# vxlerian/cpu-raymarcher

Measured on AMD Instinct MI355X. Metric: frames/sec, 3840x2160 Dense-Grid sphere-trace (+ avg SDF-calls/pixel), higher is better.
Workload: dtype f64

## Files before the change

cpu_raymarcher_amd/_native.py:

```python
import ctypes as C
import os
import subprocess

_PKG = os.path.dirname(os.path.abspath(__file__))
LIB_PATH = os.environ.get("RM_HIP_LIB") or os.path.join(_PKG, "librm_hip.so")
CSRC = os.path.join(_PKG, "csrc")

RM_OK = 0
RM_E_INVALID = -1
RM_E_UNSUPPORTED = -2
RM_E_NO_DEVICE = -3
RM_E_HIP = -4
RM_E_NO_SCENE = -5
RM_E_NOMEM = -6
RM_SCENE_UPLOADED = -(2 ** 31)

_STATUS_NAMES = {0: "RM_OK", -1: "RM_E_INVALID", -2: "RM_E_UNSUPPORTED", -3: "RM_E_NO_DEVICE",
                 -4: "RM_E_HIP", -5: "RM_E_NO_SCENE", -6: "RM_E_NOMEM"}


class RmError(RuntimeError):
    def __init__(self, code, msg):
        super().__init__("%s (%d): %s" % (_STATUS_NAMES.get(code, "?"), code, msg))
        self.code = code
# ... 48 lines not shown
class rm_field_shade(C.Structure):
    _fields_ = [("map", C.c_int32), ("reserved", C.c_int32), ("range", C.c_double), ("band", C.c_double), ("line", C.c_double),
                ("lo", C.c_uint32), ("hi", C.c_uint32)]


FIELD_MAPS = {"distance": 0, "count": 1}


class rm_point_query(C.Structure):
    _fields_ = [("time", C.c_double), ("iso", C.c_double), ("snap_tol", C.c_double), ("snap_steps", C.c_int32), ("flags", C.c_int32),
                ("reserved", C.c_int32 * 2)]


RM_POINT_NORMAL = 1


class rm_mesh_info(C.Structure):
    _fields_ = [("n_vertices", C.c_int64), ("n_quads", C.c_int64), ("n_holes", C.c_int64), ("reserved", C.c_int64)]


RM_MESH_F64, RM_MESH_F32 = 0, 1


class rm_view(C.Structure):
    _fields_ = [("camera_pitch", C.c_double), ("camera_yaw", C.c_double), ("time", C.c_double)]


class rm_frame_set(C.Structure):
    _fields_ = [("depth", C.c_void_p), ("normal", C.c_void_p), ("sdf", C.c_void_p), ("iters", C.c_void_p)]


class rm_compare_stats(C.Structure):
    _fields_ = [(name, C.c_uint64) for name in (
        "pixels", "sum_sdf_a", "sum_sdf_b", "sum_iters_a", "sum_iters_b", "sum_abs_depth", "surface_a", "surface_b",
        "surface_only_a", "surface_only_b", "depth_differs", "normal_differs", "counters_differ", "b_cheaper", "a_cheaper")] + \
        [("max_abs_depth", C.c_uint32), ("max_abs_normal", C.c_uint32)]


COMPARE_MAPS = {"none": -1, "sdf": 0, "iters": 1, "depth": 2, "normal": 3, "surface": 4}

RM_HIST_BINS = 256


class rm_counter_hist(C.Structure):
    _fields_ = [("pixels", C.c_uint64), ("sum", C.c_uint64), ("min", C.c_uint32), ("max", C.c_uint32), ("range_lo", C.c_uint32),
                ("range_hi", C.c_uint32), ("shift", C.c_uint32), ("reserved", C.c_uint32), ("bins", C.c_uint32 * RM_HIST_BINS)]


class rm_frame_hist(C.Structure):
    _fields_ = [("sdf", rm_counter_hist), ("iters", rm_counter_hist)]


HIST_MASKS = {"all": 0, "surface": 1, "background": 2}


class rm_scene_info(C.Structure):
    _fields_ = [("n_prims", C.c_int32), ("accel", C.c_int32), ("preset_index", C.c_int32),
                ("bvh_nodes", C.c_int32), ("bvh_leaves", C.c_int32), ("bvh_depth", C.c_int32),
                ("oct_nodes", C.c_int32), ("oct_leaves", C.c_int32), ("oct_empty_leaves", C.c_int32),
                ("oct_max_leaf_prims", C.c_int32), ("root_min", C.c_float * 3), ("root_max", C.c_float * 3),
                ("nodes_in_lds", C.c_int32), ("program", C.c_int32)]


class rm_node(C.Structure):
    _fields_ = [("type", C.c_int32), ("child_a", C.c_int32), ("child_b", C.c_int32), ("reserved", C.c_int32),
                ("world_to_local", C.c_float * 16), ("params", C.c_double * 6)]


class rm_prim(C.Structure):
    _fields_ = [("type", C.c_int32), ("reserved", C.c_int32), ("world_to_local", C.c_float * 16),
                ("params", C.c_double * 3), ("reserved2", C.c_double)]


class rm_sphere_edit(C.Structure):
    _fields_ = [("op", C.c_int32), ("index", C.c_int32), ("center", C.c_float * 3), ("reserved", C.c_int32),
                ("radius", C.c_double)]


RM_EDIT_SET, RM_EDIT_INSERT, RM_EDIT_REMOVE = 0, 1, 2
EDIT_OPS = {"set": 0, "insert": 1, "remove": 2}
SCENE_TABLES = {"spheres": "<f4", "radii": "<f8", "bvh": "u1", "bvh_prims": "<i4", "oct": "u1", "oct_prims": "<i4",
                "pq_cells": "<u4", "pq_list": "<u2", "nn_cells": "<u4", "nn_list": "<u2", "prims": "u1", "prog": "u1",
                "obj_ranges": "<i4", "oct_recs": "u1", "oct_lut": "<i4", "oct_sub_hdr": "<u4", "oct_sub_list": "u1",
                "slot_object": "<i4", "ext_cells": "<u4", "ext_list": "<u2", "step_tab": "<u4"}
STEP_BOX_BINS, STEP_BOX_CAP = 32, 62


class rm_diagnostics(C.Structure):
    _fields_ = [("total_sdf_calls", C.c_uint64), ("total_iterations", C.c_uint64),
                ("max_sdf_calls", C.c_uint32), ("min_sdf_calls", C.c_uint32), ("total_pixels", C.c_uint64)]


_VP = C.c_void_p
SIGNATURES = {
    "rm_create": (C.c_int, [C.c_int, C.POINTER(_VP)]),
    "rm_destroy": (None, [_VP]),
    "rm_last_error": (C.c_char_p, [_VP]),
    "rm_last_kernel": (C.c_char_p, [_VP]),
    "rm_version": (C.c_char_p, []),
    "rm_algorithm_from_string": (C.c_int, [C.c_char_p]),
    "rm_accel_from_string": (C.c_int, [C.c_char_p]),
    "rm_shader_from_string": (C.c_int, [C.c_char_p]),
    "rm_preset_count": (C.c_int, []),
    "rm_scene_from_preset": (C.c_int, [_VP, C.c_int32, C.c_int32]),
    "rm_scene_from_spheres": (C.c_int, [_VP, _VP, _VP, C.c_int32, C.c_int32]),
    "rm_scene_edit_spheres": (C.c_int, [_VP, C.POINTER(rm_sphere_edit), C.c_int32]),
    "rm_debug_scene_table": (C.c_int, [_VP, C.c_char_p, C.c_int32, _VP, C.c_int64, C.POINTER(C.c_int64)]),
    "rm_selftest_hypot64": (C.c_int, [_VP, _VP, C.c_int64, C.c_int32, _VP]),
    "rm_scene_from_prims": (C.c_int, [_VP, C.POINTER(rm_prim), C.c_int32, C.c_int32]),
    "rm_make_transform": (C.c_int, [C.c_double, C.c_double, C.c_double, _VP, _VP]),
    "rm_scene_from_nodes": (C.c_int, [_VP, C.POINTER(rm_node), C.c_int32, _VP, C.c_int32, C.c_int32]),
    "rm_scale_transform": (C.c_int, [_VP, C.c_double, C.c_double, C.c_double]),
    "rm_scene_set_time": (C.c_int, [_VP, C.c_double]),
    "rm_selftest_jsmath": (C.c_int, [_VP, C.c_int32, _VP, _VP, C.c_int64, _VP]),
    "rm_scene_get_info": (C.c_int, [_VP, C.POINTER(rm_scene_info)]),
    "rm_camera_from_angles": (C.c_int, [C.c_double, C.c_double, _VP, _VP]),
    "rm_scene_distance": (C.c_int, [_VP, _VP, C.c_int64, _VP, _VP]),
    "rm_debug_wave_distance": (C.c_int, [_VP, _VP, C.c_int64, _VP, _VP]),
    "rm_scene_field": (C.c_int, [_VP, C.POINTER(rm_lattice), _VP, _VP, _VP]),
    "rm_scene_field_device": (C.c_int, [_VP, C.POINTER(rm_lattice), _VP, _VP, _VP, _VP]),
    "rm_scene_points": (C.c_int, [_VP, C.POINTER(rm_point_query), C.c_int64, _VP, _VP, _VP, _VP, _VP, _VP, _VP]),
    "rm_scene_points_device": (C.c_int, [_VP, C.POINTER(rm_point_query), C.c_int64, _VP, _VP, _VP, _VP, _VP, _VP, _VP, _VP]),
    "rm_lattice_points": (C.c_int, [C.POINTER(rm_lattice), C.c_int64, C.c_int64, _VP]),
    "rm_shade_field_device": (C.c_int, [_VP, C.POINTER(rm_field_shade), C.c_int64, _VP, _VP, _VP]),
    "rm_shade_field": (C.c_int, [_VP, C.POINTER(rm_field_shade), C.c_int64, _VP, _VP]),
    "rm_mesh_field_device": (C.c_int, [_VP, C.POINTER(rm_lattice), _VP, C.c_int32, C.c_double, _VP, C.c_int64, _VP, C.c_int64, _VP, _VP]),
    "rm_scene_mesh": (C.c_int, [_VP, C.POINTER(rm_lattice), C.c_double, _VP, C.c_int64, _VP, C.c_int64, C.POINTER(rm_mesh_info)]),
    "rm_ray_march": (C.c_int, [_VP, C.POINTER(rm_ray_query), C.c_int64, _VP, _VP, _VP, _VP, _VP, _VP]),
    "rm_ray_march_device": (C.c_int, [_VP, C.POINTER(rm_ray_query), C.c_int64, _VP, _VP, _VP, _VP, _VP, _VP, _VP]),
    "rm_camera_rays": (C.c_int, [C.c_int32, C.c_int32, C.c_double, C.c_double, C.c_int32, C.c_int32, _VP, _VP]),
    "rm_ray_pick": (C.c_int, [_VP, C.POINTER(rm_ray_query), C.c_int64, _VP, _VP, _VP, _VP, _VP, _VP, _VP]),
    "rm_ray_pick_device": (C.c_int, [_VP, C.POINTER(rm_ray_query), C.c_int64, _VP, _VP, _VP, _VP, _VP, _VP, _VP, _VP]),
    "rm_ray_light": (C.c_int, [_VP, C.POINTER(rm_ray_query), C.POINTER(rm_light), C.c_int64, _VP, _VP, _VP, _VP, _VP, _VP, _VP, _VP, _VP,
                               _VP]),
    "rm_ray_light_device": (C.c_int, [_VP, C.POINTER(rm_ray_query), C.POINTER(rm_light), C.c_int64, _VP, _VP, _VP, _VP, _VP, _VP, _VP, _VP,
                                      _VP, _VP, _VP]),
    "rm_ray_walk": (C.c_int, [_VP, C.POINTER(rm_ray_query), C.c_int64, _VP, _VP, C.c_int32, _VP, _VP]),
    "rm_ray_walk_device": (C.c_int, [_VP, C.POINTER(rm_ray_query), C.c_int64, _VP, _VP, C.c_int32, _VP, _VP, _VP]),
    "rm_phong_light": (C.c_int, [_VP]),
    "rm_shade_lit_device": (C.c_int, [_VP, C.c_int32, C.c_int32, C.c_int32, _VP, _VP, _VP, _VP, _VP, _VP]),
    "rm_shade_lit": (C.c_int, [_VP, C.c_int32, C.c_int32, C.c_int32, _VP, _VP, _VP, _VP, _VP]),
    "rm_scene_object": (C.c_int, [_VP, C.c_int32, C.POINTER(rm_node), C.c_int32, C.POINTER(C.c_int32)]),
    "rm_render_tile": (C.c_int, [_VP, C.POINTER(rm_job), _VP, _VP, _VP, _VP]),
    "rm_render_tile_device": (C.c_int, [_VP, C.POINTER(rm_job), C.c_int32, _VP, _VP, _VP, _VP, _VP, _VP]),
    "rm_render_frames_device": (C.c_int, [_VP, C.POINTER(rm_job), C.c_int32, _VP, C.c_int32, _VP, _VP, _VP, _VP, _VP, _VP, _VP]),
    "rm_compare_frames_device": (C.c_int, [_VP, C.c_int32, C.c_int32, C.c_int32, C.POINTER(rm_frame_set), C.POINTER(rm_frame_set),
                                           C.c_int32, C.c_int32, _VP, _VP, _VP]),
    "rm_compare_frames": (C.c_int, [_VP, C.c_int32, C.c_int32, C.c_int32, C.POINTER(rm_frame_set), C.POINTER(rm_frame_set),
                                    C.c_int32, C.c_int32, _VP, _VP]),
    "rm_counter_hist_device": (C.c_int, [_VP, C.c_int32, C.c_int32, C.c_int32, _VP, _VP, _VP, C.c_int32, C.c_int32, C.c_int32, C.c_int32,
                                         _VP, _VP]),
    "rm_counter_hist": (C.c_int, [_VP, C.c_int32, C.c_int32, C.c_int32, _VP, _VP, _VP, C.c_int32, C.c_int32, C.c_int32, C.c_int32, _VP]),
    "rm_shade_ranged_device": (C.c_int, [_VP, C.c_int32, C.c_int32, C.c_int32, C.c_int32, _VP, _VP, C.c_uint32, C.c_uint32, _VP, _VP]),
    "rm_shade_ranged": (C.c_int, [_VP, C.c_int32, C.c_int32, C.c_int32, C.c_int32, _VP, _VP, C.c_uint32, C.c_uint32, _VP]),
    "rm_sweep_views": (C.c_int, [C.c_double, C.c_double, C.c_double, C.c_double, C.c_double, C.c_double, C.c_int32, _VP]),
    "rm_render_stripes_device": (C.c_int, [_VP, C.POINTER(rm_job), C.c_int32, C.c_int32, C.c_int32, C.c_int32,
                                           _VP, _VP, _VP, _VP, _VP, _VP]),
    "rm_stripe_rows": (C.c_int, [C.c_int32, C.c_int32, C.c_int32, C.c_int32, C.c_int32]),
    "rm_deal_stripes": (C.c_int, [C.c_int32, C.c_int32, C.c_int32, _VP, _VP]),
    "rm_render_stripe_list_device": (C.c_int, [_VP, C.POINTER(rm_job), C.c_int32, C.c_int32, _VP, C.c_int32,
                                               _VP, _VP, _VP, _VP, _VP, _VP]),
    "rm_assemble_frame_device": (C.c_int, [_VP, _VP, C.c_int64, C.c_int64, C.c_int32, C.c_int32, C.c_int32, _VP,
                                           C.c_int32, C.c_int32, _VP, C.c_int64, _VP, _VP]),
    "rm_shade": (C.c_int, [_VP, C.c_int32, C.c_int32, C.c_int32, _VP, _VP, _VP, _VP, _VP]),
    "rm_shade_device": (C.c_int, [_VP, C.c_int32, C.c_int32, C.c_int32, _VP, _VP, _VP, _VP, _VP, _VP]),
    "rm_reduce_counters": (C.c_int, [_VP, _VP, _VP, C.c_int64, C.POINTER(rm_diagnostics)]),
    "rm_reduce_counters_device": (C.c_int, [_VP, _VP, _VP, C.c_int64, C.POINTER(rm_diagnostics), _VP]),
    "rm_reduce_counters_enqueue": (C.c_int, [_VP, _VP, _VP, C.c_int64, _VP, _VP]),
    "rm_render_attach_diagnostics": (C.c_int, [_VP, _VP]),
    "rm_partition_rows": (C.c_int, [C.c_int32, C.c_int32, C.c_int32, C.POINTER(C.c_int32), C.POINTER(C.c_int32)]),
    "rm_selftest_hypot": (C.c_int, [_VP, _VP, C.c_int64, _VP]),
    "rm_selftest_fastdiv": (C.c_int, [_VP, C.c_uint64, C.c_int64, C.POINTER(C.c_uint64)]),
    "rm_selftest_recip": (C.c_int, [_VP, C.c_int, _VP]),
    "rm_debug_read_stamps": (C.c_int, [_VP, _VP]),
    "rm_debug_read_wave_times": (C.c_int, [_VP, _VP]),
    "rm_debug_read_batch_log": (C.c_int, [_VP, _VP]),
    "rm_debug_read_counts": (C.c_int, [_VP, _VP]),
    "rm_debug_read_lpt_costs": (C.c_int, [_VP, _VP, C.c_int64]),
    "rm_debug_launch_fill": (C.c_int, [_VP, C.c_int32, C.POINTER(C.c_int32)]),
    "rm_debug_last_launch": (C.c_int, [_VP, C.POINTER(C.c_uint32)]),
    "rm_debug_overlap_fill": (C.c_int, [_VP, C.c_int32, C.c_int64, C.POINTER(C.c_int32)]),
    "rm_debug_step_box": (C.c_int, [_VP, C.POINTER(C.c_int32)]),
    "rm_debug_rect_cull": (C.c_int, [_VP, _VP, _VP, C.c_int32, C.c_int32, C.POINTER(C.c_int32)]),
    "rm_debug_leaf_rects": (C.c_int, [_VP, _VP, _VP, C.c_int32, C.c_int32, _VP, _VP, C.c_int64, C.POINTER(C.c_int64)]),
    "rm_rtc_source": (C.c_int, [_VP, C.c_char_p, C.c_int64, C.POINTER(C.c_int64)]),
    "rm_rtc_compile_check": (C.c_int, [_VP, C.c_int32, C.c_int32, C.c_char_p, C.c_int64, C.POINTER(C.c_double)]),
    "rm_rtc_status": (C.c_int, [_VP, C.POINTER(C.c_int32), C.POINTER(C.c_int32), C.c_char_p, C.c_int64]),
    "rm_set_option": (C.c_int, [_VP, C.c_char_p, C.c_int64]),
    "rm_get_option": (C.c_int, [_VP, C.c_char_p, C.POINTER(C.c_int64)]),
}

_lib = None


def build(force=False, verbose=False):
    srcs = [os.path.join(CSRC, f) for f in os.listdir(CSRC) if f.endswith((".hip", ".cpp", ".h"))]
    srcs.append(os.path.join(os.path.dirname(_PKG), "include", "rm_raymarch.h"))
    if not force and os.path.exists(LIB_PATH) and all(
            os.path.getmtime(LIB_PATH) >= os.path.getmtime(s) for s in srcs):
        return LIB_PATH
    cmd = ["make", "-j%d" % min(8, os.cpu_count() or 1), "-C", CSRC, "all"] + (["-B"] if force else [])
    subprocess.check_call(cmd, stdout=None if verbose else subprocess.DEVNULL)
    return LIB_PATH


def lib():
    global _lib
    if _lib is None:
        if not os.path.exists(LIB_PATH):
            raise ImportError(
                "cpu_raymarcher_amd: %s is missing. Build it with `python -c 'import __graft_entry__ as g; "
                "g.build()'` or `make -C cpu_raymarcher_amd/csrc`. There is no CPU fallback." % LIB_PATH)
        try:
            import torch
        except ImportError:
            pass
        L = C.CDLL(LIB_PATH)
        for name, (res, args) in SIGNATURES.items():
            if os.environ.get("RM_HIP_LIB") and not hasattr(L, name):
                continue
            fn = getattr(L, name)
            fn.restype = res
            fn.argtypes = args
        _lib = L
    return _lib


def check(ctx, rc):
    if rc == RM_OK:
        return
    msg = lib().rm_last_error(ctx).decode() if ctx else ""
    raise (RmUnsupported if rc == RM_E_UNSUPPORTED else RmError)(rc, msg)
```

cpu_raymarcher_amd/context.py:

```python
import collections
import ctypes as C

import numpy as np

from . import _native as N

Points = collections.namedtuple("Points", "position dist normal object steps count")


def _is_torch(x):
    return type(x).__module__.startswith("torch")


def _ptr(x):
    if x is None:
        return None
    if _is_torch(x):
        return C.c_void_p(x.data_ptr())
    return x.ctypes.data_as(C.c_void_p)


_BPP = {"depth": 1, "normal": 3, "sdf": 2, "iters": 2, "rgba": 4}


# ... 53 lines not shown
    if not (_is_torch(hist) or isinstance(hist, np.ndarray)):
        raise ValueError("hist must be a numpy array or a torch tensor")
    d = bool(_is_torch(hist) and hist.is_cuda)
    contiguous = hist.is_contiguous() if _is_torch(hist) else hist.flags["C_CONTIGUOUS"]
    nbytes = hist.numel() * hist.element_size() if _is_torch(hist) else hist.nbytes
    if not contiguous or nbytes < 2128 * max(0, n_frames):
        raise ValueError("hist must be a contiguous buffer of 2128 bytes per frame")
    if on_dev is not None and on_dev != d:
        raise ValueError("buffers must be all on the host or all on the device")
    return d


def percentile(record, permille):
    p = int(permille)
    if not 0 <= p <= 1000:
        raise ValueError("permille must be in [0, 1000]")
    M = int(record["pixels"])
    if M == 0:
        return 0, 0
    r = p * (M - 1) // 1000
    b = int(np.searchsorted(np.cumsum(np.asarray(record["bins"], dtype=np.uint64)), r, side="right"))
    shift, mn, mx = int(record["shift"]), int(record["min"]), int(record["max"])
    return max(mn, b << shift), (mx if b == 255 else min(mx, ((b + 1) << shift) - 1))


def _current_stream_ptr():
    import torch
    return C.c_void_p(torch.cuda.current_stream().cuda_stream)


class Context:

    def __init__(self, device=0):
        self._h = C.c_void_p()
        self.device = -1 if device is None else int(device)
        rc = N.lib().rm_create(self.device, C.byref(self._h))
        if rc != N.RM_OK:
            raise N.RmError(rc, "rm_create(device=%d) failed: no usable HIP device" % self.device)

    def close(self):
        if self._h:
            N.lib().rm_destroy(self._h)
            self._h = C.c_void_p()

    def __del__(self):
        try:
            self.close()
        except Exception:
            pass

    def __enter__(self):
        return self

    def __exit__(self, *a):
        self.close()

    def set_option(self, key, value):
        N.check(self._h, N.lib().rm_set_option(self._h, key.encode(), int(value)))

    def get_option(self, key):
        v = C.c_int64(0)
        N.check(self._h, N.lib().rm_get_option(self._h, key.encode(), C.byref(v)))
        return v.value

    def launch_fill(self, asked):
        v = C.c_int32(0)
        N.check(self._h, N.lib().rm_debug_launch_fill(self._h, int(asked), C.byref(v)))
        return v.value

    def last_launch(self):
        out = (C.c_uint32 * 4)()
        N.check(self._h, N.lib().rm_debug_last_launch(self._h, out))
        return dict(workgroups=out[0], threads=out[1], lds_bytes=out[2], cus=out[3])

    def overlap_fill(self, asked, items):
        v = C.c_int32(0)
        N.check(self._h, N.lib().rm_debug_overlap_fill(self._h, int(asked), int(items), C.byref(v)))
        return v.value

    def step_box(self):
        out = (C.c_int32 * 6)()
        N.check(self._h, N.lib().rm_debug_step_box(self._h, out))
        return dict(last=bool(out[0]), planned=bool(out[1]), reason=out[2], list_cap=out[3], list_cap_without=out[4], table_bytes=out[5])

    def rect_cull(self, rot, origin, width, height):
        r = np.ascontiguousarray(rot, dtype=np.float32).reshape(9)
        o = np.ascontiguousarray(origin, dtype=np.float32).reshape(3)
        out = (C.c_int32 * 5)()
        N.check(self._h, N.lib().rm_debug_rect_cull(self._h, _ptr(r), _ptr(o), int(width), int(height), out))
        return dict(last=bool(out[0]), planned=bool(out[1]), reason=out[2], leaves=out[3], max_leaves=out[4])

    def leaf_rects(self, rot, origin, width, height):
        r = np.ascontiguousarray(rot, dtype=np.float32).reshape(9)
        o = np.ascontiguousarray(origin, dtype=np.float32).reshape(3)
        n = C.c_int64(0)
        N.check(self._h, N.lib().rm_debug_leaf_rects(self._h, _ptr(r), _ptr(o), int(width), int(height), None, None, 0, C.byref(n)))
        rects = np.zeros((max(1, n.value), 4), np.uint16)
        nodes = np.zeros(max(1, n.value), np.int32)
        N.check(self._h, N.lib().rm_debug_leaf_rects(self._h, _ptr(r), _ptr(o), int(width), int(height), _ptr(rects), _ptr(nodes),
                                                     n.value, C.byref(n)))
        return rects[:n.value], nodes[:n.value]

    def scene_from_preset(self, index, accel):
        N.check(self._h, N.lib().rm_scene_from_preset(self._h, int(index), int(accel)))

    def scene_from_spheres(self, centers, radii, accel):
        c = np.ascontiguousarray(centers, dtype=np.float32).reshape(-1, 3)
        r = np.ascontiguousarray(radii, dtype=np.float64).reshape(-1)
        if len(c) != len(r):
            raise ValueError("centers and radii differ in length")
        N.check(self._h, N.lib().rm_scene_from_spheres(self._h, _ptr(c), _ptr(r), len(r), int(accel)))

    def scene_from_prims(self, prims, accel):
        prims = list(prims)
        arr = (N.rm_prim * max(1, len(prims)))()
        for i, (t, m, par) in enumerate(prims):
            arr[i].type = int(t)
            for k in range(16):
                arr[i].world_to_local[k] = float(m[k])
            for k in range(3):
                arr[i].params[k] = float(par[k]) if k < len(par) else 0.0
        N.check(self._h, N.lib().rm_scene_from_prims(self._h, arr, len(prims), int(accel)))

    def scene_from_nodes(self, nodes, roots, accel):
        nodes = list(nodes)
        arr = (N.rm_node * max(1, len(nodes)))()
        for i, (t, a, b, m, par) in enumerate(nodes):
            arr[i].type, arr[i].child_a, arr[i].child_b = int(t), int(a), int(b)
            for k in range(16):
                arr[i].world_to_local[k] = 0.0 if m is None else float(m[k])
            for k in range(6):
                arr[i].params[k] = float(par[k]) if k < len(par) else 0.0
        r = np.ascontiguousarray(roots, dtype=np.int32)
        N.check(self._h, N.lib().rm_scene_from_nodes(self._h, arr, len(nodes), _ptr(r), len(r), int(accel)))

    def edit_spheres(self, edits):
        if isinstance(edits, C.Array) and edits._type_ is N.rm_sphere_edit:
            arr, n = edits, len(edits)
        else:
            edits = list(edits)
            n = len(edits)
            arr = (N.rm_sphere_edit * max(1, n))()
            for k, e in enumerate(edits):
                arr[k].op = N.EDIT_OPS[e[0]] if isinstance(e[0], str) else int(e[0])
                arr[k].index = int(e[1])
                if len(e) > 2:
                    arr[k].center[:] = [float(v) for v in np.asarray(e[2], np.float32).reshape(3)]
                    arr[k].radius = float(e[3])
        N.check(self._h, N.lib().rm_scene_edit_spheres(self._h, arr, n))

    def scene_table(self, name, from_device=True):
        size = C.c_int64(0)
        key = name.encode()
        N.check(self._h, N.lib().rm_debug_scene_table(self._h, key, int(bool(from_device)), None, 0, C.byref(size)))
        out = np.zeros(size.value, np.uint8)
        N.check(self._h, N.lib().rm_debug_scene_table(self._h, key, int(bool(from_device)), _ptr(out), out.size, C.byref(size)))
        return out.view(N.SCENE_TABLES.get(name, "u1"))

    def selftest_hypot64(self, xyz, on_device=True):
        a = np.ascontiguousarray(xyz, dtype=np.float64).reshape(-1, 3)
        out = np.zeros(len(a), np.float64)
        N.check(self._h, N.lib().rm_selftest_hypot64(self._h, _ptr(a), len(a), int(bool(on_device)), _ptr(out)))
        return out

    def scene_set_time(self, time):
        N.check(self._h, N.lib().rm_scene_set_time(self._h, float(time)))
# ... 789 lines not shown
```

cpu_raymarcher_amd/csrc/rm_api.cpp:

```cpp
#include <hip/hip_runtime_api.h>

#include <algorithm>
#include <array>
#include <cerrno>
#include <climits>
#include <cmath>
#include <cstdio>
#include <cstdlib>
#include <cstring>
#include <functional>
#include <limits>
#include <map>
#include <unordered_map>
#include <new>
#include <string>
#include <vector>

#include "../../include/rm_raymarch.h"
#include "rm_diag.h"
#include "rm_kernels.h"
#include "rm_rtc.h"
#include "rm_scene_host.h"

namespace {

#define RM_SCENE_ARRAYS(X)                                                                                                        \
    X(spheres, 1) X(radii, 1) X(bvh, 1) X(bvh_prims, 1) X(oct, 1) X(oct_prims, 1) X(pq_cells, 1) X(pq_list, 1) X(nn_cells, 1)      \
    X(nn_list, 1) X(prims, 1) X(prog, 1) X(obj_ranges, 1) X(oct_recs, 1) X(oct_lut, 1) X(oct_sub_hdr, 1) X(oct_sub_list, 1)       \
    X(slot_object, 0) X(ext_cells, 1) X(ext_list, 1) X(step_tab, 1)

struct DeviceScene {
#define RM_X(name, always) decltype(rmh::HostScene::name)::value_type *name = nullptr;
    RM_SCENE_ARRAYS(RM_X)
#undef RM_X
    uint16_t *bvh_leaves = nullptr;
    int32_t bvh_leaf_count = 0;
};

struct SceneDesc {
    enum Kind { kSpheres, kPrims, kNodes } kind = kSpheres;
    std::vector<float> centers;
    std::vector<double> radii;
    std::vector<rmh::PrimDesc> prims;
    std::vector<rmh::NodeDesc> nodes;
    std::vector<int> roots;
};

struct LaunchSlots {
    static constexpr unsigned kLaunches = 1024, kHeads = 64, kHeadWords = 64;
    unsigned int *heads = nullptr;
    RmDiagBlock *blocks = nullptr;
    RmLeafRect *rects = nullptr;
    unsigned int head_slot = 0, block_slot = 0;

    hipError_t init() {
        const size_t head_bytes = sizeof(unsigned int) * kLaunches * kHeads * kHeadWords, block_bytes = sizeof(RmDiagBlock) * kLaunches;
        hipError_t e = hipMalloc(reinterpret_cast<void **>(&heads), head_bytes);
        if (e == hipSuccess) e = hipMemset(heads, 0, head_bytes);
        if (e == hipSuccess) e = hipMalloc(reinterpret_cast<void **>(&blocks), block_bytes);
        if (e == hipSuccess) e = hipMemset(blocks, 0, block_bytes);
        return e == hipSuccess ? hipMalloc(reinterpret_cast<void **>(&rects), sizeof(RmLeafRect) * kLaunches * RM_RECT_CULL_MAX_LEAVES) : e;
    }
    void release() {
        (void)hipFree(heads);
        (void)hipFree(blocks);
        (void)hipFree(rects);
    }
    RmLeafRect *rects_of_last_heads() { return rects && head_slot ? rects + static_cast<size_t>(RM_RECT_CULL_MAX_LEAVES) * ((head_slot - 1) % kLaunches) : nullptr; }
    unsigned int *take_heads() { return heads ? heads + static_cast<size_t>(kHeads) * kHeadWords * (head_slot++ % kLaunches) : nullptr; }
    RmDiagBlock *take_block() { return blocks ? blocks + block_slot++ % kLaunches : nullptr; }
};

struct RingClaims {
    struct Claim {
        size_t first, n;
        hipEvent_t done;
    };
    size_t next = 0;
    std::vector<Claim> claims;

    void retire_all() {
        for (Claim &c : claims) (void)hipEventDestroy(c.done);
        claims.clear();
        next = 0;
    }
    hipError_t take(size_t n, size_t cap, size_t *first) {
        if (next + n > cap) next = 0;
        const size_t lo = next, hi = next + n;
        for (size_t k = 0; k < claims.size();) {
            const Claim c = claims[k];
            if (c.first < hi && lo < c.first + c.n) {
                const hipError_t e = hipEventSynchronize(c.done);
                if (e != hipSuccess) return e;
                (void)hipEventDestroy(c.done);
                claims.erase(claims.begin() + static_cast<std::ptrdiff_t>(k));
            } else ++k;
        }
        *first = lo;
        next = hi;
        return hipSuccess;
    }
    void launched(size_t first, size_t n, hipStream_t stream) {
        hipEvent_t ev = nullptr;
        if (hipEventCreateWithFlags(&ev, hipEventDisableTiming) == hipSuccess && hipEventRecord(ev, stream) == hipSuccess) {
            claims.push_back(Claim{first, n, ev});
            return;
        }
        if (ev) (void)hipEventDestroy(ev);
        (void)hipStreamSynchronize(stream);
    }
};

// ... 172 lines not shown
        for (auto &u : t.users) {
            (void)hipEventSynchronize(u.second);
            (void)hipEventDestroy(u.second);
        }
        t.users.clear();
        t.valid = false;
        const size_t n = static_cast<size_t>(oct_nodes);
        if (t.nodes < n) {
            (void)hipFree(t.dev);
            t.dev = nullptr;
            t.nodes = 0;
            if (hipMalloc(reinterpret_cast<void **>(&t.dev), n * sizeof(RmOctFrameNode)) == hipSuccess) t.nodes = n;
            else (void)hipGetLastError();
        }
        if (!t.dev || rm_launch_oct_frame_table(oct, oct_nodes, origin, t.dev, stream) != hipSuccess) return nullptr;
        for (int a = 0; a < 3; ++a) t.origin[a] = origin[a];
        t.gen = gen;
        t.valid = true;
        t.builder = stream;
        if (!t.built && hipEventCreateWithFlags(&t.built, hipEventDisableTiming) != hipSuccess) t.built = nullptr;
        if (!t.built || hipEventRecord(t.built, stream) != hipSuccess) (void)hipStreamSynchronize(stream);
        cur = k;
        return &t;
    }
    static void read_by(Table &t, hipStream_t stream) {
        hipEvent_t ev = nullptr;
        for (auto &u : t.users)
            if (u.first == stream) ev = u.second;
        if (!ev) {
            if (hipEventCreateWithFlags(&ev, hipEventDisableTiming) == hipSuccess) t.users.emplace_back(stream, ev);
            else ev = nullptr;
        }
        if (ev) (void)hipEventRecord(ev, stream);
        else (void)hipStreamSynchronize(stream);
    }
    void release() {
        for (Table &t : slots) {
            (void)hipFree(t.dev);
            for (auto &u : t.users) (void)hipEventDestroy(u.second);
            if (t.built) (void)hipEventDestroy(t.built);
        }
    }
};

}

struct rm_ctx {
    int device = -1;
    bool has_device = false;
    std::string err = "";
    hipStream_t stream = nullptr;

    bool have_scene = false;
    bool scene_is_uploaded = false;
    int scene_preset = 0;
    rmh::HostScene host;
    DeviceScene dev;

    bool have_uploaded = false;
    SceneDesc uploaded;
    double time = 0.0;

    void *scratch = nullptr;
    size_t scratch_bytes = 0;
    hipEvent_t scratch_busy = nullptr;
    RmDiagDevice *d_diag = nullptr;
    float light[3] = {0, 0, 0};

    int64_t opt_tile_w = 8;
    bool tile_w_set = false;
    int64_t opt_filter = 1;
    int64_t opt_lds = 1;
    int64_t opt_kernel = 0;
    int64_t opt_list_cap = 32;
    int64_t opt_coop = 1;
    int64_t opt_grid = 1;
    int64_t opt_nn = 2;
    int64_t opt_ext = 1;
    int64_t opt_blocks_per_cu = 6;
    int64_t opt_lds_fill = 0;
    int64_t opt_min_fill = 1;
    int64_t opt_overlap_fill = 1;
    int hw_queues = 4;
    uint32_t last_v2_shape[5] = {0, 0, 0, 0, 0};
    int64_t opt_item_wide = 0;
    int64_t opt_multi_step = 1;
    int64_t opt_step_box = 1;
    int64_t opt_lds_kb = 0;
    int64_t opt_refill = 64;
    int64_t opt_recs = 1;
    int64_t opt_static = 0;
    int64_t opt_lut = 1;
    int64_t opt_cull = 1;
    int64_t opt_rect_cull = 1;
    std::vector<uint16_t> cull_leaves;
    int64_t opt_rel = 1;
    int64_t opt_uniform = 1;
    int64_t opt_sub = 1;
    int64_t opt_hw_xcd = 1;
    int64_t opt_v1_lists = 1;
    int64_t opt_v1_block = 64;
    int64_t opt_oct_lean = 1;
    int64_t opt_lpt = 1;
    LaunchSlots slots;
    LptRing lpt;
    OctTableRing oct_tables;
    FrameRing frames;
    CompareRing compare;
    HistRing hists;
    unsigned long long scene_gen = 0;
    int64_t opt_n0_batch = 64;
    int64_t opt_length = 0;
    const char *last_kernel = "";
    std::string last_kernel_kept;
    int64_t opt_device_build = 1;
    int64_t opt_specialise = 1;
    int64_t opt_rtc_spheres = 16;
    int64_t opt_prune = 1;
    std::string rtc_src;
    std::map<int, rmrtc::Kernel> rtc_kernels;
    std::vector<rmrtc::Kernel> rtc_owned;
    std::map<int, std::string> rtc_failed;
    std::string rtc_log;
    struct V2Special {
        int launches = 0;
        int state = 0;
        bool lite = false;
        rmrtc::Kernel k;
    };
    std::unordered_map<uint64_t, V2Special> v2_special;
    int64_t opt_v2_after = 3;
    struct DevTable {
        std::vector<int32_t> host;
        int32_t *dev = nullptr;
    };
    std::vector<DevTable> tables;
    int64_t opt_item_px = 128;
    void *diag_next = nullptr;
    unsigned long long *d_stamps = nullptr;
    int num_cus = 256;
};

namespace {

int fail(rm_ctx *ctx, int code, const std::string &msg) {
    if (ctx) ctx->err = msg;
    return code;
}

int hip_fail(rm_ctx *ctx, hipError_t e, const char *what) {
    return fail(ctx, RM_E_HIP, std::string(what) + ": " + hipGetErrorString(e));
}

int read_hw_queues() {
    const char *s = std::getenv("GPU_MAX_HW_QUEUES");
    if (!s || !*s) return 4;
    char *end = nullptr;
    errno = 0;
    const long long v = std::strtoll(s, &end, 10);
    if (errno || end == s || *end != '\0' || v <= 0) return 4;
    return static_cast<int>(std::min<long long>(v, INT_MAX));
}

int launch_fill(int asked, int queues, bool min_fill) {
    if (!min_fill) return asked;
    const int q = queues > 0 ? queues : 4;
    return std::max(asked, (RM_V2_WAVES + q - 1) / q);
}

int overlap_fill(int asked, int queues, bool min_fill, bool overlap) {
// ... 567 lines not shown
    p.step_size = std::isnan(job->step_size) ? 0.1 : job->step_size;
    p.local_rows = job->y_end > job->y_start ? job->y_end - job->y_start : 0;
    p.stripe_rows = 0;
    p.n_parts = 1;
    p.part = 0;
    rmh::camera_from_angles(job->camera_pitch, job->camera_yaw, p.rot, p.origin);
    std::memcpy(p.light, ctx->light, sizeof p.light);
    for (int k = 0; k < 9; ++k) p.rot_d[k] = p.rot[k];
    for (int k = 0; k < 3; ++k) {
        p.origin_d[k] = p.origin[k];
        p.light_d[k] = p.light[k];
    }
    fill_scene_view(ctx, p);
    if (!std::isfinite(job->time)) return fail(ctx, RM_E_INVALID, "non-finite time");
    ctx->time = job->time;
    p.time = job->time;
    p.tile_w = static_cast<int32_t>(ctx->opt_tile_w);
    p.nodes_in_lds = static_cast<int32_t>(ctx->opt_lds);
    p.filter = static_cast<int32_t>(ctx->opt_filter);
    p.variant = static_cast<int32_t>(ctx->opt_kernel);
    if (p.variant == 0)
        p.variant = (ctx->host.accel == RM_ACCEL_OCTREE || ctx->host.spheres.size() < 8 ||
                     (ctx->opt_specialise && !ctx->rtc_src.empty() && rmrtc::available(nullptr) &&
                      static_cast<int64_t>(ctx->host.spheres.size()) < ctx->opt_rtc_spheres))
                        ? 1
                        : 2;
    if (p.algorithm != RM_ALG_SPHERE_TRACER) p.variant = 1;
    if (ctx->host.general) p.variant = 1;
    if (p.variant == 1 && !ctx->tile_w_set) p.tile_w = 8;
    p.list_cap = static_cast<int32_t>(ctx->opt_list_cap);
    p.coop = static_cast<int32_t>(ctx->opt_coop);
    p.bvh_prim_count = static_cast<int32_t>(ctx->host.bvh_prims.size());
    p.oct_prim_count = static_cast<int32_t>(ctx->host.oct_prims.size());
    p.blocks_per_cu = static_cast<int32_t>(ctx->opt_blocks_per_cu);
    p.launch_per_cu = launch_fill(p.blocks_per_cu, ctx->hw_queues, ctx->opt_min_fill != 0);
    p.overlap_per_cu = overlap_fill(p.blocks_per_cu, ctx->hw_queues, ctx->opt_min_fill != 0, ctx->opt_overlap_fill != 0);
    p.num_cus = ctx->num_cus;
    p.refill_threshold = static_cast<int32_t>(ctx->opt_refill);
    p.hw_xcd = static_cast<int32_t>(ctx->opt_hw_xcd);
    p.item_px = static_cast<int32_t>(ctx->opt_item_px);
    p.stamps = ctx->d_stamps;
    for (int k = 0; k < 3; ++k) {
        p.pq_dim[k] = ctx->host.pq_dim[k];
        p.pq_origin[k] = ctx->host.pq_origin[k];
        p.pq_inv[k] = ctx->host.pq_inv[k];
        p.pq_cell[k] = ctx->host.pq_inv[k] > 0.f ? static_cast<float>((1.0 / static_cast<double>(ctx->host.pq_inv[k])) * 0.9999) : 0.f;
    }
    p.pq_cell_count = static_cast<int32_t>(ctx->host.pq_cells.size());
    p.pq_list_count = static_cast<int32_t>(ctx->host.pq_list.size());
    p.use_grid = (ctx->opt_grid && !ctx->host.pq_cells.empty()) ? 1 : 0;
    p.pq_cells = ctx->dev.pq_cells;
    p.pq_list = ctx->dev.pq_list;
    p.bvh_leaves = ctx->dev.bvh_leaves;
    p.bvh_leaf_count = (ctx->opt_cull && ctx->host.accel == RM_ACCEL_BVH) ? ctx->dev.bvh_leaf_count : 0;
    p.rect_cull = rect_cull_refusal(ctx, p.rot, p.origin, p.width, p.height) == 0 ? 1 : 0;
    p.nn_cells = ctx->dev.nn_cells;
    p.nn_list = ctx->dev.nn_list;
    p.nn_cell_count = static_cast<int32_t>(ctx->host.nn_cells.size());
    p.nn_list_count = static_cast<int32_t>(ctx->host.nn_list.size());
    const bool nn_on = ctx->opt_nn == 1 || (ctx->opt_nn == 2 && ctx->host.spheres.size() <= 512);
    p.use_nn = (p.use_grid && nn_on && !ctx->host.nn_cells.empty()) ? 1 : 0;
    p.leaf_order = ctx->host.leaf_order ? 1 : 0;
    p.rel_boxes = static_cast<int32_t>(ctx->opt_rel);
    p.n0_batch = static_cast<int32_t>(ctx->opt_n0_batch);
    p.v1_lists = static_cast<int32_t>(ctx->opt_v1_lists);
    p.v1_block = static_cast<int32_t>(ctx->opt_v1_block);
    p.oct_lean = static_cast<int32_t>(ctx->opt_oct_lean);
    p.v1_list_offset = -1;
    p.prim_filter = (ctx->opt_filter && ctx->host.general && !ctx->host.program && ctx->host.prim_filter_ok &&
                     ctx->host.spheres.size() == ctx->host.prims.size()) ? 1 : 0;
    p.lds_budget_kb = static_cast<int32_t>(ctx->opt_lds_kb);
    p.lds_fill = static_cast<int32_t>(ctx->opt_lds_fill);
    p.item_wide = static_cast<int32_t>(ctx->opt_item_wide);
    p.multi_step = static_cast<int32_t>(ctx->opt_multi_step);
    p.step_tab = ctx->dev.step_tab;
    p.sb_bins = ctx->host.sb_bins;
    p.sb_stride = ctx->host.sb_stride;
    for (int k = 0; k < 3; ++k) {
        p.sb_origin[k] = ctx->host.sb_origin[k];
        p.sb_inv[k] = ctx->host.sb_inv[k];
    }
    p.step_box = (ctx->opt_step_box && ctx->opt_multi_step && ctx->host.accel == RM_ACCEL_BVH && !ctx->host.step_tab.empty() &&
                  (ctx->dev.step_tab || !ctx->has_device)) ? 1 : 0;
    p.uniform_radius = 0;
    if (ctx->opt_uniform && !ctx->host.general && ctx->host.spheres.size() >= 2 &&
        ctx->host.spheres.size() <= 256) {
        const auto &sp = ctx->host.spheres;
        const auto &rd = ctx->host.radii;
        bool same = rd.size() == sp.size();
        for (size_t k = 1; same && k < sp.size(); ++k)
            same = std::memcmp(&sp[k].rf, &sp[0].rf, sizeof(float)) == 0 && std::memcmp(&rd[k], &rd[0], sizeof(double)) == 0;
        p.uniform_radius = same ? 1 : 0;
    }
    for (int k = 0; k < 3; ++k) {
        p.nn_dim[k] = ctx->host.nn_dim[k];
        p.nn_inv[k] = ctx->host.nn_inv[k];
    }
    p.oct_recs = ctx->opt_recs ? ctx->dev.oct_recs : nullptr;
    p.oct_sub_hdr = (ctx->opt_sub && ctx->opt_recs) ? ctx->dev.oct_sub_hdr : nullptr;
    p.oct_sub_list = ctx->dev.oct_sub_list;
    return RM_OK;
}

template <typename Launch>
int read_mismatches(rm_ctx *ctx, Launch launch, uint64_t *mismatches) {
    RM_HIP(ctx, hipSetDevice(ctx->device));
    Staging st{ctx};
    const size_t o = st.region(sizeof(unsigned long long));
    const int rc = st.reserve();
    if (rc) return rc;
    RM_HIP(ctx, st.zero(o, sizeof(unsigned long long)));
    RM_HIP(ctx, launch(st.at<unsigned long long>(o)));
    unsigned long long h = 0;
    RM_HIP(ctx, st.out(&h, o, sizeof h));
    RM_HIP(ctx, st.sync());
    *mismatches = h;
    return RM_OK;
}

int norm_shader(int s) { return (s >= RM_SHADE_NORMAL && s <= RM_SHADE_ITERATION_HEATMAP) ? s : RM_SHADE_NORMAL; }

int fill_query_params(rm_ctx *ctx, const rm_ray_query *q, RmRenderParams &p) {
    const double scene_time = ctx->time;
    rm_job job;
    std::memset(&job, 0, sizeof job);
    job.width = 1;
    job.height = 1;
    job.y_end = 1;
    job.time = q->time;
    const bool known = q->algorithm >= RM_ALG_SPHERE_TRACER && q->algorithm <= RM_ALG_ADAPTIVE_STEP_V3;
    job.algorithm = known ? q->algorithm : RM_ALG_SPHERE_TRACER;
    job.scene_preset_index = ctx->scene_is_uploaded ? RM_SCENE_UPLOADED : ctx->scene_preset;
    job.acceleration_structure = ctx->host.accel;
    job.overshoot_factor = q->overshoot_factor;
    job.step_size = q->step_size;
    const int rc = fill_params(ctx, &job, p);
    ctx->time = scene_time;
    p.rtc_function = nullptr;
    return rc;
}

int check_query(rm_ctx *ctx, const rm_ray_query *q, int64_t n, const void *origins, const void *dirs) {
    if (!q) return fail(ctx, RM_E_INVALID, "null query");
    if (n < 0 || n > std::numeric_limits<int32_t>::max()) return fail(ctx, RM_E_INVALID, "ray count out of range");
    if (n > 0 && (!origins || !dirs)) return fail(ctx, RM_E_INVALID, "null ray buffer");
    if (!ctx->has_device) return fail(ctx, RM_E_NO_DEVICE, "host-only context: there is no CPU ray path");
    if (!ctx->have_scene) return fail(ctx, RM_E_NO_SCENE, "no scene set");
    return RM_OK;
}

struct RayColumn {
    void *ptr;
    size_t bytes;
    size_t member;
    bool in;
};
constexpr int kRayMaxColumns = 8;
template <typename Args>
struct RayCall {
    Args args;
    hipError_t (*launch[2])(const RmRenderParams &, const RmRays &, const Args &, hipStream_t, const char **);
    int64_t chunk;
    int n_cols;
    RayColumn cols[kRayMaxColumns];
};
constexpr int64_t kRayChunk = int64_t(1) << 22;
// ... 1756 lines not shown
    if (ok) return RM_OK;
    if (text.compare(0, 8, "refused:") == 0) return fail(ctx, RM_E_UNSUPPORTED, "hiprtc: the specialised kernel spills and would not be loaded (see the log)");
    return fail(ctx, RM_E_INVALID, "hiprtc: the specialised kernel did not compile (see the log)");
}

int rm_rtc_status(rm_ctx *ctx, int32_t *compiled, int32_t *failed, char *log, int64_t cap) {
    if (!ctx) return RM_E_INVALID;
    int v2_ready = 0, v2_failed = 0;
    for (const auto &kv : ctx->v2_special) {
        v2_ready += kv.second.state == 1;
        v2_failed += kv.second.state < 0;
    }
    if (compiled) *compiled = static_cast<int32_t>(ctx->rtc_kernels.size()) + v2_ready;
    if (failed) *failed = static_cast<int32_t>(ctx->rtc_failed.size()) + v2_failed;
    std::string why;
    if (!rmrtc::available(&why)) return copy_text(why, log, cap, nullptr);
    return copy_text(ctx->rtc_log, log, cap, nullptr);
}

int rm_debug_read_lpt_costs(rm_ctx *ctx, uint8_t *out, int64_t n) {
    if (!out) return RM_E_INVALID;
    RM_NEED_DEVICE(ctx, "host-only context");
    const uint8_t *costs = ctx->lpt.last_costs();
    if (!costs || n < 0 || static_cast<size_t>(n) > LptRing::kPerSlot) return fail(ctx, RM_E_INVALID, "no costs recorded");
    RM_HIP(ctx, hipSetDevice(ctx->device));
    RM_HIP(ctx, hipDeviceSynchronize());
    RM_HIP(ctx, hipMemcpy(out, costs, static_cast<size_t>(n), hipMemcpyDeviceToHost));
    return RM_OK;
}

int rm_debug_launch_fill(rm_ctx *ctx, int32_t asked, int32_t *effective) {
    if (!ctx || !effective) return RM_E_INVALID;
    if (asked < 1 || asked > 8) return fail(ctx, RM_E_INVALID, "blocks_per_cu must be in [1, 8]");
    *effective = launch_fill(asked, ctx->hw_queues, ctx->opt_min_fill != 0);
    return RM_OK;
}

int rm_debug_overlap_fill(rm_ctx *ctx, int32_t asked, int64_t items, int32_t *effective) {
    if (!ctx || !effective) return RM_E_INVALID;
    if (asked < 1 || asked > 8) return fail(ctx, RM_E_INVALID, "blocks_per_cu must be in [1, 8]");
    if (items < 0) return fail(ctx, RM_E_INVALID, "items must not be negative");
    const bool min_fill = ctx->opt_min_fill != 0;
    *effective = rm_v2_overlap_per_cu(launch_fill(asked, ctx->hw_queues, min_fill),
                                      overlap_fill(asked, ctx->hw_queues, min_fill, ctx->opt_overlap_fill != 0), items, ctx->num_cus);
    return RM_OK;
}

int rm_debug_last_launch(rm_ctx *ctx, uint32_t out[4]) {
    if (!ctx || !out) return RM_E_INVALID;
    for (int k = 0; k < 3; ++k) out[k] = ctx->last_v2_shape[k];
    out[3] = static_cast<uint32_t>(ctx->num_cus);
    return RM_OK;
}

int rm_debug_step_box(rm_ctx *ctx, int32_t out[6]) {
    if (!ctx || !out) return RM_E_INVALID;
    for (int k = 0; k < 6; ++k) out[k] = 0;
    out[0] = static_cast<int32_t>(ctx->last_v2_shape[3]);
    if (!ctx->have_scene) return fail(ctx, RM_E_NO_SCENE, "no scene set");
    rm_job job;
    std::memset(&job, 0, sizeof job);
    job.width = job.height = job.y_end = 64;
    job.algorithm = RM_ALG_SPHERE_TRACER;
    job.scene_preset_index = ctx->scene_is_uploaded ? RM_SCENE_UPLOADED : ctx->scene_preset;
    job.acceleration_structure = ctx->host.accel;
    job.overshoot_factor = job.step_size = std::nan("");
    const double scene_time = ctx->time;
    RmRenderParams p;
    const int rc = fill_params(ctx, &job, p);
    ctx->time = scene_time;
    if (rc) return rc;
    out[5] = static_cast<int32_t>(ctx->host.step_tab.size() * sizeof(uint32_t));
    RmRenderParams plain = p;
    plain.step_box = 0;
    out[4] = rm_v2_plan(plain).list_cap;
    const RmV2Plan plan = rm_v2_plan(p);
    out[3] = plan.list_cap;
    const bool v2 = p.variant == 2 && p.algorithm == 0 && p.accel == 2;
    out[1] = v2 && plan.step_box ? 1 : 0;
    out[2] = out[1] ? 0 : (ctx->host.step_tab.empty() && v2 && ctx->opt_step_box && ctx->opt_multi_step ? 2 : (v2 && plan.refused ? 3 : 1));
    return RM_OK;
}

int rm_debug_rect_cull(rm_ctx *ctx, const float *rot9, const float *origin3, int32_t width, int32_t height, int32_t out[5]) {
    if (!ctx || !out || !rot9 || !origin3) return RM_E_INVALID;
    for (int k = 0; k < 5; ++k) out[k] = 0;
    out[0] = static_cast<int32_t>(ctx->last_v2_shape[4]);
    out[4] = RM_RECT_CULL_MAX_LEAVES;
    if (!ctx->have_scene) return fail(ctx, RM_E_NO_SCENE, "no scene set");
    rm_job job;
    std::memset(&job, 0, sizeof job);
    job.width = job.height = job.y_end = 64;
    job.algorithm = RM_ALG_SPHERE_TRACER;
    job.scene_preset_index = ctx->scene_is_uploaded ? RM_SCENE_UPLOADED : ctx->scene_preset;
    job.acceleration_structure = ctx->host.accel;
    job.overshoot_factor = job.step_size = std::nan("");
    const double scene_time = ctx->time;
    RmRenderParams p;
    const int rc = fill_params(ctx, &job, p);
    ctx->time = scene_time;
    if (rc) return rc;
    out[3] = static_cast<int32_t>(ctx->cull_leaves.size());
    const bool v2 = p.variant == 2 && p.algorithm == 0 && p.accel == 2;
    out[2] = v2 ? rect_cull_refusal(ctx, rot9, origin3, width, height) : 1;
    out[1] = out[2] == 0 ? 1 : 0;
    return RM_OK;
}

int rm_debug_leaf_rects(rm_ctx *ctx, const float *rot9, const float *origin3, int32_t width, int32_t height, uint16_t *rects,
                        int32_t *nodes, int64_t cap, int64_t *n) {
    if (!ctx || !n || !rot9 || !origin3 || cap < 0) return RM_E_INVALID;
    *n = 0;
    int32_t why[5];
    const int rc = rm_debug_rect_cull(ctx, rot9, origin3, width, height, why);
    if (rc) return rc;
    if (!why[1]) return RM_OK;
    *n = static_cast<int64_t>(ctx->cull_leaves.size());
    for (int64_t j = 0; j < *n && j < cap; ++j) {
        const RmBvhNode &nd = ctx->host.bvh[ctx->cull_leaves[static_cast<size_t>(j)]];
        const RmLeafRect r = rm_leaf_rect(nd.lo, nd.hi, origin3, rot9, width, height);
        if (rects) {
            rects[4 * j] = r.x_lo;
            rects[4 * j + 1] = r.x_hi;
            rects[4 * j + 2] = r.y_lo;
            rects[4 * j + 3] = r.y_hi;
        }
        if (nodes) nodes[j] = ctx->cull_leaves[static_cast<size_t>(j)];
    }
    return RM_OK;
}

enum OptionKind {
    kSwitch,
    kRange,
    kZeroOrRange,
    kSet,
};
struct OptionRow {
    const char *key;
    int64_t rm_ctx::*member;
    OptionKind kind;
    int64_t v[4];
    const char *error;
};
static const OptionRow kOptions[] = {
    {"tile_w", &rm_ctx::opt_tile_w, kSet, {8, 16, 32, 64}, "tile_w must be 8, 16, 32 or 64"},
    {"filter", &rm_ctx::opt_filter, kSwitch, {}, nullptr},
    {"nodes_in_lds", &rm_ctx::opt_lds, kSwitch, {}, nullptr},
    {"kernel", &rm_ctx::opt_kernel, kRange, {0, 2}, "kernel must be 0 (auto), 1 or 2"},
    {"list_cap", &rm_ctx::opt_list_cap, kRange, {1, 64}, "list_cap must be in [1, 64]"},
    {"coop", &rm_ctx::opt_coop, kSwitch, {}, nullptr},
    {"recs", &rm_ctx::opt_recs, kSwitch, {}, nullptr},
    {"lut", &rm_ctx::opt_lut, kSwitch, {}, nullptr},
    {"uniform", &rm_ctx::opt_uniform, kSwitch, {}, nullptr},
    {"lds_kb", &rm_ctx::opt_lds_kb, kZeroOrRange, {16, 64}, "lds_kb must be 0 (auto) or in [16, 64]"},
    {"multi_step", &rm_ctx::opt_multi_step, kSwitch, {}, nullptr},
    {"step_box", &rm_ctx::opt_step_box, kSwitch, {}, nullptr},
    {"item_wide", &rm_ctx::opt_item_wide, kSwitch, {}, nullptr},
    {"prune", &rm_ctx::opt_prune, kSwitch, {}, nullptr},
    {"rtc_spheres", &rm_ctx::opt_rtc_spheres, kRange, {0, 33}, "rtc_spheres must be 0..33"},
    {"specialise_v2_after", &rm_ctx::opt_v2_after, kRange, {0, 1000000}, "specialise_v2_after must be 0 (never) .. 1000000 launches"},
    {"specialise", &rm_ctx::opt_specialise, kRange, {0, 2}, "specialise must be 0, 1 or 2"},
    {"lds_fill", &rm_ctx::opt_lds_fill, kSwitch, {}, nullptr},
    {"min_fill", &rm_ctx::opt_min_fill, kSwitch, {}, nullptr},
    {"overlap_fill", &rm_ctx::opt_overlap_fill, kSwitch, {}, nullptr},
    {"cull", &rm_ctx::opt_cull, kSwitch, {}, nullptr},
    {"rect_cull", &rm_ctx::opt_rect_cull, kSwitch, {}, nullptr},
    {"rel", &rm_ctx::opt_rel, kSwitch, {}, nullptr},
    {"static", &rm_ctx::opt_static, kRange, {0, 95}, "static must be in [0, 95] percent"},
    {"sub", &rm_ctx::opt_sub, kSwitch, {}, nullptr},
    {"refill", &rm_ctx::opt_refill, kRange, {1, 64}, "refill must be in [1, 64]"},
    {"item_px", &rm_ctx::opt_item_px, kSet, {64, 128, 256, 256}, "item_px must be 64, 128 or 256"},
    {"hw_xcd", &rm_ctx::opt_hw_xcd, kSwitch, {}, nullptr},
    {"grid", &rm_ctx::opt_grid, kSwitch, {}, nullptr},
    {"nn", &rm_ctx::opt_nn, kRange, {0, 2}, "nn must be 0 (off), 1 (on) or 2 (auto)"},
    {"ext", &rm_ctx::opt_ext, kSwitch, {}, nullptr},
    {"blocks_per_cu", &rm_ctx::opt_blocks_per_cu, kRange, {1, 8}, "blocks_per_cu must be in [1, 8]"},
    {"v1_lists", &rm_ctx::opt_v1_lists, kSwitch, {}, nullptr},
    {"v1_block", &rm_ctx::opt_v1_block, kSet, {64, 128, 256, 256}, "v1_block must be 64, 128 or 256"},
    {"oct_lean", &rm_ctx::opt_oct_lean, kSwitch, {}, nullptr},
    {"lpt", &rm_ctx::opt_lpt, kSwitch, {}, nullptr},
    {"n0_batch", &rm_ctx::opt_n0_batch, kRange, {1, 64}, "n0_batch must be in [1, 64]"},
    {"device_build", &rm_ctx::opt_device_build, kSwitch, {}, nullptr},
    {"length", &rm_ctx::opt_length, kRange, {0, 1}, "length must be 0 (Math.hypot) or 1 (Math.sqrt)"},
};

static const OptionRow *find_option(const char *key) {
    for (const OptionRow &o : kOptions)
        if (!std::strcmp(key, o.key)) return &o;
    return nullptr;
}

int rm_set_option(rm_ctx *ctx, const char *key, int64_t value) {
    if (!ctx || !key) return RM_E_INVALID;
    const OptionRow *o = find_option(key);
    if (!o) return fail(ctx, RM_E_INVALID, std::string("unknown option ") + key);
    bool ok = true;
    switch (o->kind) {
        case kSwitch: value = value ? 1 : 0; break;
        case kRange: ok = value >= o->v[0] && value <= o->v[1]; break;
        case kZeroOrRange: ok = value == 0 || (value >= o->v[0] && value <= o->v[1]); break;
        case kSet: ok = std::find(std::begin(o->v), std::end(o->v), value) != std::end(o->v); break;
    }
    if (!ok) return fail(ctx, RM_E_INVALID, o->error);
    const bool changed = ctx->*(o->member) != value;
    ctx->*(o->member) = value;
    if (o->member == &rm_ctx::opt_tile_w) ctx->tile_w_set = true;
    if (o->member == &rm_ctx::opt_length && changed && ctx->have_scene) {
        ctx->have_scene = false;
        return ensure_scene(ctx, ctx->scene_is_uploaded ? RM_SCENE_UPLOADED : ctx->scene_preset, ctx->host.accel);
    }
    return RM_OK;
}

int rm_get_option(const rm_ctx *ctx, const char *key, int64_t *value) {
    if (!ctx || !key || !value) return RM_E_INVALID;
    const OptionRow *o = find_option(key);
    if (!o) return RM_E_INVALID;
    *value = ctx->*(o->member);
    return RM_OK;
}

}
```

cpu_raymarcher_amd/csrc/rm_kernels.h:

```cpp
#pragma once
#ifndef __HIPCC_RTC__
#include <hip/hip_runtime_api.h>
#include <stdint.h>
#endif

#include "rm_types.h"

struct RmDiagDevice {
    unsigned long long total_sdf;
    unsigned long long total_iters;
    unsigned int max_sdf;
    unsigned int min_sdf;
    unsigned long long pad;
};

#ifdef RM_LENGTH_SQRT
#define RM_LEN_VARIANT(name) name##_sqrt
#define RM_LEN_TAG " [length=sqrt]"
#define RM_LEN_IS_SQRT true
#else
#define RM_LEN_VARIANT(name) name
#define RM_LEN_TAG ""
#define RM_LEN_IS_SQRT false
#endif
// ... 165 lines not shown
    unsigned int lo, hi;
    int map, pad;
};
#define RM_MESH_BLOCK 256
#define RM_MESH_SCAN_STEP 1024
struct RmMeshInfo {
    long long n_vertices, n_quads, n_holes, reserved;
};
struct RmMeshArgs {
    double origin[3], du[3], dv[3], dw[3];
    const void *values;
    double iso;
    float *vertices;
    uint32_t *quads;
    RmMeshInfo *info;
    uint32_t *map;
    uint32_t *totals;
    long long n, cap_vertices, cap_quads;
    unsigned int nu, nv, nw, n_blocks;
    int f32, pad;
};
struct RmCandGrid {
    double org[3], w[3];
    int32_t dim[3];
    int32_t first, n, pad;
};
#define RM_CAND_NO_LIST 0xFFFFFFFFu
struct RmCandArgs {
    const RmCandGrid *grids;
    const double *spheres;
    const int32_t *ids;
    uint32_t *counts;
    double *u;
    const uint32_t *offsets;
    long long n_cells;
    unsigned long long list_len;
    double u0;
    double root_lo[3], root_hi[3];
    int32_t n_grids, cells_per_grid, n_spheres, n_ids, use_root, pad;
};
struct RmEmptyDistArgs {
    const float *boxes, *prim_lo, *prim_hi;
    double *out;
    int32_t n_nodes, n_prims;
};

#ifndef __HIPCC_RTC__
hipError_t rm_launch_cand_count(const RmCandArgs &a, hipStream_t stream);
hipError_t rm_launch_cand_fill(const RmCandArgs &a, void *list, int elem_bytes, hipStream_t stream);
hipError_t rm_launch_empty_dist(const RmEmptyDistArgs &a, hipStream_t stream);
hipError_t rm_launch_hypot64(const double *xyz, int64_t n, double *out, hipStream_t stream);

hipError_t rm_launch_render(const RmRenderParams &p, hipStream_t stream, const char **kernel_name, uint32_t *v2_shape = nullptr);
hipError_t rm_launch_render_sqrt(const RmRenderParams &p, hipStream_t stream, const char **kernel_name, uint32_t *v2_shape = nullptr);

const void *rm_rtc_v2_hook(const RmRenderParams &p, int accel, bool lds, bool ur, bool rel, bool length_sqrt);

hipError_t rm_launch_render_v2(const RmRenderParams &p, hipStream_t stream, const char **kernel_name, uint32_t *shape = nullptr);
hipError_t rm_launch_render_v2_sqrt(const RmRenderParams &p, hipStream_t stream, const char **kernel_name, uint32_t *shape = nullptr);

#define RM_V2_OVERLAP_ITEMS_PER_WAVE 3
inline int rm_v2_overlap_per_cu(int floor_per_cu, int candidate, long long items, int cus) {
    if (candidate <= floor_per_cu || cus <= 0) return floor_per_cu;
    const long long needed = (items + 3) / 4, resident = static_cast<long long>(cus) * candidate;
    const long long waves = 4 * (needed < resident ? needed : resident);
    return items >= RM_V2_OVERLAP_ITEMS_PER_WAVE * waves ? candidate : floor_per_cu;
}

inline bool rm_rect_cull_camera_ok(const float rot[9], const float origin[3]) {
    for (int k = 0; k < 3; ++k)
        if (!(origin[k] - origin[k] == 0.f)) return false;
    for (int i = 0; i < 3; ++i)
        for (int j = i; j < 3; ++j) {
            double d = 0.0;
            for (int k = 0; k < 3; ++k) d += static_cast<double>(rot[3 * i + k]) * static_cast<double>(rot[3 * j + k]);
            const double err = d - (i == j ? 1.0 : 0.0);
            if (!(err >= -1e-6 && err <= 1e-6)) return false;
        }
    return true;
}

struct RmV2Plan {
    bool lds, rel;
    int list_cap, step_box, tier, refused;
    size_t scene_bytes, list_bytes;
};
RmV2Plan rm_v2_plan(const RmRenderParams &p);

hipError_t rm_launch_wave_distance(const RmRenderParams &p, const float *points, int64_t n, double *dist, uint32_t *count, hipStream_t stream);
hipError_t rm_launch_wave_distance_sqrt(const RmRenderParams &p, const float *points, int64_t n, double *dist, uint32_t *count, hipStream_t stream);

hipError_t rm_launch_oct_frame_table(const RmOctNode *nodes, int n, const double origin[3], RmOctFrameNode *out, hipStream_t stream);

hipError_t rm_launch_shade(int shader, int64_t n, const uint8_t *depth, const uint8_t *normal,
                           const uint16_t *sdf, const uint16_t *iters, uint8_t *rgba,
                           const float light[3], hipStream_t stream);

hipError_t rm_launch_reduce_init(RmDiagDevice *acc, hipStream_t stream);

hipError_t rm_launch_reduce(const uint16_t *sdf, const uint16_t *iters, int64_t n, RmDiagDevice *acc,
                            hipStream_t stream);

hipError_t rm_launch_distance(const RmRenderParams &p, const float *points, int64_t n, double *dist,
                              uint32_t *count, hipStream_t stream);
hipError_t rm_launch_distance_sqrt(const RmRenderParams &p, const float *points, int64_t n, double *dist,
                                   uint32_t *count, hipStream_t stream);

hipError_t rm_launch_cast(const RmRenderParams &p, const RmRays &r, const RmQueryArgs &a, hipStream_t stream, const char **kernel_name);
hipError_t rm_launch_cast_sqrt(const RmRenderParams &p, const RmRays &r, const RmQueryArgs &a, hipStream_t stream, const char **kernel_name);
hipError_t rm_launch_pick(const RmRenderParams &p, const RmRays &r, const RmQueryArgs &a, hipStream_t stream, const char **kernel_name);
hipError_t rm_launch_pick_sqrt(const RmRenderParams &p, const RmRays &r, const RmQueryArgs &a, hipStream_t stream, const char **kernel_name);
hipError_t rm_launch_light(const RmRenderParams &p, const RmRays &r, const RmLightArgs &a, hipStream_t stream, const char **kernel_name);
hipError_t rm_launch_light_sqrt(const RmRenderParams &p, const RmRays &r, const RmLightArgs &a, hipStream_t stream, const char **kernel_name);
hipError_t rm_launch_walk(const RmRenderParams &p, const RmRays &r, const RmWalkArgs &a, hipStream_t stream, const char **kernel_name);
hipError_t rm_launch_walk_sqrt(const RmRenderParams &p, const RmRays &r, const RmWalkArgs &a, hipStream_t stream, const char **kernel_name);

hipError_t rm_launch_field(const RmRenderParams &p, const RmFieldArgs &a, hipStream_t stream, const char **kernel_name);
hipError_t rm_launch_field_sqrt(const RmRenderParams &p, const RmFieldArgs &a, hipStream_t stream, const char **kernel_name);

hipError_t rm_launch_points(const RmRenderParams &p, const RmPointArgs &a, hipStream_t stream, const char **kernel_name);
hipError_t rm_launch_points_sqrt(const RmRenderParams &p, const RmPointArgs &a, hipStream_t stream, const char **kernel_name);

hipError_t rm_launch_mesh(const RmMeshArgs &a, hipStream_t stream, const char **kernel_name);

hipError_t rm_launch_frames(const RmRenderParams &p, const RmFrameView *views, int32_t n_views, RmFrameDiagBlock *blocks, RmDiagDevice *acc,
                            hipStream_t stream, const char **kernel_name);
hipError_t rm_launch_frames_sqrt(const RmRenderParams &p, const RmFrameView *views, int32_t n_views, RmFrameDiagBlock *blocks, RmDiagDevice *acc,
                                 hipStream_t stream, const char **kernel_name);

hipError_t rm_launch_lpt_sort(const uint8_t *cost_prev, uint16_t *perm, int stride, int tiles_x, int tiles_y, hipStream_t stream);

hipError_t rm_launch_assemble(const unsigned char *gathered, int64_t rank_stride, int64_t section_offset, int32_t row_bytes,
                              int32_t height, int32_t stripe_rows, const int32_t *stripe_src, int32_t n_stripes,
                              unsigned char *frame, int64_t acc_offset, int32_t world, RmDiagDevice *acc, hipStream_t stream);

int32_t rm_compare_blocks_per_frame(int64_t npx, int32_t n_frames);
hipError_t rm_launch_compare(const RmCompareArgs &a, int32_t map, int32_t n_frames, int32_t blocks_per_frame, hipStream_t stream,
                             const char **kernel_name);

hipError_t rm_launch_hist(const RmHistArgs &a, bool masked, int32_t n_frames, int32_t blocks_per_frame, hipStream_t stream,
                          const char **kernel_name);
hipError_t rm_launch_shade_ranged(const RmShadeRangedArgs &a, int32_t n_frames, hipStream_t stream, const char **kernel_name);
hipError_t rm_launch_shade_lit(const RmShadeLitArgs &a, int32_t n_frames, hipStream_t stream, const char **kernel_name);
hipError_t rm_launch_shade_field(const RmShadeFieldArgs &a, hipStream_t stream, const char **kernel_name);

hipError_t rm_launch_hypot(const float *xyz, int64_t n, double *out, hipStream_t stream);
hipError_t rm_launch_jsmath(int fn, const double *a, const double *b, int64_t n, double *out, hipStream_t stream);

hipError_t rm_launch_fastdiv_selftest(uint64_t seed, int64_t n, unsigned long long *d_mismatches, hipStream_t stream);
hipError_t rm_launch_recip_selftest(int mode, unsigned long long *d_mismatches, hipStream_t stream);
#endif
```

cpu_raymarcher_amd/csrc/rm_render_v2.hip:

```cpp
#ifndef __HIPCC_RTC__
#include <hip/hip_runtime.h>
#endif

#include "rm_device.h"
#ifdef RM_RTC_V2
#include "rm_v2_fixed.inc"
#endif

#ifdef RM_COUNTS
__shared__ unsigned int rm_cnt_s[32];
#define RM_CNT(i)                                                                                  \
    {                                                                                              \
        const unsigned int n_ = static_cast<unsigned int>(__popcll(__ballot(1)));                  \
        const int l_ = static_cast<int>(__lane_id());                                              \
        if (__builtin_amdgcn_readfirstlane(l_) == l_) {                                            \
            atomicAdd(&rm_cnt_s[i], 1u);                                                           \
            atomicAdd(&rm_cnt_s[(i) + 16], n_);                                                    \
        }                                                                                          \
    }
__shared__ unsigned int rm_cnt_e[8];
#define RM_CNT_END(i)                                                                              \
    {                                                                                              \
        const unsigned int n_ = static_cast<unsigned int>(__popcll(__ballot(1)));                  \
        const int l_ = static_cast<int>(__lane_id());                                              \
// ... 116 lines not shown
            float err;
            const float a = sphere_sdf_estimate(S.spheres[j0], b, err);
            lb0 = a - err;
            ub = a + err < ub ? a + err : ub;
        }
        if (j1 < S.n_prims) {
            float err;
            const float a = sphere_sdf_estimate(S.spheres[j1], b, err);
            lb1 = a - err;
            ub = a + err < ub ? a + err : ub;
        }
        ub = wave_min_f32(ub);
        const bool c0 = lb0 <= ub, c1 = lb1 <= ub;
        double e0 = RM_MAX_DIST, e1 = RM_MAX_DIST;
        if (c0) e0 = sphere_sdf_fast(S.spheres[j0], S.radii[j0], b);
        double best = masked_min_f64(e0, __ballot(c0), RM_MAX_DIST);
        if (c1) e1 = sphere_sdf_fast(S.spheres[j1], S.radii[j1], b);
        return masked_min_f64(e1, __ballot(c1), best);
    }
    float ub = 10.0f;
    for (int j = lane; j < S.n_prims; j += 64) {
        float err;
        const float a = sphere_sdf_estimate(S.spheres[j], b, err);
        const float hi = a + err;
        ub = hi < ub ? hi : ub;
    }
    ub = wave_min_f32(ub);
    double best = RM_MAX_DIST;
    for (int j0 = 0; j0 < S.n_prims; j0 += 64) {
        const int j = j0 + lane;
        bool cand = false;
        double e = RM_MAX_DIST;
        if (j < S.n_prims) {
            const RmSphere s = S.spheres[j];
            float err;
            const float a = sphere_sdf_estimate(s, b, err);
            cand = a - err <= ub;
            if (cand) e = sphere_sdf_fast(s, S.radii[j], b);
        }
        best = masked_min_f64(e, __ballot(cand), best);
    }
    return best;
}

__device__ double all_prims_wave(const SceneView &S, bool need, const Vec3f &q, int lane, bool coop, bool filter) {
    double closest = RM_MAX_DIST;
    unsigned long long fb = __ballot(need);
    if (fb == 0) return closest;
    const int n = S.n_prims;
    const int m = __popcll(fb);
    const bool use_coop = coop && n > 8 && static_cast<long long>(m) * (28 * ((n + 63) / 64) + 250) < 16ll * n + 300;
    if (use_coop) {
        while (fb) {
            const int src = __builtin_ctzll(fb);
            fb &= fb - 1;
            RM_CNT(12)
            Vec3f b;
            b.x = readlane_f32(q.x, src);
            b.y = readlane_f32(q.y, src);
            b.z = readlane_f32(q.z, src);
            const double r = coop_all_prims(S, b, lane);
            if (lane == src) closest = r;
        }
    } else if (need) {
        closest = (filter && n >= 2) ? lane_min_filtered(S, nullptr, n, q, closest) : lane_min_exact(S, nullptr, n, q, closest);
    }
    return closest;
}

__device__ double bvh_distance_wave_seq(const RmRenderParams &P, const SceneView &S, bool need, const Vec3f &q,
                                    uint32_t &count, int lane, bool coop, bool filter, bool use_grid,
                                    unsigned long long *dbg_fallback_cycles) {
    double closest = RM_MAX_DIST;
    uint32_t found = 0;
    bool walk_tree = false;
    bool in_root = false;
    if (need && use_grid) {
        const RmBvhNode root = S.nodes[0];
        if (box_contains(root.lo, root.hi, q)) {
            const int cx = min(max(static_cast<int>((q.x - P.pq_origin[0]) * P.pq_inv[0]), 0), P.pq_dim[0] - 1);
            const int cy = min(max(static_cast<int>((q.y - P.pq_origin[1]) * P.pq_inv[1]), 0), P.pq_dim[1] - 1);
            const int cz = min(max(static_cast<int>((q.z - P.pq_origin[2]) * P.pq_inv[2]), 0), P.pq_dim[2] - 1);
            in_root = true;
            const uint32_t cell = S.pq_cells[(cz * P.pq_dim[1] + cy) * P.pq_dim[0] + cx];
            const int ccnt = static_cast<int>(cell & 0xFFu);
            if (ccnt == 255) walk_tree = true;
            else {
                const uint16_t *lst = S.pq_list + (cell >> 8);
                for (int e = 0; e < ccnt; ++e) {
                    const RmBvhNode node = S.nodes[lst[e]];
                    if (!box_contains(node.lo, node.hi, q)) continue;
                    const int first = node.leaf >> 8, cnt = node.leaf & 0xFF;
                    const int32_t *ids = P.leaf_order ? nullptr : S.bvh_prims + first;
                    closest = (filter && cnt >= 2) ? lane_min_filtered(S, ids, cnt, q, closest, first)
                                                   : lane_min_exact(S, ids, cnt, q, closest, first);
                    found += static_cast<uint32_t>(cnt);
                }
            }
        }
    }
    if (need && (!use_grid || walk_tree)) {
        int i = 0;
        const int n = S.bvh_nodes;
        while (i < n) {
            const RmBvhNode node = S.nodes[i];
            if (!box_contains(node.lo, node.hi, q)) {
                i = node.skip;
                continue;
            }
            if (node.leaf < 0) {
                i = i + 1;
                continue;
            }
            const int first = node.leaf >> 8, cnt = node.leaf & 0xFF;
            const int32_t *ids = P.leaf_order ? nullptr : S.bvh_prims + first;
            closest = (filter && cnt >= 2) ? lane_min_filtered(S, ids, cnt, q, closest, first)
                                           : lane_min_exact(S, ids, cnt, q, closest, first);
            found += static_cast<uint32_t>(cnt);
            i = node.skip;
        }
    }
    bool fallback = need && found == 0;
    bool served = false;
    if (fallback && P.use_nn && in_root) {
        const int nx = min(max(static_cast<int>((q.x - P.pq_origin[0]) * P.nn_inv[0]), 0), P.nn_dim[0] - 1);
        const int ny = min(max(static_cast<int>((q.y - P.pq_origin[1]) * P.nn_inv[1]), 0), P.nn_dim[1] - 1);
        const int nz = min(max(static_cast<int>((q.z - P.pq_origin[2]) * P.nn_inv[2]), 0), P.nn_dim[2] - 1);
        const uint32_t cell = S.nn_cells[(nz * P.nn_dim[1] + ny) * P.nn_dim[0] + nx];
        const int ccnt = static_cast<int>(cell & 0xFFu);
        if (ccnt != 255) {
            closest = prims_min_best<uint16_t>(S.spheres, S.radii, S.nn_list + (cell >> 8), ccnt, 0, q, RM_MAX_DIST);
            served = true;
        }
    }
#ifdef RM_STAMPS
    const unsigned long long t_fb0 = __builtin_amdgcn_s_memtime();
#endif
    const double all = all_prims_wave(S, fallback && !served, q, lane, coop, filter);
#ifdef RM_STAMPS
    if (dbg_fallback_cycles) *dbg_fallback_cycles += __builtin_amdgcn_s_memtime() - t_fb0;
#endif
    if (fallback) {
        if (!served) closest = all;
        count += static_cast<uint32_t>(S.n_prims);
    } else if (need) {
        count += found;
    }
    return closest;
}

struct BestScan {
    int k1;
    float hi1, lb1, lb2;
    uint32_t kbest, ksecond;
};
template <bool UR>
__device__ __forceinline__ void scan_sphere(BestScan &b, const RmSphere &s, int id, const Vec3f &p) {
    if (UR) {
        const float dx = p.x - s.cx, dy = p.y - s.cy, dz = p.z - s.cz;
        const float s2 = dx * dx + dy * dy + dz * dz;
        const uint32_t key = (__float_as_uint(s2) & 0xFFFFFF00u) | static_cast<uint32_t>(id);
        const uint32_t lo = min(key, b.kbest), hi = max(key, b.kbest);
        b.kbest = lo;
        b.ksecond = min(hi, b.ksecond);
        return;
    }
    float err;
    const float a = sphere_sdf_estimate(s, p, err);
    const float lb = a - err, hi = a + err;
    const bool better = hi < b.hi1;
    b.lb2 = __builtin_fminf(b.lb2, better ? b.lb1 : lb);
    b.k1 = better ? id : b.k1;
    b.lb1 = better ? lb : b.lb1;
    b.hi1 = better ? hi : b.hi1;
}
__device__ __forceinline__ void scan_finish_uniform(BestScan &b, float rf) {
    const float len = __builtin_amdgcn_sqrtf(b.lb2);
    const float lb = (len - rf) - (len + __builtin_fabsf(rf) + 1.0f) * 4e-6f;
    b.lb2 = b.lb2 < __builtin_inff() ? lb : __builtin_inff();
}

struct NormalAux {
    int k1;
    float lb2;
    uint32_t found;
    float rho;
    float rho_cell;
    bool ok;
};
#define RM_NRM_DELTA 0.010003f
__device__ __forceinline__ float box_margin(const float lo[3], const float hi[3], const Vec3f &p) {
    const float a = __builtin_fminf(__builtin_fminf(p.x - lo[0], p.y - lo[1]), p.z - lo[2]);
    const float b = __builtin_fminf(__builtin_fminf(hi[0] - p.x, hi[1] - p.y), hi[2] - p.z);
    return __builtin_fminf(a, b);
}

template <bool UR>
__device__ double bvh_distance_wave(const RmRenderParams &P, const SceneView &S, bool need, const Vec3f &q,
                                    uint32_t &count, int lane, bool coop, bool filter, bool use_grid,
                                    unsigned long long *dbg_fallback_cycles, NormalAux *aux) {
    aux->ok = false;
    aux->rho = 0.f;
    aux->rho_cell = 0.f;
    if (!filter) return bvh_distance_wave_seq(P, S, need, q, count, lane, coop, filter, use_grid, dbg_fallback_cycles);
    double closest = RM_MAX_DIST;
    uint32_t found = 0;
    bool walk_tree = false;
    bool in_root = false;
    float rho = __builtin_inff();
    float rho_cell = 0.f;
    uint32_t nleaf16 = 0xFFFF0000u;
    BestScan bs;
    bs.k1 = -1;
    bs.hi1 = bs.lb1 = bs.lb2 = __builtin_inff();
    bs.kbest = bs.ksecond = 0xFFFFFFFFu;
    auto scan_leaf = [&](const RmBvhNode &node) {
        const int first = node.leaf >> 8, cnt = node.leaf & 0xFF;
        for (int k = 0; k < cnt; ++k) {
            const int id = P.leaf_order ? first + k : S.bvh_prims[first + k];
            RM_CNT(8)
            scan_sphere<UR>(bs, S.spheres[id], id, q);
        }
        found += static_cast<uint32_t>(cnt);
    };
    if (need && use_grid) {
        const RmBvhNode root = S.nodes[0];
        const float m_root = box_margin(root.lo, root.hi, q);
        if (m_root >= 0.f) {
            const float gx = (q.x - P.pq_origin[0]) * P.pq_inv[0], gy = (q.y - P.pq_origin[1]) * P.pq_inv[1], gz = (q.z - P.pq_origin[2]) * P.pq_inv[2];
            const int cx = min(max(static_cast<int>(gx), 0), P.pq_dim[0] - 1);
            const int cy = min(max(static_cast<int>(gy), 0), P.pq_dim[1] - 1);
            const int cz = min(max(static_cast<int>(gz), 0), P.pq_dim[2] - 1);
            in_root = true;
            {
                const float fx = gx - static_cast<float>(cx), fy = gy - static_cast<float>(cy), fz = gz - static_cast<float>(cz);
                const float in_cell = __builtin_fminf(__builtin_fminf(__builtin_fminf(fx, 1.0f - fx) * P.pq_cell[0], __builtin_fminf(fy, 1.0f - fy) * P.pq_cell[1]),
                                                      __builtin_fminf(fz, 1.0f - fz) * P.pq_cell[2]);
                rho_cell = 0.0100f + __builtin_fmaxf(in_cell, 0.f);
            }
            rho = __builtin_fmaxf(__builtin_fmaxf(__builtin_fabsf(q.x), __builtin_fabsf(q.y)), __builtin_fabsf(q.z)) < 16.0f ? m_root : 0.f;
            const uint32_t cell = S.pq_cells[(cz * P.pq_dim[1] + cy) * P.pq_dim[0] + cx];
            const int ccnt = static_cast<int>(cell & 0xFFu);
            if (ccnt == 255) walk_tree = true;
            else {
                const uint16_t *lst = S.pq_list + (cell >> 8);
                for (int e = 0; e < ccnt; ++e) {
                    RM_CNT(7)
                    const RmBvhNode node = S.nodes[lst[e]];
                    const float m = box_margin(node.lo, node.hi, q);
                    rho = __builtin_fminf(rho, __builtin_fabsf(m));
                    if (m >= 0.f) {
                        scan_leaf(node);
                        found += 0x10000u;
                    }
                }
                nleaf16 = found & 0xFFFF0000u;
                found &= 0xFFFFu;
            }
        }
    }
    if (need && (!use_grid || walk_tree)) {
        rho = 0.f;
        int i = 0;
        const int n = S.bvh_nodes;
        while (i < n) {
            const RmBvhNode node = S.nodes[i];
            if (!box_contains(node.lo, node.hi, q)) {
                i = node.skip;
                continue;
            }
            if (node.leaf < 0) {
                i = i + 1;
                continue;
            }
            scan_leaf(node);
            i = node.skip;
        }
    }
    const bool fallback = need && found == 0;
    bool served = false;
    if (fallback && P.use_nn && in_root) {
        const int nx = min(max(static_cast<int>((q.x - P.pq_origin[0]) * P.nn_inv[0]), 0), P.nn_dim[0] - 1);
        const int ny = min(max(static_cast<int>((q.y - P.pq_origin[1]) * P.nn_inv[1]), 0), P.nn_dim[1] - 1);
        const int nz = min(max(static_cast<int>((q.z - P.pq_origin[2]) * P.nn_inv[2]), 0), P.nn_dim[2] - 1);
        const uint32_t cell = S.nn_cells[(nz * P.nn_dim[1] + ny) * P.nn_dim[0] + nx];
        const int ccnt = static_cast<int>(cell & 0xFFu);
        if (ccnt != 255) {
            const uint16_t *lst = S.nn_list + (cell >> 8);
            for (int e = 0; e < ccnt; ++e) {
                const int id = lst[e];
                RM_CNT(9)
                scan_sphere<UR>(bs, S.spheres[id], id, q);
            }
            served = true;
        }
    }
    if (fallback && !served && P.use_ext) {
        const float gx = (q.x - P.ext_origin[0]) * P.ext_inv[0], gy = (q.y - P.ext_origin[1]) * P.ext_inv[1], gz = (q.z - P.ext_origin[2]) * P.ext_inv[2];
        const float lo = __builtin_fminf(__builtin_fminf(gx, gy), gz);
        const bool inside = lo >= 0.f && gx < static_cast<float>(P.ext_dim[0]) && gy < static_cast<float>(P.ext_dim[1]) && gz < static_cast<float>(P.ext_dim[2]);
        if (inside) {
            const uint32_t cell = S.ext_cells[(static_cast<int>(gz) * P.ext_dim[1] + static_cast<int>(gy)) * P.ext_dim[0] + static_cast<int>(gx)];
            const int ccnt = static_cast<int>(cell & 0xFFu);
            if (ccnt != 255) {
                const uint16_t *lst = S.ext_list + (cell >> 8);
                for (int e = 0; e < ccnt; ++e) {
                    const int id = lst[e];
                    RM_CNT(9)
                    scan_sphere<UR>(bs, S.spheres[id], id, q);
                }
                served = true;
            }
        }
    }
    if (fallback && !served) RM_CNT(13)
    {
        const unsigned long long unserved = __ballot(fallback && !served);
        if (unserved) {
            const int n = S.n_prims, m = __popcll(unserved);
            const bool one_by_one = coop && n > 8 && static_cast<long long>(m) * (28 * ((n + 63) / 64) + 250) < 14ll * n + 200;
            if (!one_by_one && (!UR || n <= 256)) {
                if (fallback && !served) {
                    for (int id = 0; id < n; ++id) scan_sphere<UR>(bs, S.spheres[id], id, q);
                    served = true;
                }
            }
        }
    }
    bool redo = false;
    if (UR && bs.kbest != 0xFFFFFFFFu) {
        bs.k1 = static_cast<int>(bs.kbest & 0xFFu);
        bs.lb2 = bs.ksecond == 0xFFFFFFFFu ? __builtin_inff() : __uint_as_float(bs.ksecond & 0xFFFFFF00u);
    }
    if (bs.k1 >= 0) {
        RM_CNT(10)
        const RmSphere s1 = S.spheres[bs.k1];
        if (UR) scan_finish_uniform(bs, s1.rf);
        closest = sphere_sdf_fast(s1, S.radii[bs.k1], q);
        if (closest > RM_MAX_DIST) closest = RM_MAX_DIST;
        redo = bs.lb2 <= f32_upper_bound(closest);
    }
    {
        aux->k1 = bs.k1;
        aux->lb2 = bs.lb2;
// ... 82 lines not shown
#pragma unroll
    for (int p = 0; p < 4; ++p) {
        float mx = 0.f, mn = 0.f, mag = 0.f;
#pragma unroll
        for (int k = 0; k < 3; ++k) {
            const float a = ql[k] * b.n[p][k], c = qh[k] * b.n[p][k];
            mx += __builtin_fmaxf(a, c);
            mn += __builtin_fminf(a, c);
            mag += __builtin_fmaxf(__builtin_fabsf(a), __builtin_fabsf(c));
        }
        const float tol = 1e-6f * mag;
        miss = miss || ((p & 1) ? mn > tol : mx < -tol);
    }
    return miss;
}

__device__ __forceinline__ bool rect_overlaps(const RmLeafRect &q, int x0, int x1, int y0, int y1) {
    return x0 <= static_cast<int>(q.x_hi) && x1 >= static_cast<int>(q.x_lo) && y0 <= static_cast<int>(q.y_hi) && y1 >= static_cast<int>(q.y_lo);
}

template <bool REL>
__device__ bool bvh_prologue_cull(const SceneView &S, const RmRenderParams &C, int x0, int x1, int y0, int y1, bool rect,
                                  unsigned long long cand0, bool active, const Ray &r,
                                  const RayInv &ri, RayList &L, Interval &first, int lane) {
    bool have = false;
    L.cnt = 0;
    if (!rect) {
        const RmBvhNode root = S.nodes[0];
        double tE = 0.0, tX = 0.0;
        const bool hit = active && node_slab<REL>(S, root, 0, r, ri, tE, tX) && !(tX < 0.0) && !(tE > RM_MAX_DIST);
        if (!__any(hit)) {
            L.live = 0;
            return false;
        }
        active = hit;
    }
    const float o[3] = {C.origin[0], C.origin[1], C.origin[2]};
    Bundle B = {};
    if (!rect) B = make_bundle(C, x0, x1, y0, y1);
    for (int j0 = 0; j0 < C.bvh_leaf_count; j0 += 64) {
        const int j = j0 + lane;
        int li = 0;
        bool cand = false;
        if (j < C.bvh_leaf_count) {
            li = C.bvh_leaves[j];
            if (!rect) {
                const RmBvhNode nd = S.nodes[li];
                cand = !bundle_misses_box(B, nd.lo, nd.hi, o);
            } else if (j0 != 0) {
                cand = rect_overlaps(C.leaf_rects[j], x0, x1, y0, y1);
            }
        }
        unsigned long long m = rect && j0 == 0 ? cand0 : __ballot(cand);
        while (m) {
            const int src = __builtin_ctzll(m);
            m &= m - 1;
            const int i = __builtin_amdgcn_readlane(li, src);
            RM_CNT(5)
            if (active) {
                const RmBvhNode node = S.nodes[i];
                double tE, tX;
                if (node_slab<REL>(S, node, i, r, ri, tE, tX) && !(tX < 0.0) && !(tE > RM_MAX_DIST)) {
                    const double cE = __builtin_fmax(tE, 0.0);
                    const double cX = __builtin_fmin(tX, RM_MAX_DIST);
                    if (L.cnt < L.cap) L.col[L.cnt * 64] = static_cast<uint16_t>(i);
                    L.cnt++;
                    if (!have || cE < first.tEnter) {
                        first.tEnter = cE;
                        first.tExit = cX;
                        first.ord = i;
                        have = true;
                        L.cur_pos = L.cnt - 1;
                    }
                }
            }
        }
    }
    L.live = L.cnt;
    return have;
}


struct LdsLayout {
    uint32_t nodes, prims, cells, list, oct, oct_prims, spheres, radii, rel, end, step;
};
inline LdsLayout lds_layout_host(const RmRenderParams &C, int accel, bool lds, bool rel) {
    auto up = [](uint32_t v) { return (v + 15u) & ~15u; };
    auto words = [](uint32_t count, uint32_t size) { return ((count * size + 3u) / 4u) * 4u; };
    LdsLayout o = {0, 0, 0, 0, 0, 0, 0, 0, 0, 0, 0};
    uint32_t off = 0;
    if (lds) {
        if (accel == 2) {
            o.nodes = off = up(off);
            off += words(static_cast<uint32_t>(C.bvh_nodes), sizeof(RmBvhNode));
            o.prims = off = up(off);
            off += words(static_cast<uint32_t>(C.bvh_prim_count), 4);
            o.cells = off = up(off);
            off += words(static_cast<uint32_t>(C.pq_cell_count), 4);
            o.list = off = up(off);
            off += words(static_cast<uint32_t>(C.pq_list_count), 2);
        } else if (accel == 1) {
            o.oct = off = up(off);
            off += words(static_cast<uint32_t>(C.oct_nodes), sizeof(RmOctNode));
            o.oct_prims = off = up(off);
            off += words(static_cast<uint32_t>(C.oct_prim_count), 4);
        }
        o.spheres = off = up(off);
        off += words(static_cast<uint32_t>(C.n_prims), sizeof(RmSphere));
        o.radii = off = up(off);
        off += words(static_cast<uint32_t>(C.n_prims), 8);
        off = up(off);
        if (accel == 2 && C.step_box) {
            o.step = off;
            off = up(off + 3u * static_cast<uint32_t>(C.sb_stride) * 4u);
        }
        if (rel) {
            o.rel = off;
            off += static_cast<uint32_t>(C.bvh_nodes) * 48u;
        }
    }
    o.end = off;
    return o;
}
template <int ACCEL, bool LDS, bool REL>
__device__ __forceinline__ LdsLayout lds_layout(const RmRenderParams &C) {
    LdsLayout o;
    o.nodes = C.lds_off[0];
    o.prims = C.lds_off[1];
    o.cells = C.lds_off[2];
    o.list = C.lds_off[3];
    o.oct = C.lds_off[4];
    o.oct_prims = C.lds_off[5];
    o.spheres = C.lds_off[6];
    o.radii = C.lds_off[7];
    o.rel = C.lds_off[8];
    o.end = C.lds_off[9];
    o.step = C.lds_off[10];
    return o;
}
template <int ACCEL, bool LDS, bool REL>
__device__ __forceinline__ SceneView scene_view(const RmRenderParams &C, unsigned char *smem) {
    SceneView S;
    S.nodes = C.bvh;
    S.bvh_prims = C.bvh_prims;
    S.oct = C.oct;
    S.oct_prims = C.oct_prims;
    S.spheres = C.spheres;
    S.radii = C.radii;
    S.pq_cells = C.pq_cells;
    S.pq_list = C.pq_list;
    S.nn_cells = C.nn_cells;
    S.nn_list = C.nn_list;
    S.ext_cells = C.ext_cells;
    S.ext_list = C.ext_list;
    S.rel = nullptr;
    S.n_prims = C.n_prims;
    S.bvh_nodes = C.bvh_nodes;
    if (LDS) {
        const LdsLayout o = lds_layout<ACCEL, LDS, REL>(C);
        if (ACCEL == 2) {
            S.nodes = reinterpret_cast<const RmBvhNode *>(smem + o.nodes);
            S.bvh_prims = reinterpret_cast<const int32_t *>(smem + o.prims);
            S.pq_cells = reinterpret_cast<const uint32_t *>(smem + o.cells);
            S.pq_list = reinterpret_cast<const uint16_t *>(smem + o.list);
        } else if (ACCEL == 1) {
            S.oct = reinterpret_cast<const RmOctNode *>(smem + o.oct);
            S.oct_prims = reinterpret_cast<const int32_t *>(smem + o.oct_prims);
        }
        S.spheres = reinterpret_cast<const RmSphere *>(smem + o.spheres);
        S.radii = reinterpret_cast<const double *>(smem + o.radii);
        if (REL) S.rel = reinterpret_cast<const double *>(smem + o.rel);
    }
    return S;
}

template <typename T>
__device__ __forceinline__ const T *stage(unsigned char *smem, size_t &off, const T *src, int count) {
    off = (off + 15) & ~static_cast<size_t>(15);
    T *dst = reinterpret_cast<T *>(smem + off);
    const int words = static_cast<int>((static_cast<size_t>(count) * sizeof(T) + 3) / 4);
    const uint32_t *s = reinterpret_cast<const uint32_t *>(src);
    uint32_t *d = reinterpret_cast<uint32_t *>(dst);
    for (int i = threadIdx.x; i < words; i += blockDim.x) d[i] = s[i];
    off += static_cast<size_t>(words) * 4;
    return dst;
}

#define RM_SUBQ 8
#define RM_QUEUES (8 * RM_SUBQ)
#define RM_QSTRIDE 64
inline int queue_rows_host(int tiles_y, int qid) {
    const int x = qid / RM_SUBQ, s = qid % RM_SUBQ, Rx = (tiles_y - x + 7) >> 3;
    return Rx > s ? (Rx - s + RM_SUBQ - 1) / RM_SUBQ : 0;
}
struct TileQueue {
    unsigned int *counters;
    int tiles_x, tiles_y, tile_w, tile_h, item_px;
    unsigned int tiles_x_magic;
    const uint16_t *perm;
    int perm_stride;
};

__device__ __forceinline__ int queue_rows(int tiles_y, int qid) {
    const int x = qid / RM_SUBQ, s = qid % RM_SUBQ;
    const int Rx = (tiles_y - x + 7) >> 3;
    return Rx > s ? (Rx - s + RM_SUBQ - 1) / RM_SUBQ : 0;
}

__device__ __forceinline__ bool queue_entry(const TileQueue &Q, int qid, unsigned int k, int &tile_col, int &tile_row) {
    const int R = queue_rows(Q.tiles_y, qid);
    if (k >= static_cast<unsigned int>(R) * static_cast<unsigned int>(Q.tiles_x)) return false;
    if (Q.perm) k = Q.perm[static_cast<size_t>(qid) * Q.perm_stride + k];
    const unsigned int q = Q.tiles_x_magic ? __umulhi(k, Q.tiles_x_magic) : k;
    const int qi = static_cast<int>(q), mid = R >> 1;
    const int j = (qi & 1) ? mid - ((qi + 1) >> 1) : mid + (qi >> 1);
    tile_row = (qid / RM_SUBQ) + 8 * ((qid % RM_SUBQ) + RM_SUBQ * j);
    tile_col = static_cast<int>(k - q * static_cast<unsigned int>(Q.tiles_x));
    return true;
}
__device__ __forceinline__ unsigned int queue_slot_of(const TileQueue &Q, int qid, int tile_col, int tile_row) {
    const int R = queue_rows(Q.tiles_y, qid), mid = R >> 1;
    const int j = (tile_row >> 3) / RM_SUBQ;
    const int qi = j >= mid ? 2 * (j - mid) : 2 * (mid - j) - 1;
    return static_cast<unsigned int>(qi) * static_cast<unsigned int>(Q.tiles_x) + static_cast<unsigned int>(tile_col);
}

__device__ __forceinline__ bool pull_tile(const TileQueue &Q, int &home, int &tile_col, int &tile_row, int lane,
                                          unsigned int first_claim) {
    unsigned int k = static_cast<unsigned int>(__builtin_amdgcn_readfirstlane(static_cast<int>(first_claim)));
    if (queue_entry(Q, home, k, tile_col, tile_row)) return true;
    const unsigned int mine = static_cast<unsigned int>(queue_rows(Q.tiles_y, lane)) * static_cast<unsigned int>(Q.tiles_x);
    for (int attempt = 0; attempt < 4096; ++attempt) {
        const unsigned int head = __hip_atomic_load(&Q.counters[lane * RM_QSTRIDE], __ATOMIC_RELAXED, __HIP_MEMORY_SCOPE_AGENT);
        const unsigned long long avail = __ballot(head < mine);
        if (avail == 0) return false;
        const int h = (home + 1) & (RM_QUEUES - 1);
        const unsigned long long rot = h ? ((avail >> h) | (avail << (RM_QUEUES - h))) : avail;
        const int x = (h + __builtin_ctzll(rot)) & (RM_QUEUES - 1);
        k = 0;
        if (lane == 0) k = atomicAdd(&Q.counters[x * RM_QSTRIDE], 1u);
        k = static_cast<unsigned int>(__builtin_amdgcn_readfirstlane(static_cast<int>(k)));
        if (queue_entry(Q, x, k, tile_col, tile_row)) {
            home = x;
            return true;
        }
    }
    return false;
}

__device__ __forceinline__ RmRenderParams cold_params() {
#if __HIP_DEVICE_COMPILE__
    typedef const __attribute__((address_space(4))) RmRenderParams *KernArgs;
    KernArgs p = (KernArgs)__builtin_amdgcn_kernarg_segment_ptr();
    asm volatile("" : "+s"(p));
#ifdef RM_RTC_V2
    RmRenderParams r = *p;
    rm_v2_fix(r);
    return r;
#else
    return *p;
#endif
#else
    return RmRenderParams();
#endif
}

template <int ACCEL, bool LDS, bool UR = false, bool REL = false>
__device__ __forceinline__ void render_v2_body(const RmRenderParams &P) {
    extern __shared__ __align__(16) unsigned char smem[];
    __shared__ WaveDiag wave_diag[4];
    const int lane0 = threadIdx.x & 63;
    const int lane = lane0;
    const int wave = __builtin_amdgcn_readfirstlane(static_cast<int>(threadIdx.x >> 6));
    if (lane < 8) {
        wave_diag[wave].sdf[lane] = 0;
        wave_diag[wave].iters[lane] = 0;
        wave_diag[wave].mx[lane] = 0;
        wave_diag[wave].mn_inv[lane] = 0;
    }
#ifdef RM_STAMPS
    if (lane == 0 && P.stamps && blockIdx.x * 4 + wave < 8192) P.stamps[40 + 2 * 8192 + blockIdx.x * 4 + wave] = __builtin_amdgcn_s_memrealtime();
#endif

    if (ACCEL == 2 && P.rect_cull) {
        const float o[3] = {P.origin[0], P.origin[1], P.origin[2]};
        const float rot[9] = {P.rot[0], P.rot[1], P.rot[2], P.rot[3], P.rot[4], P.rot[5], P.rot[6], P.rot[7], P.rot[8]};
        for (int j = threadIdx.x; j < P.bvh_leaf_count && j < RM_RECT_CULL_MAX_LEAVES; j += blockDim.x) {
            const RmBvhNode nd = P.bvh[P.bvh_leaves[j]];
            P.leaf_rects[j] = rm_leaf_rect(nd.lo, nd.hi, o, rot, P.width, P.height);
        }
        if (!LDS) __syncthreads();
    }
    {
        const LdsLayout lay = lds_layout<ACCEL, LDS, REL>(P);
        if (LDS) {
            size_t off;
            if (ACCEL == 2) {
                off = lay.nodes;
                stage(smem, off, P.bvh, P.bvh_nodes);
                off = lay.prims;
                stage(smem, off, P.bvh_prims, P.bvh_prim_count);
                off = lay.cells;
                stage(smem, off, P.pq_cells, P.pq_cell_count);
                off = lay.list;
                stage(smem, off, P.pq_list, P.pq_list_count);
            } else if (ACCEL == 1) {
                off = lay.oct;
                stage(smem, off, P.oct, P.oct_nodes);
                off = lay.oct_prims;
                stage(smem, off, P.oct_prims, P.oct_prim_count);
            }
            off = lay.spheres;
            stage(smem, off, P.spheres, P.n_prims);
            off = lay.radii;
            stage(smem, off, P.radii, P.n_prims);
            if (ACCEL == 2) {
                off = lay.step;
                stage(smem, off, P.step_tab, P.step_box ? 3 * P.sb_stride : 0);
            }
            if (REL) {
                double *rel = reinterpret_cast<double *>(smem + lay.rel);
                for (int k = threadIdx.x; k < P.bvh_nodes * 6; k += blockDim.x) {
                    const int node = k / 6, c = k - node * 6;
                    const float v = c < 3 ? P.bvh[node].lo[c] : P.bvh[node].hi[c - 3];
                    rel[k] = static_cast<double>(v) - P.origin_d[c < 3 ? c : c - 3];
                }
            }
            __syncthreads();
        }
    }
    const int list_cap = P.list_cap;
    auto lane_now = []() {
        int l;
        asm volatile("v_mbcnt_lo_u32_b32 %0, -1, 0\n\tv_mbcnt_hi_u32_b32 %0, -1, %0" : "=v"(l));
        return l;
    };
    auto list_column = [&](const RmRenderParams &C) {
        const uint32_t end = C.lds_off[9];
        return reinterpret_cast<uint16_t *>(smem + end) + (static_cast<uint32_t>(wave) * static_cast<uint32_t>(C.list_cap)) * 64u + static_cast<uint32_t>(lane_now());
    };
    const int item_px = P.item_px;
    int home = (P.hw_xcd ? (__builtin_amdgcn_s_getreg(20 | (3 << 11)) & 7) : (static_cast<int>(blockIdx.x) & 7)) * RM_SUBQ +
               static_cast<int>((blockIdx.x >> 3) % RM_SUBQ);
    const int refill_at = P.refill_threshold;

    int tile_col = -1, tile_row = 0, qpos = item_px;
    bool no_more = false;
    unsigned int item_t0 = 0;

    enum : int { ST_PHASE = 7, ST_TRIP_SHIFT = 3, ST_TRIP_MASK = 127 << 3, ST_HAVECUR = 1 << 10, ST_PAR_SHIFT = 11, ST_PAR_MASK = 7 << 11,
                 ST_PIXEL = 1 << 14,
                 ST_LIVE_SHIFT = 15, ST_POS_SHIFT = 22, ST_OVF = 1 << 29, ST_LIST_MASK = (0x3FFF << 15) | (1 << 29) };
    Vec3f rd = {0.f, 0.f, -1.f};
    double inv0 = 0.0, inv1 = 0.0, inv2 = 0.0;
    double t = RM_MAX_DIST;
    double sA = 0.0, sB = 0.0;
    int sC = -1;
    uint32_t counters = 0;
    uint32_t pidx = 0;
    int st = PH_DONE;

    auto ray_of = [&](const RmRenderParams &C) {
        Ray r;
        r.d = rd;
        r.o = {C.origin[0], C.origin[1], C.origin[2]};
        r.od[0] = C.origin_d[0];
        r.od[1] = C.origin_d[1];
        r.od[2] = C.origin_d[2];
        return r;
    };
    auto inv_of = [&]() {
        RayInv ri;
        ri.inv[0] = inv0;
        ri.inv[1] = inv1;
        ri.inv[2] = inv2;
        ri.par[0] = (st & (1 << ST_PAR_SHIFT)) != 0;
        ri.par[1] = (st & (2 << ST_PAR_SHIFT)) != 0;
        ri.par[2] = (st & (4 << ST_PAR_SHIFT)) != 0;
        ri.any_par = (st & ST_PAR_MASK) != 0;
        return ri;
    };
    auto list_of = [&](const RmRenderParams &C) {
        RayList L;
        L.col = list_column(C);
        L.cap = list_cap;
        L.live = (st >> ST_LIVE_SHIFT) & 127;
        L.cur_pos = (st >> ST_POS_SHIFT) & 127;
        L.cnt = (st & ST_OVF) ? list_cap + 1 : L.live;
// ... 202 lines not shown
                        if (t < sA) skip = sA - t;
                        else if (t > sB) {
                            RayList L = list_of(CA);
                            Interval cur;
                            cur.tEnter = sA;
                            cur.tExit = sB;
                            cur.ord = sC;
                            const bool hc = bvh_next<REL>(S, ray, inv_of(), L, sA, sC, cur);
                            keep_list(L);
                            if (!hc) {
                                st &= ~ST_HAVECUR;
                                terminate = true;
                            } else {
                                sA = cur.tEnter;
                                sB = cur.tExit;
                                sC = cur.ord;
                                if (sA > t) skip = sA - t;
                            }
                        }
                    }
                    if (terminate) {
                        finish_march(RM_MAX_DIST);
                        break;
                    }
                    if (skip > 0.0) {
                        t += skip;
                        if (t > RM_MAX_DIST) {
                            finish_march(t);
                            break;
                        }
                        continue;
                    }
                } else if (ACCEL == 1) {
                    onode = oct_find(S, p);
                    if (onode >= 0) {
                        const double skip = oct_skip(S.oct[onode], ray, t);
                        if (skip > 0.0) {
                            t += skip;
                            if (t > RM_MAX_DIST) {
                                finish_march(t);
                                break;
                            }
                            continue;
                        }
                    }
                }
                q = p;
                need = true;
                break;
            }
        }
        bool n0_go = true;
        if (ACCEL == 2) n0_go = !__any(need) || __popcll(__ballot((st & ST_PHASE) == PH_N0)) >= CA.n0_batch;
        {
            const int ph = st & ST_PHASE;
            if (ph >= PH_N0 && ph <= PH_N3 && (ph != PH_N0 || n0_go)) {
                RM_CNT(14)
                q = point_at(ray, t);
                if (ph == PH_N1) q.x = to_f32(static_cast<double>(q.x) - 0.01);
                if (ph == PH_N2) q.y = to_f32(static_cast<double>(q.y) - 0.01);
                if (ph == PH_N3) q.z = to_f32(static_cast<double>(q.z) - 0.01);
                if (ACCEL == 1) onode = oct_find(S, q);
                need = true;
            }
        }
        RM_T(1)
        if (!__any(need)) continue;

        if (need) RM_CNT(6)
        const RmRenderParams CB = cold_params();
        const SceneView SB = scene_view<ACCEL, LDS, REL>(CB, smem);
        const bool coop = CB.coop != 0, filter = CB.filter != 0;
        const bool use_grid = ACCEL == 2 && CB.use_grid != 0;
        double dist;
        const int lane_b = lane_now();
        uint32_t evaluated = 0;
        NormalAux aux;
        aux.ok = false;
        aux.k1 = 0;
        aux.lb2 = 0.f;
        aux.found = 0;
        aux.rho = 0.f;
        aux.rho_cell = 0.f;
        if (ACCEL == 2) {
#ifdef RM_STAMPS
            unsigned long long fbc = 0;
            dist = bvh_distance_wave<UR>(CB, SB, need, q, evaluated, lane_b, coop, filter, use_grid, &fbc, &aux);
            t_acc_[4] += fbc;
            t_prev_ += fbc;
#else
            dist = bvh_distance_wave<UR>(CB, SB, need, q, evaluated, lane_b, coop, filter, use_grid, nullptr, &aux);
#endif
        }
        else if (ACCEL == 1) dist = need ? oct_distance_lane(SB, onode, q, evaluated, filter) : RM_MAX_DIST;
        else {
            dist = all_prims_wave(SB, need, q, lane_b, coop, filter);
            if (need) evaluated = static_cast<uint32_t>(SB.n_prims);
        }
        counters += evaluated << 16;

        RM_T(2)
        const bool fuse = ACCEL == 2 && need && (st & ST_PHASE) == PH_N0 && aux.ok && aux.rho > RM_NRM_DELTA;
        const bool was_marching = need && (st & ST_PHASE) == PH_MARCH;
        if (need) {
            const int ph = st & ST_PHASE;
            if (ph == PH_MARCH) {
                t += dist;
                counters += 1;
                if (dist < RM_EPSILON || t > RM_MAX_DIST) finish_march(t);
            } else if (ph == PH_N0) {
                sA = dist;
                set_phase(PH_N1);
            } else if (ph == PH_N1) {
                sB = __hiloint2double(__double2hiint(sB), __float_as_int(to_f32(sA - dist)));
                set_phase(PH_N2);
            } else if (ph == PH_N2) {
                sB = __hiloint2double(__float_as_int(to_f32(sA - dist)), __double2loint(sB));
                set_phase(PH_N3);
            } else {
                float nx = nrm_x(), ny = nrm_y(), nz = to_f32(sA - dist);
                normalize3(nx, ny, nz);
                set_normal(nx, ny, nz);
                set_phase(PH_DONE);
            }
        }
        if (ACCEL == 2 && CB.multi_step) {
            const bool go = was_marching && aux.ok && (aux.found >> 16) != 0xFFFFu && (st & ST_PHASE) == PH_MARCH;
            if (__any(go)) {
                if (go) {
                    const RmRenderParams CM = cold_params();
                    const SceneView SM = scene_view<ACCEL, LDS, REL>(CM, smem);
                    const RmSphere s1 = SM.spheres[aux.k1];
                    const double r1 = SM.radii[aux.k1];
                    const bool step_box = CM.step_box != 0;
                    float b_lo[3], b_hi[3];
                    if (step_box) {
                        const uint32_t *tab = LDS ? reinterpret_cast<const uint32_t *>(smem + CM.lds_off[10]) : CM.step_tab;
                        const int last = CM.sb_stride - (CM.sb_bins >> 2) - 2;
                        const float qk[3] = {q.x, q.y, q.z};
#pragma unroll
                        for (int k = 0; k < 3; ++k) {
                            const uint32_t *axis = tab + k * CM.sb_stride;
                            const int b = min(max(static_cast<int>((qk[k] - CM.sb_origin[k]) * CM.sb_inv[k]), 0), CM.sb_bins - 1);
                            int i = static_cast<int>(reinterpret_cast<const uint8_t *>(axis)[b]);
                            i = min(i, last);
                            const float *T = reinterpret_cast<const float *>(axis + (CM.sb_bins >> 2));
                            float lo = T[i], hi = T[i + 1];
                            while (hi <= qk[k] && i < last) {
                                i += 1;
                                lo = hi;
                                hi = T[i + 1];
                            }
                            b_lo[k] = lo;
                            b_hi[k] = hi;
                        }
                    }
                    for (;;) {
                        if ((st & ST_TRIP_MASK) >= (RM_MAX_STEPS << ST_TRIP_SHIFT)) {
                            finish_march(t);
                            break;
                        }
                        if (t < sA || t > sB) {
                            RM_CNT_END(2)
                            break;
                        }
                        const Vec3f p2 = point_at(ray, t);
                        if (step_box) {
                            if (!(p2.x >= b_lo[0] && p2.x < b_hi[0] && p2.y >= b_lo[1] && p2.y < b_hi[1] && p2.z >= b_lo[2] && p2.z < b_hi[2])) {
                                RM_CNT_END(0)
                                break;
                            }
                        } else {
                            const RmBvhNode root = SM.nodes[0];
                            bool same = box_margin(root.lo, root.hi, p2) >= 0.f;
                            uint32_t cell = 255u;
                            if (same) {
                                const float gx = (p2.x - CM.pq_origin[0]) * CM.pq_inv[0], gy = (p2.y - CM.pq_origin[1]) * CM.pq_inv[1], gz = (p2.z - CM.pq_origin[2]) * CM.pq_inv[2];
                                const int cx = min(max(static_cast<int>(gx), 0), CM.pq_dim[0] - 1);
                                const int cy = min(max(static_cast<int>(gy), 0), CM.pq_dim[1] - 1);
                                const int cz = min(max(static_cast<int>(gz), 0), CM.pq_dim[2] - 1);
                                cell = SM.pq_cells[(cz * CM.pq_dim[1] + cy) * CM.pq_dim[0] + cx];
                            }
                            const int ccnt = static_cast<int>(cell & 0xFFu);
                            if (ccnt == 255) {
                                RM_CNT_END(1)
                                break;
                            }
                            const uint16_t *lst = SM.pq_list + (cell >> 8);
                            uint32_t left = aux.found >> 16;
                            for (int k = 0; k < ccnt; ++k) {
                                const RmBvhNode node = SM.nodes[lst[k]];
                                if (box_margin(node.lo, node.hi, p2) >= 0.f) {
                                    same = same && box_margin(node.lo, node.hi, q) >= 0.f;
                                    left -= 1u;
                                }
                            }
                            if (!same || left != 0u) {
                                RM_CNT_END(0)
                                break;
                            }
                        }
                        const float ex = p2.x - q.x, ey = p2.y - q.y, ez = p2.z - q.z;
                        const float dd = __builtin_amdgcn_sqrtf(ex * ex + ey * ey + ez * ez) * 1.00001f + 1e-7f;
                        const double e = sphere_sdf_fast(s1, r1, p2);
                        if (!(aux.lb2 - dd > f32_upper_bound(e))) {
                            RM_CNT_END(3)
                            break;
                        }
                        RM_CNT(15)
                        st += 1 << ST_TRIP_SHIFT;
                        counters += (aux.found << 16) + 1u;
                        const double d2 = __builtin_fmin(e, RM_MAX_DIST);
                        t += d2;
                        if (d2 < RM_EPSILON || t > RM_MAX_DIST) {
                            finish_march(t);
                            break;
                        }
                    }
                }
            }
        }
        if (ACCEL == 2 && __any(fuse)) {
            if (fuse) {
                const SceneView SN = scene_view<ACCEL, LDS, REL>(cold_params(), smem);
                const RmSphere s1 = SN.spheres[aux.k1];
                const double r1 = SN.radii[aux.k1];
                Vec3f qx = q, qy = q, qz = q;
                qx.x = to_f32(static_cast<double>(q.x) - 0.01);
                qy.y = to_f32(static_cast<double>(q.y) - 0.01);
                qz.z = to_f32(static_cast<double>(q.z) - 0.01);
                const double e1 = sphere_sdf_fast(s1, r1, qx), e2 = sphere_sdf_fast(s1, r1, qy), e3 = sphere_sdf_fast(s1, r1, qz);
                const double emax = __builtin_fmax(__builtin_fmax(e1, e2), e3);
                if (aux.lb2 - RM_NRM_DELTA > f32_upper_bound(emax)) {
                    counters += (3u * aux.found) << 16;
                    float nx = to_f32(sA - __builtin_fmin(e1, RM_MAX_DIST));
                    float ny = to_f32(sA - __builtin_fmin(e2, RM_MAX_DIST));
                    float nz = to_f32(sA - __builtin_fmin(e3, RM_MAX_DIST));
                    normalize3(nx, ny, nz);
                    set_normal(nx, ny, nz);
                    set_phase(PH_DONE);
                }
            }
        }
        RM_T(3)
    }
    RM_TEND()
    {
        const RmRenderParams C = cold_params();
        if (C.diag_block) {
            const WaveDiag *w = &wave_diag[wave];
            unsigned long long ts = 0, ti = 0;
            unsigned int mx = 0, mi = 0;
#pragma unroll
            for (int k = 0; k < 8; ++k) {
                ts += w->sdf[k];
                ti += w->iters[k];
                mx = w->mx[k] > mx ? w->mx[k] : mx;
                mi = w->mn_inv[k] > mi ? w->mn_inv[k] : mi;
            }
            diag_flush_wave(C.diag_block, C.diag_out, C.tile_counters, ts, ti, mx, mi, blockIdx.x * 4u + static_cast<unsigned int>(wave),
                            gridDim.x * 4u, lane_now());
        }
    }
#ifdef RM_COUNTS
    __syncthreads();
    if (threadIdx.x < 32 && P.stamps) atomicAdd(&P.stamps[8 + threadIdx.x], static_cast<unsigned long long>(rm_cnt_s[threadIdx.x]));
    if (threadIdx.x < 8 && P.stamps) atomicAdd(&P.stamps[40 + threadIdx.x], static_cast<unsigned long long>(rm_cnt_e[threadIdx.x]));
#endif
}

#ifdef RM_RTC_V2
}
extern "C" __global__ __launch_bounds__(256, RM_V2_WAVES) void rm_rtc_render_v2(const RmRenderParams P) {
    render_v2_body<RM_RTC_V2_ACCEL, RM_RTC_V2_LDS != 0, RM_RTC_V2_UR != 0, RM_RTC_V2_REL != 0>(P);
}
#else
template <int ACCEL, bool LDS, bool UR = false, bool REL = false>
__global__ __launch_bounds__(256, RM_V2_WAVES) void render_kernel_v2(const RmRenderParams P) {
    render_v2_body<ACCEL, LDS, UR, REL>(P);
}

template <bool UR>
__global__ __launch_bounds__(256) void wave_distance_kernel(const RmRenderParams P, const float *pts, int64_t n, double *dist, uint32_t *count) {
    const int64_t i = static_cast<int64_t>(blockIdx.x) * 256 + threadIdx.x;
    const bool need = i < n;
    Vec3f q;
    q.x = need ? pts[3 * i] : 0.f;
    q.y = need ? pts[3 * i + 1] : 0.f;
    q.z = need ? pts[3 * i + 2] : 0.f;
    const SceneView S = scene_view<2, false, false>(P, nullptr);
    uint32_t c = 0;
    NormalAux aux;
    const double d = bvh_distance_wave<UR>(P, S, need, q, c, static_cast<int>(threadIdx.x & 63), P.coop != 0, P.filter != 0, P.use_grid != 0, nullptr, &aux);
    if (need) {
        dist[i] = d;
        count[i] = c;
    }
}

size_t scene_lds_bytes(const RmRenderParams &p) {
    auto up = [](size_t v) { return (v + 15) & ~static_cast<size_t>(15); };
    size_t b = 0;
    if (p.accel == 2) {
        b += up(static_cast<size_t>(p.bvh_nodes) * sizeof(RmBvhNode)) + up(static_cast<size_t>(p.bvh_prim_count) * 4);
        b += up(static_cast<size_t>(p.pq_cell_count) * 4) + up(static_cast<size_t>(p.pq_list_count) * 2 + 4);
    } else if (p.accel == 1) {
        b += up(static_cast<size_t>(p.oct_nodes) * sizeof(RmOctNode)) + up(static_cast<size_t>(p.oct_prim_count) * 4);
    }
    b += up(static_cast<size_t>(p.n_prims) * sizeof(RmSphere)) + up(static_cast<size_t>(p.n_prims) * 8);
    if (p.accel == 2 && p.step_box) b += up(static_cast<size_t>(3) * p.sb_stride * 4);
    return b + 16;
}

}

#ifndef RM_LENGTH_SQRT
RmV2Plan rm_v2_plan(const RmRenderParams &p_in) {
    RmRenderParams p = p_in;
    if (p.leaf_order) p.bvh_prim_count = 0;
    if (p.list_cap < 1) p.list_cap = 1;
    const bool want = p.accel == 2 && p.step_box != 0 && p.multi_step != 0 && p.sb_stride > 0;
    auto pass = [&](bool with_table) {
        RmRenderParams c = p;
        c.step_box = with_table ? 1 : 0;
        RmV2Plan r;
        r.step_box = c.step_box;
        r.list_cap = c.list_cap;
        r.list_bytes = c.accel == 2 ? static_cast<size_t>(4) * c.list_cap * 128 : 0;
        r.scene_bytes = scene_lds_bytes(c);
        r.lds = c.nodes_in_lds != 0 && r.scene_bytes + r.list_bytes + 16 <= 64 * 1024;
        r.rel = false;
        r.tier = 0;
        r.refused = 0;
        if (!(r.lds && c.accel == 2)) return r;
        const size_t rel_bytes = static_cast<size_t>(c.bvh_nodes) * 48;
        constexpr size_t kLdsPerCu = 160 * 1024, kGranule = 1280, kStatic = sizeof(WaveDiag) * 4;
        auto budget_for = [&](size_t bytes) { return bytes / kGranule * kGranule - kStatic; };
        auto fits = [&](size_t extra, int cap, size_t budget) { return r.scene_bytes + extra + static_cast<size_t>(4) * cap * 128 + 16 <= budget; };
        auto trim = [&](size_t extra, size_t budget) {
            int cap = c.list_cap;
            while (cap > 12 && !fits(extra, cap, budget)) cap -= 1;
            return fits(extra, cap, budget) ? cap : 0;
        };
        size_t budgets[4];
        int nb = 0;
        if (c.lds_budget_kb > 0) budgets[nb++] = budget_for(static_cast<size_t>(c.lds_budget_kb) * 1024);
        else {
            budgets[nb++] = budget_for(kLdsPerCu / RM_V2_WAVES);
            budgets[nb++] = budget_for(kLdsPerCu / 5);
        }
        budgets[nb++] = budget_for(kLdsPerCu / 4);
        r.tier = nb;
        for (int b = 0; b < nb; ++b) {
            int cap = c.rel_boxes ? trim(rel_bytes + 16, budgets[b]) : 0;
            if (cap > 0) r.rel = true;
            else cap = trim(0, budgets[b]);
            if (cap > 0) {
                r.list_cap = cap;
                r.list_bytes = static_cast<size_t>(4) * cap * 128;
                r.tier = b;
                break;
            }
            r.rel = false;
        }
        return r;
    };
    RmV2Plan plain = pass(false);
    if (!want) return plain;
    const RmV2Plan with_table = pass(true);
    if (with_table.lds == plain.lds && with_table.rel == plain.rel && with_table.tier <= plain.tier) return with_table;
    plain.refused = 1;
    return plain;
}
#endif

#ifndef RM_LENGTH_SQRT
namespace {
__global__ __launch_bounds__(1024) void lpt_sort_kernel(const uint8_t *cost_prev, uint16_t *perm, int stride, int tiles_x, int tiles_y) {
    extern __shared__ unsigned char lpt_smem[];
    const int x = blockIdx.x;
    const int R = queue_rows(tiles_y, x);
    const int n = R * tiles_x;
    uint8_t *cost = lpt_smem;
    unsigned int *cnt = reinterpret_cast<unsigned int *>(lpt_smem + ((stride + 15) & ~15));
    __shared__ unsigned int sum_s, nz_s, base_s[4];
    if (threadIdx.x == 0) sum_s = nz_s = 0;
    __syncthreads();
    unsigned int sum = 0, nz = 0;
    for (int e = threadIdx.x; e < n; e += 1024) {
        const uint8_t c = cost_prev ? cost_prev[static_cast<size_t>(x) * stride + e] : 0;
        cost[e] = c;
        sum += c;
        nz += c != 0;
    }
    atomicAdd(&sum_s, sum);
    atomicAdd(&nz_s, nz);
    __syncthreads();
    const float mean = nz_s ? static_cast<float>(sum_s) / static_cast<float>(nz_s) : 1e9f;
    auto cls = [&](uint8_t c) { const float f = c; return f >= 4.f * mean ? 0 : (f >= 2.f * mean ? 1 : (f >= 1.25f * mean ? 2 : 3)); };
    const int chunk = (n + 1023) / 1024, e0 = threadIdx.x * chunk, e1 = min(n, e0 + chunk);
    unsigned int mine[4] = {0, 0, 0, 0};
    for (int e = e0; e < e1; ++e) mine[cls(cost[e])]++;
    for (int c = 0; c < 4; ++c) cnt[c * 1024 + threadIdx.x] = mine[c];
    __syncthreads();
    if (threadIdx.x < 4) {
        unsigned int run = 0;
        for (int t = 0; t < 1024; ++t) {
            const unsigned int v = cnt[threadIdx.x * 1024 + t];
            cnt[threadIdx.x * 1024 + t] = run;
            run += v;
        }
        base_s[threadIdx.x] = run;
    }
    __syncthreads();
    unsigned int start[4], acc = 0;
    for (int c = 0; c < 4; ++c) {
        start[c] = acc + cnt[c * 1024 + threadIdx.x];
        acc += base_s[c];
    }
    for (int e = e0; e < e1; ++e) {
        const int c = cls(cost[e]);
        perm[static_cast<size_t>(x) * stride + start[c]++] = static_cast<uint16_t>(e);
    }
}
}
hipError_t rm_launch_lpt_sort(const uint8_t *cost_prev, uint16_t *perm, int stride, int tiles_x, int tiles_y, hipStream_t stream) {
    const size_t shmem = static_cast<size_t>((stride + 15) & ~15) + 4 * 1024 * sizeof(unsigned int);
    hipLaunchKernelGGL(lpt_sort_kernel, dim3(RM_QUEUES), dim3(1024), shmem, stream, cost_prev, perm, stride, tiles_x, tiles_y);
    return hipGetLastError();
}
#endif

hipError_t RM_LEN_VARIANT(rm_launch_wave_distance)(const RmRenderParams &p, const float *points, int64_t n, double *dist, uint32_t *count, hipStream_t stream) {
    if (p.accel != 2 || p.general || p.bvh_nodes <= 0) return hipErrorInvalidValue;
    if (n <= 0) return hipSuccess;
    const dim3 grid(static_cast<unsigned>((n + 255) / 256)), block(256);
    if (p.uniform_radius) hipLaunchKernelGGL(wave_distance_kernel<true>, grid, block, 0, stream, p, points, n, dist, count);
    else hipLaunchKernelGGL(wave_distance_kernel<false>, grid, block, 0, stream, p, points, n, dist, count);
    return hipGetLastError();
}

hipError_t RM_LEN_VARIANT(rm_launch_render_v2)(const RmRenderParams &p_in, hipStream_t stream, const char **kernel_name, uint32_t *shape) {
    RmRenderParams p = p_in;
    const int rows = p.local_rows;
    if (kernel_name) *kernel_name = "";
    if (rows <= 0 || p.width <= 0) return hipSuccess;
    if (!p.tile_counters) return hipErrorInvalidValue;
    if (p.leaf_order) p.bvh_prim_count = 0;
    if (p.item_px != 64 && p.item_px != 128 && p.item_px != 256) p.item_px = 64;
    if (p.item_px < p.tile_w) p.item_px = p.tile_w;
    const int tw = p.tile_w;
    const bool wide = p.item_wide != 0 && tw < 64 && p.item_px > 64;
    const int iw = wide ? tw * (p.item_px / 64) : tw, th = wide ? 64 / tw : p.item_px / tw;
    const int tiles_x = (p.width + iw - 1) / iw;
    const int tiles_y = (rows + th - 1) / th;
    auto log2i = [](int v) { int l = 0; while ((1 << l) < v) ++l; return l; };
    if ((tw & (tw - 1)) != 0 || tiles_x <= 0 || static_cast<long long>(tiles_x) * (tiles_y + 8) >= (1ll << 31)) return hipErrorInvalidValue;
    p.tile_w_log2 = log2i(tw);
    p.tile_h_log2 = log2i(th);
    p.item_w_log2 = log2i(iw);
    p.sub_dx = wide ? tw : 0;
    p.sub_dy = wide ? 0 : 64 / tw;
    p.tiles_x = tiles_x;
    p.tiles_y = tiles_y;
    p.tiles_x_magic = tiles_x == 1 ? 0u : static_cast<uint32_t>((1ull << 32) / static_cast<unsigned long long>(tiles_x)) + 1u;
    const unsigned needed = static_cast<unsigned>((static_cast<long long>(tiles_x) * tiles_y + 3) / 4);
    unsigned resident = 0, blocks = 0;
    if (p.refill_threshold < 1) p.refill_threshold = 1;
    if (p.refill_threshold > 64) p.refill_threshold = 64;
    const RmV2Plan plan = rm_v2_plan(p);
    const bool lds = plan.lds, rel = plan.rel;
    p.list_cap = plan.list_cap;
    p.step_box = plan.step_box;
    if (p.accel != 2 || !p.leaf_rects || !p.bvh_leaves || p.bvh_leaf_count <= 0 || p.bvh_leaf_count > RM_RECT_CULL_MAX_LEAVES ||
        p.width > 65536 || p.height > 65536)
        p.rect_cull = 0;
    const size_t list_bytes = plan.list_bytes, scene_bytes = plan.scene_bytes, rel_bytes = static_cast<size_t>(p.bvh_nodes) * 48;
    size_t shmem = (lds ? scene_bytes : 0) + (rel ? rel_bytes + 16 : 0) + list_bytes + 16;
    if (p.lds_fill && p.blocks_per_cu >= 2 && p.blocks_per_cu <= 8) {
        const size_t room = (160 * 1024 / static_cast<size_t>(p.blocks_per_cu)) / 1280 * 1280 - sizeof(WaveDiag) * 4;
        if (room > shmem && room <= 64 * 1024) shmem = room;
    }
    {
        const LdsLayout lay = lds_layout_host(p, p.accel, lds, rel && p.accel == 2);
        const uint32_t v[11] = {lay.nodes, lay.prims, lay.cells, lay.list, lay.oct, lay.oct_prims, lay.spheres, lay.radii, lay.rel, lay.end, lay.step};
        for (int k = 0; k < 11; ++k) p.lds_off[k] = v[k];
        if (lay.end + list_bytes > shmem) return hipErrorInvalidValue;
    }
    const int cus = p.num_cus > 0 ? p.num_cus : 256;
    const int floor_per_cu = p.launch_per_cu > 0 ? p.launch_per_cu : p.blocks_per_cu;
    const int per_cu = rm_v2_overlap_per_cu(floor_per_cu, p.overlap_per_cu, static_cast<long long>(tiles_x) * tiles_y, cus);
    resident = static_cast<unsigned>(cus) * static_cast<unsigned>(per_cu > 0 ? per_cu : 4);
    blocks = needed < resident ? (needed ? needed : 1u) : resident;
    if (shape) {
        shape[0] = blocks;
        shape[1] = 256;
        shape[2] = static_cast<uint32_t>(shmem);
        shape[3] = p.step_box ? 1u : 0u;
        shape[4] = p.rect_cull ? 1u : 0u;
    }
    hipError_t e = hipSuccess;
    if (!p.diag_block) e = hipMemsetAsync(p.tile_counters, 0, RM_QUEUES * RM_QSTRIDE * sizeof(unsigned int), stream);
    if (e != hipSuccess) return e;
    p.lpt_perm = nullptr;
    if (p.lpt_perm_out) {
        const long long per_queue = static_cast<long long>(queue_rows_host(tiles_y, 0)) * tiles_x;
        if (per_queue <= p.lpt_stride && per_queue <= 32768) {
            e = rm_launch_lpt_sort(p.lpt_cost_prev, p.lpt_perm_out, p.lpt_stride, tiles_x, tiles_y, stream);
            if (e != hipSuccess) return e;
            p.lpt_perm = p.lpt_perm_out;
        } else {
            p.lpt_cost_out = nullptr;
        }
    } else {
        p.lpt_cost_out = nullptr;
    }
    const dim3 grid(blocks), block(256);
#define RM_V2X(A, L, U, R)                                                                                                   \
    {                                                                                                                        \
        const void *fn_ = p.rtc_ctx ? rm_rtc_v2_hook(p, A, L, U, R, RM_LEN_IS_SQRT) : nullptr;                               \
        if (fn_) {                                                                                                           \
            size_t bytes_ = sizeof p;                                                                                        \
            void *extra_[] = {HIP_LAUNCH_PARAM_BUFFER_POINTER, &p, HIP_LAUNCH_PARAM_BUFFER_SIZE, &bytes_, HIP_LAUNCH_PARAM_END}; \
            e = hipModuleLaunchKernel(reinterpret_cast<hipFunction_t>(const_cast<void *>(fn_)), grid.x, 1, 1, 256, 1, 1,     \
                                      static_cast<unsigned>(shmem), stream, nullptr, extra_);                               \
            if (e != hipSuccess) return e;                                                                                   \
            if (kernel_name) *kernel_name = "render_kernel_v2<" #A ", " #L ", " #U ", " #R ">" RM_LEN_TAG " [launch constants compiled in]"; \
        } else {                                                                                                             \
            hipLaunchKernelGGL((render_kernel_v2<A, L, U, R>), grid, block, shmem, stream, p);                               \
            if (kernel_name) *kernel_name = "render_kernel_v2<" #A ", " #L ", " #U ", " #R ">" RM_LEN_TAG;                   \
        }                                                                                                                    \
    }
#define RM_V2(A, L) RM_V2X(A, L, false, false)
    if (p.accel == 2) {
        if (lds && rel && p.uniform_radius) RM_V2X(2, true, true, true)
        else if (lds && rel) RM_V2X(2, true, false, true)
        else if (lds && p.uniform_radius) RM_V2X(2, true, true, false)
        else if (lds) RM_V2(2, true)
        else RM_V2(2, false)
    }
    else if (p.accel == 1) { if (lds) RM_V2(1, true) else RM_V2(1, false) }
    else { if (lds) RM_V2(0, true) else RM_V2(0, false) }
#undef RM_V2X
#undef RM_V2
    return hipGetLastError();
}
#endif
```

cpu_raymarcher_amd/csrc/rm_scene_host.cpp:

```cpp
#include "rm_scene_host.h"

#include <algorithm>
#include <cmath>
#include <cstring>
#include <limits>
#include <numeric>

namespace rmh {

namespace {

inline float to_f32(double v) { return static_cast<float>(v); }


struct Mat4 {
    float m[16];
    static Mat4 identity() {
        Mat4 r;
        for (int i = 0; i < 16; ++i) r.m[i] = (i % 5 == 0) ? 1.0f : 0.0f;
        return r;
    }
};

Mat4 rotate_y(const Mat4 &a, double rad) {
    const double s = std::sin(rad), c = std::cos(rad);
    Mat4 r = a;
    for (int k = 0; k < 4; ++k) {
        const double row0 = a.m[k], row2 = a.m[8 + k];
        r.m[k] = to_f32(row0 * c - row2 * s);
        r.m[8 + k] = to_f32(row0 * s + row2 * c);
    }
    return r;
}

Mat4 rotate_x(const Mat4 &a, double rad) {
    const double s = std::sin(rad), c = std::cos(rad);
    Mat4 r = a;
    for (int k = 0; k < 4; ++k) {
        const double row1 = a.m[4 + k], row2 = a.m[8 + k];
        r.m[4 + k] = to_f32(row1 * c + row2 * s);
        r.m[8 + k] = to_f32(row2 * c - row1 * s);
    }
    return r;
}

Mat4 translate(const Mat4 &a, const float v[3]) {
    Mat4 r = a;
    const double x = v[0], y = v[1], z = v[2];
    for (int k = 0; k < 4; ++k)
        r.m[12 + k] = to_f32(double(a.m[k]) * x + double(a.m[4 + k]) * y + double(a.m[8 + k]) * z +
                             double(a.m[12 + k]));
    return r;
}

inline double js_min2(double a, double b) {
    if (a == 0.0 && b == 0.0) return std::signbit(a) ? a : b;
    return a < b ? a : b;
}
inline double js_max2(double a, double b) {
    if (a == 0.0 && b == 0.0) return std::signbit(a) ? b : a;
    return a > b ? a : b;
}

struct Box {
    float lo[3], hi[3];
};

inline bool boxes_touch(const Box &a, const float *blo, const float *bhi) {
    for (int k = 0; k < 3; ++k)
        if (!(a.lo[k] <= bhi[k] && a.hi[k] >= blo[k])) return false;
    return true;
}

double box_gap(const Box &a, const float *blo, const float *bhi) {
    double g[3];
    for (int k = 0; k < 3; ++k) {
        g[k] = 0.0;
        if (a.hi[k] < blo[k]) g[k] = double(blo[k]) - double(a.hi[k]);
        else if (bhi[k] < a.lo[k]) g[k] = double(a.lo[k]) - double(bhi[k]);
    }
    return js_hypot3(g[0], g[1], g[2]);
}

Box bounds_of(const HostScene &s, const int32_t *ids, int n) {
    Box b;
    if (n == 0) {
        std::memset(&b, 0, sizeof b);
        return b;
// ... 132 lines not shown
    for (int z = 0; z < s.nn_dim[2]; ++z)
        for (int y = 0; y < s.nn_dim[1]; ++y)
            for (int x = 0; x < s.nn_dim[0]; ++x) {
                const int ci[3] = {x, y, z};
                double lo[3], hi[3];
                for (int k = 0; k < 3; ++k) {
                    const double w = s.nn_inv[k] > 0 ? 1.0 / double(s.nn_inv[k]) : 0.0;
                    lo[k] = double(s.pq_origin[k]) + (ci[k] - 0.03) * w;
                    hi[k] = double(s.pq_origin[k]) + (ci[k] + 1.03) * w;
                }
                double U = 10.0;
                for (size_t j = 0; j < n; ++j) {
                    const double c[3] = {s.spheres[j].cx, s.spheres[j].cy, s.spheres[j].cz};
                    double dmin2 = 0, dmax2 = 0;
                    for (int k = 0; k < 3; ++k) {
                        const double below = lo[k] - c[k], above = c[k] - hi[k];
                        const double dmin = below > 0 ? below : (above > 0 ? above : 0.0);
                        const double dmax = std::max(std::fabs(c[k] - lo[k]), std::fabs(c[k] - hi[k]));
                        dmin2 += dmin * dmin;
                        dmax2 += dmax * dmax;
                    }
                    lb[j] = std::sqrt(dmin2) - s.radii[j];
                    const double ub = std::sqrt(dmax2) - s.radii[j];
                    if (ub < U) U = ub;
                }
                std::vector<uint16_t> cand;
                for (size_t j = 0; j < n; ++j)
                    if (lb[j] <= U + margin) cand.push_back(static_cast<uint16_t>(j));
                const size_t c_idx = (static_cast<size_t>(z) * s.nn_dim[1] + y) * s.nn_dim[0] + x;
                if (cand.size() >= 255 || s.nn_list.size() + cand.size() >= (1u << 24)) continue;
                s.nn_cells[c_idx] = static_cast<uint32_t>(s.nn_list.size() << 8) | static_cast<uint32_t>(cand.size());
                s.nn_list.insert(s.nn_list.end(), cand.begin(), cand.end());
            }
}

void build_step_box(HostScene &s) {
    s.step_tab.clear();
    s.sb_bins = s.sb_stride = 0;
    if (s.general || s.program || s.bvh.empty() || s.bvh_leaves == 0) return;
    std::vector<float> T[3];
    for (size_t i = 0; i < s.bvh.size(); ++i) {
        const RmBvhNode &nd = s.bvh[i];
        if (i != 0 && (nd.leaf < 0 || (nd.leaf & 0xFF) == 0)) continue;
        for (int k = 0; k < 3; ++k) {
            for (const float v : {nd.lo[k], nd.hi[k]})
                if (!std::isfinite(v) || (v != 0.0f && std::fabs(v) < 1e-30f)) return;
            T[k].push_back(nd.lo[k]);
            T[k].push_back(std::nextafter(nd.hi[k], std::numeric_limits<float>::infinity()));
        }
    }
    size_t longest = 0;
    for (int k = 0; k < 3; ++k) {
        std::sort(T[k].begin(), T[k].end());
        T[k].erase(std::unique(T[k].begin(), T[k].end()), T[k].end());
        if (T[k].size() > static_cast<size_t>(kStepBoxCap)) return;
        longest = std::max(longest, T[k].size());
    }
    const float inf = std::numeric_limits<float>::infinity();
    s.sb_bins = kStepBoxBins;
    s.sb_stride = kStepBoxBins / 4 + static_cast<int>(longest) + 2;
    s.step_tab.assign(3 * static_cast<size_t>(s.sb_stride), 0);
    for (int k = 0; k < 3; ++k) {
        const RmBvhNode &root = s.bvh[0];
        const double ext = double(root.hi[k]) - double(root.lo[k]);
        s.sb_origin[k] = root.lo[k];
        s.sb_inv[k] = ext > 0 ? static_cast<float>(kStepBoxBins / ext) : 0.0f;
        if (!std::isfinite(s.sb_inv[k])) s.sb_inv[k] = 0.0f;
        uint32_t *axis = s.step_tab.data() + static_cast<size_t>(k) * s.sb_stride;
        std::vector<float> th(static_cast<size_t>(longest) + 2, inf);
        th[0] = -inf;
        std::copy(T[k].begin(), T[k].end(), th.begin() + 1);
        std::memcpy(axis + kStepBoxBins / 4, th.data(), th.size() * sizeof(float));
        uint8_t *bins = reinterpret_cast<uint8_t *>(axis);
        const double w = s.sb_inv[k] > 0 ? 1.0 / double(s.sb_inv[k]) : 0.0;
        for (int b = 0; b < kStepBoxBins; ++b) {
            size_t i = 0;
            if (b > 0 && w > 0) {
                const double edge = double(s.sb_origin[k]) + (b - 0.01) * w;
                while (i < T[k].size() && double(T[k][i]) <= edge) ++i;
            }
            bins[b] = static_cast<uint8_t>(i);
        }
    }
}

void build_exterior_grid(HostScene &s, const PairLoops *loops) {
    const double kExtReach = 8.7;
    if (s.general || s.program || s.bvh.empty()) return;
    const size_t n = s.spheres.size();
    if (n < 16 || n > 2048) return;
    int g = 32;
    while (g > 8 && static_cast<unsigned long long>(g) * g * g * n > 40000000ull) g -= 4;
    bool covered = true;
    double w[3], lo3[3], hi3[3];
    for (int k = 0; k < 3; ++k) {
        covered = covered && double(s.root_min[k]) <= -kExtReach && double(s.root_max[k]) >= kExtReach;
        lo3[k] = std::min(double(s.root_min[k]) - 0.5, -kExtReach);
        hi3[k] = std::max(double(s.root_max[k]) + 0.5, kExtReach);
        if (!std::isfinite(lo3[k]) || !std::isfinite(hi3[k]) || !(hi3[k] > lo3[k])) return;
    }
    if (covered) return;
    for (int k = 0; k < 3; ++k) {
        s.ext_origin[k] = static_cast<float>(lo3[k]);
        s.ext_inv[k] = static_cast<float>(g / (hi3[k] - lo3[k]));
        w[k] = 1.0 / double(s.ext_inv[k]);
    }
    s.ext_dim[0] = s.ext_dim[1] = s.ext_dim[2] = g;
    s.ext_cells.assign(static_cast<size_t>(g) * g * g, 255);
    if (loops && loops->ext_grid && loops->ext_grid(s)) return;
    const double margin = 1e-6;
    std::vector<double> lb(n);
    auto candidates = [&](const double lo[3], const double hi[3], const std::vector<uint16_t> &from, std::vector<uint16_t> &out) {
        double U = 10.0;
        for (size_t e = 0; e < from.size(); ++e) {
            const size_t j = from[e];
            const double c[3] = {s.spheres[j].cx, s.spheres[j].cy, s.spheres[j].cz};
            double dmin2 = 0, dmax2 = 0;
            for (int k = 0; k < 3; ++k) {
                const double below = lo[k] - c[k], above = c[k] - hi[k];
                const double dmin = below > 0 ? below : (above > 0 ? above : 0.0);
                const double dmax = std::max(std::fabs(c[k] - lo[k]), std::fabs(c[k] - hi[k]));
                dmin2 += dmin * dmin;
                dmax2 += dmax * dmax;
            }
            lb[e] = std::sqrt(dmin2) - s.radii[j];
            const double ub = std::sqrt(dmax2) - s.radii[j];
            if (ub < U) U = ub;
        }
        out.clear();
        for (size_t e = 0; e < from.size(); ++e)
            if (lb[e] <= U + margin) out.push_back(from[e]);
    };
    std::vector<uint16_t> all(n), block, cand;
    std::iota(all.begin(), all.end(), static_cast<uint16_t>(0));
    const int B = 4;
    for (int bz = 0; bz < g; bz += B)
        for (int by = 0; by < g; by += B)
            for (int bx = 0; bx < g; bx += B) {
                const int b0[3] = {bx, by, bz};
                double lo[3], hi[3];
                for (int k = 0; k < 3; ++k) {
                    lo[k] = double(s.ext_origin[k]) + (b0[k] - 0.03) * w[k];
                    hi[k] = double(s.ext_origin[k]) + (b0[k] + B - 1 + 1.03) * w[k];
                }
                candidates(lo, hi, all, block);
                for (int z = bz; z < bz + B; ++z)
                    for (int y = by; y < by + B; ++y)
                        for (int x = bx; x < bx + B; ++x) {
                            const int ci[3] = {x, y, z};
                            bool inside = true;
                            for (int k = 0; k < 3; ++k) {
                                lo[k] = double(s.ext_origin[k]) + (ci[k] - 0.03) * w[k];
                                hi[k] = double(s.ext_origin[k]) + (ci[k] + 1.03) * w[k];
                                inside = inside && lo[k] >= double(s.root_min[k]) && hi[k] <= double(s.root_max[k]);
                            }
                            if (inside) continue;
                            candidates(lo, hi, block, cand);
                            if (cand.size() >= 255 || s.ext_list.size() + cand.size() >= (1u << 24)) continue;
                            const size_t c_idx = (static_cast<size_t>(z) * g + y) * g + x;
                            s.ext_cells[c_idx] = static_cast<uint32_t>(s.ext_list.size() << 8) | static_cast<uint32_t>(cand.size());
                            s.ext_list.insert(s.ext_list.end(), cand.begin(), cand.end());
                        }
            }
}


// ... 268 lines not shown
                                U = std::min(U, std::sqrt(dmax2) - s.radii[id]);
                            }
                            const size_t first = s.oct_sub_list.size();
                            uint32_t cnt = 0;
                            for (int j = 0; j < n; ++j)
                                if (lb[j] <= U + margin) {
                                    s.oct_sub_list.push_back(static_cast<uint8_t>(j));
                                    ++cnt;
                                }
                            s.oct_sub_hdr.push_back(static_cast<uint32_t>(first << 8) | cnt);
                        }
            }
        }
        if (!s.general) {
            s.oct_recs.resize(s.oct_prims.size());
            for (size_t k = 0; k < s.oct_prims.size(); ++k) {
                const int id = s.oct_prims[k];
                const RmSphere &sp = s.spheres[id];
                s.oct_recs[k] = RmSphereRec{sp.cx, sp.cy, sp.cz, sp.rf, s.radii[id], id, 0};
            }
        }
        std::memcpy(s.root_min, root.lo, sizeof root.lo);
        std::memcpy(s.root_max, root.hi, sizeof root.hi);
    }
    return true;
}

bool build_scene(HostScene &s, const float *centers, const double *radii, int n, int accel,
                 std::string &err, const PairLoops *loops) {
    if (n < 0 || (n > 0 && (!centers || !radii))) {
        err = "bad sphere list";
        return false;
    }
    for (int i = 0; i < n; ++i) {
        if (!std::isfinite(centers[3 * i]) || !std::isfinite(centers[3 * i + 1]) ||
            !std::isfinite(centers[3 * i + 2]) || !std::isfinite(radii[i])) {
            err = "non-finite sphere centre or radius";
            return false;
        }
    }
    s = HostScene();
    s.accel = (accel == 1 || accel == 2) ? accel : 0;
    s.spheres.resize(n);
    s.radii.assign(radii, radii + n);
    s.prim_lo.resize(3 * size_t(n));
    s.prim_hi.resize(3 * size_t(n));
    for (int i = 0; i < n; ++i) {
        s.spheres[i] = RmSphere{centers[3 * i], centers[3 * i + 1], centers[3 * i + 2], to_f32(radii[i])};
        const double scale = js_max2(js_max2(js_hypot3(1, 0, 0), js_hypot3(0, 1, 0)), js_hypot3(0, 0, 1));
        const double pad = radii[i] * scale * 1.5;
        for (int k = 0; k < 3; ++k) {
            s.prim_lo[3 * i + k] = to_f32(double(centers[3 * i + k]) - pad);
            s.prim_hi[3 * i + k] = to_f32(double(centers[3 * i + k]) + pad);
        }
    }
    s.world_pos.assign(centers, centers + 3 * size_t(n));
    if (!build_accel(s, n, err, loops)) return false;
    if (s.accel == 2 && s.bvh_prims.size() == size_t(n) && n > 0) {
        std::vector<RmSphere> sp(n);
        std::vector<double> rd(n);
        std::vector<int32_t> pos(n, -1), obj(n);
        bool perm = true;
        for (int k = 0; k < n; ++k) {
            const int id = s.bvh_prims[k];
            if (id < 0 || id >= n || pos[id] >= 0) {
                perm = false;
                break;
            }
            pos[id] = k;
            obj[k] = id;
            sp[k] = s.spheres[id];
            rd[k] = s.radii[id];
        }
        if (perm) {
            s.spheres.swap(sp);
            s.radii.swap(rd);
            std::iota(s.bvh_prims.begin(), s.bvh_prims.end(), 0);
            for (uint16_t &e : s.nn_list) e = static_cast<uint16_t>(pos[e]);
            for (uint16_t &e : s.ext_list) e = static_cast<uint16_t>(pos[e]);
            s.leaf_order = true;
            s.slot_object.swap(obj);
        }
    }
    return true;
}


namespace {

bool invert4(const float a[16], float out[16]) {
    const double a00 = a[0], a01 = a[1], a02 = a[2], a03 = a[3], a10 = a[4], a11 = a[5], a12 = a[6], a13 = a[7];
    const double a20 = a[8], a21 = a[9], a22 = a[10], a23 = a[11], a30 = a[12], a31 = a[13], a32 = a[14], a33 = a[15];
    const double b00 = a00 * a11 - a01 * a10, b01 = a00 * a12 - a02 * a10, b02 = a00 * a13 - a03 * a10;
    const double b03 = a01 * a12 - a02 * a11, b04 = a01 * a13 - a03 * a11, b05 = a02 * a13 - a03 * a12;
    const double b06 = a20 * a31 - a21 * a30, b07 = a20 * a32 - a22 * a30, b08 = a20 * a33 - a23 * a30;
    const double b09 = a21 * a32 - a22 * a31, b10 = a21 * a33 - a23 * a31, b11 = a22 * a33 - a23 * a32;
    double det = b00 * b11 - b01 * b10 + b02 * b09 + b03 * b08 - b04 * b07 + b05 * b06;
    if (!(det != 0.0)) return false;
    det = 1.0 / det;
    float o[16];
    o[0] = to_f32((a11 * b11 - a12 * b10 + a13 * b09) * det);
    o[1] = to_f32((a02 * b10 - a01 * b11 - a03 * b09) * det);
    o[2] = to_f32((a31 * b05 - a32 * b04 + a33 * b03) * det);
    o[3] = to_f32((a22 * b04 - a21 * b05 - a23 * b03) * det);
    o[4] = to_f32((a12 * b08 - a10 * b11 - a13 * b07) * det);
    o[5] = to_f32((a00 * b11 - a02 * b08 + a03 * b07) * det);
    o[6] = to_f32((a32 * b02 - a30 * b05 - a33 * b01) * det);
    o[7] = to_f32((a20 * b05 - a22 * b02 + a23 * b01) * det);
    o[8] = to_f32((a10 * b10 - a11 * b08 + a13 * b06) * det);
    o[9] = to_f32((a01 * b08 - a00 * b10 - a03 * b06) * det);
    o[10] = to_f32((a30 * b04 - a31 * b02 + a33 * b00) * det);
    o[11] = to_f32((a21 * b02 - a20 * b04 - a23 * b00) * det);
    o[12] = to_f32((a11 * b07 - a10 * b09 - a12 * b06) * det);
    o[13] = to_f32((a00 * b09 - a01 * b07 + a02 * b06) * det);
    o[14] = to_f32((a31 * b01 - a30 * b03 - a32 * b00) * det);
    o[15] = to_f32((a20 * b03 - a21 * b01 + a22 * b00) * det);
    std::memcpy(out, o, sizeof o);
    return true;
}

Mat4 rotate_z(const Mat4 &a, double rad) {
    const double s = std::sin(rad), c = std::cos(rad);
    Mat4 r = a;
    for (int k = 0; k < 4; ++k) {
        const double row0 = a.m[k], row1 = a.m[4 + k];
        r.m[k] = to_f32(row0 * c + row1 * s);
        r.m[4 + k] = to_f32(row1 * c - row0 * s);
    }
    return r;
}

}

void make_transform(double x, double y, double z, const float *rot, float out16[16]) {
    Mat4 model = Mat4::identity();
    model.m[12] = to_f32(x);
    model.m[13] = to_f32(y);
    model.m[14] = to_f32(z);
    if (rot) model = rotate_z(rotate_y(rotate_x(model, rot[0]), rot[1]), rot[2]);
    Mat4 inv = Mat4::identity();
    invert4(model.m, inv.m);
    std::memcpy(out16, inv.m, sizeof inv.m);
}

bool preset_prims(int index, std::vector<PrimDesc> &out) {
    out.clear();
    index = std::max(0, std::min(index, kPresetCount - 1));
    auto add = [&](int type, double x, double y, double z, const float *rot, double p0, double p1, double p2) {
        PrimDesc d;
        d.type = type;
        make_transform(x, y, z, rot, d.m);
        d.params[0] = p0;
        d.params[1] = p1;
        d.params[2] = p2;
        out.push_back(d);
    };
    if (index <= 4) {
        std::vector<float> c;
        std::vector<double> r;
        preset_spheres(index, c, r);
        for (size_t i = 0; i < r.size(); ++i) add(0, c[3 * i], c[3 * i + 1], c[3 * i + 2], nullptr, r[i], 0, 0);
        return true;
    }
    switch (index) {
        case 5: {
            const float rot[3] = {to_f32(-3.141592653589793 / 2), 0.0f, 0.0f};
// ... 505 lines not shown
```

cpu_raymarcher_amd/csrc/rm_scene_host.h:

```cpp
#pragma once
#include <functional>
#include <string>
#include <vector>

#include "rm_types.h"

namespace rmh {

constexpr int kPresetCount = 19;
constexpr int kStepBoxCap = 62;
constexpr int kStepBoxBins = 32;

struct PrimDesc {
    int type = 0;
    float m[16];
    double params[3];
};

struct NodeDesc {
    int type = 0;
    int a = -1, b = -1;
    float m[16];
    double params[6];
};

struct ProgTreeNode {
    int pre = -1, main = -1, a = -1, b = -1;
};

struct HostScene {
    int accel = 0;
    int preset = 0;
    bool general = false;
    bool program = false;
    int prog_slots = 1, prog_vals = 1;
    std::vector<RmInstr> prog;
    std::vector<int32_t> obj_ranges;
    std::vector<ProgTreeNode> prog_tree;
    std::vector<int32_t> prog_roots;
    std::vector<RmPrim> prims;
    std::vector<float> world_pos;
    bool leaf_order = false;
    std::vector<int32_t> slot_object;
    std::vector<RmSphere> spheres;
    std::vector<double> radii;
    std::vector<float> prim_lo, prim_hi;
    std::vector<RmBvhNode> bvh;
    std::vector<int32_t> bvh_prims;
    int bvh_leaves = 0, bvh_depth = 0;
    int pq_dim[3] = {0, 0, 0};
    float pq_origin[3] = {0, 0, 0}, pq_inv[3] = {0, 0, 0};
    std::vector<uint32_t> pq_cells;
    std::vector<uint16_t> pq_list;
    int nn_dim[3] = {0, 0, 0};
    float nn_inv[3] = {0, 0, 0};
    std::vector<uint32_t> nn_cells;
    std::vector<uint16_t> nn_list;
    int ext_dim[3] = {0, 0, 0};
    float ext_origin[3] = {0, 0, 0}, ext_inv[3] = {0, 0, 0};
    std::vector<uint32_t> ext_cells;
    std::vector<uint16_t> ext_list;
    int sb_bins = 0, sb_stride = 0;
    float sb_origin[3] = {0, 0, 0}, sb_inv[3] = {0, 0, 0};
    std::vector<uint32_t> step_tab;
    std::vector<RmOctNode> oct;
    std::vector<int32_t> oct_prims;
    std::vector<RmSphereRec> oct_recs;
    std::vector<int32_t> oct_lut;
    std::vector<uint32_t> oct_sub_hdr;
    std::vector<uint8_t> oct_sub_list;
    bool prim_filter_ok = true;
    int oct_leaves = 0, oct_empty = 0, oct_max_leaf = 0;
    float root_min[3] = {0, 0, 0}, root_max[3] = {0, 0, 0};
};

double js_hypot3(double x, double y, double z);
void set_length_mode(int use_sqrt);
double vec3_length_host(double x, double y, double z);

bool preset_spheres(int index, std::vector<float> &centers, std::vector<double> &radii);

struct PairLoops {
    std::function<bool(HostScene &s)> nn_grid;
    std::function<bool(HostScene &s)> ext_grid;
    std::function<bool(HostScene &s, const std::vector<int32_t> &leaves)> oct_sub;
    std::function<bool(const HostScene &s, const std::vector<int32_t> &nodes, std::vector<double> &out)> empty_dist;
};

bool build_scene(HostScene &s, const float *centers, const double *radii, int n, int accel,
                 std::string &err, const PairLoops *loops = nullptr);

void make_transform(double x, double y, double z, const float *rot, float out16[16]);

bool preset_prims(int index, std::vector<PrimDesc> &out);

bool build_scene_general(HostScene &s, const PrimDesc *prims, int n, int accel, std::string &err);

bool preset_nodes(int index, std::vector<NodeDesc> &nodes, std::vector<int> &roots);

bool build_scene_nodes(HostScene &s, const NodeDesc *nodes, int n_nodes, const int *roots, int n_roots, int accel,
                       std::string &err);

bool leaf_objects(const HostScene &s, std::vector<RmInstr> &prog, std::vector<int32_t> &obj_ranges, std::vector<ProgTreeNode> &tree,
                  std::vector<int32_t> &roots);

void scale_transform(float m[16], double x, double y, double z);

void camera_from_angles(double pitch, double yaw, float rot9[9], float origin3[3]);
double clamp_pitch(double pitch);

void phong_light_dir(float out[3]);

}
```

cpu_raymarcher_amd/csrc/rm_types.h:

```cpp
#pragma once
#ifndef __HIPCC_RTC__
#include <stdint.h>
#else
using __hip_internal::int8_t;
using __hip_internal::int16_t;
using __hip_internal::int32_t;
using __hip_internal::int64_t;
using __hip_internal::uint8_t;
using __hip_internal::uint16_t;
using __hip_internal::uint32_t;
using __hip_internal::uint64_t;
#endif

struct RmBvhNode {
    float lo[3];
    int32_t skip;
    float hi[3];
    int32_t leaf;
};

struct RmOctNode {
    float lo[3];
    int32_t first_child;
    float hi[3];
// ... 28 lines not shown
struct RmPrim {
    float m[16];
    int32_t type;
    float half[3];
    double a, b;
};

struct RmInstr {
    float T[16];
    float Tinv[16];
    double p[6];
    int32_t op, src, dst;
    int32_t flags;
};
#define RM_PROG_MAX_SLOTS 16
#define RM_PROG_MAX_VALS 16

#define RM_BVH_LEAF_MAX 255
#define RM_MAX_STEPS 100
#define RM_MAX_DIST 10.0
#define RM_EPSILON 0.001

struct RmDiagBlock;
struct RmFrameDiagBlock;
struct RmDiagDevice;

struct RmFrameView {
    float rot[9];
    float origin[3];
    double origin_d[3];
    double time;
};

#define RM_V2_WAVES 6

struct alignas(8) RmLeafRect {
    uint16_t x_lo, x_hi, y_lo, y_hi;
};
#define RM_RECT_CULL_MAX_LEAVES 256

struct RmRenderParams {
    int32_t width, height, y_start, y_end;
    float rot[9];
    float origin[3];
    float light[3];
    double rot_d[9], origin_d[3], light_d[3];
    int32_t n_prims;
    int32_t accel;
    int32_t shader;
    int32_t bvh_nodes;
    int32_t oct_nodes;
    int32_t tile_w;
    int32_t nodes_in_lds;
    int32_t filter;
    int32_t variant;
    int32_t list_cap;
    int32_t coop;
    int32_t bvh_prim_count;
    int32_t oct_prim_count;
    int32_t blocks_per_cu;
    int32_t num_cus;
    int32_t pq_dim[3];
    int32_t pq_cell_count;
    int32_t pq_list_count;
    int32_t use_grid;
    float pq_origin[3];
    float pq_inv[3];
    float pq_cell[3];
    int32_t refill_threshold;
    int32_t hw_xcd;
    int32_t item_px;
    int32_t local_rows;
    int32_t stripe_rows;
    int32_t n_parts, part;
    int32_t rel_boxes;
    const uint16_t *lpt_perm;
    uint8_t *lpt_cost_out;
    const uint8_t *lpt_cost_prev;
    uint16_t *lpt_perm_out;
    int32_t lpt_stride;
    int32_t launch_per_cu;
    int32_t v1_lists;
    int32_t v1_list_offset;
    uint32_t lds_off[11];
    int32_t prim_filter;
    int32_t n0_batch;
    const int32_t *stripe_ids;
    unsigned int *tile_counters;
    unsigned long long *stamps;
    const uint32_t *pq_cells;
    const uint16_t *pq_list;
    const uint16_t *bvh_leaves;
    int32_t bvh_leaf_count;
    int32_t v1_block;
    int32_t oct_lean;
    const uint32_t *nn_cells;
    const uint16_t *nn_list;
    int32_t nn_cell_count, nn_list_count, use_nn;
    int32_t tile_w_log2, tile_h_log2, tiles_x, tiles_y;
    int32_t item_wide, item_w_log2, sub_dx, sub_dy;
    const void *rtc_function;
    void *rtc_ctx;
    uint32_t tiles_x_magic;
    int32_t lds_budget_kb;
    int32_t leaf_order;
    int32_t nn_dim[3];
    float nn_inv[3];
    int32_t overlap_per_cu;
    const uint32_t *ext_cells;
    const uint16_t *ext_list;
    int32_t ext_dim[3];
    float ext_origin[3], ext_inv[3];
    int32_t use_ext;
    int32_t algorithm;
    int32_t general;
    int32_t uniform_radius;
    const RmPrim *prims;
    const RmInstr *prog;
    const int32_t *obj_ranges;
    int32_t prog_slots, prog_vals;
    double time;
    double overshoot;
    double step_size;
    const RmSphere *spheres;
    const double *radii;
    const RmBvhNode *bvh;
    const int32_t *bvh_prims;
    const RmOctNode *oct;
    const int32_t *oct_prims;
    const RmSphereRec *oct_recs;
    const int32_t *oct_lut;
    const RmOctFrameNode *oct_frame;
    const uint32_t *oct_sub_hdr;
    const uint8_t *oct_sub_list;
    uint8_t *depth;
    uint8_t *normal;
    uint16_t *sdf;
    uint16_t *iters;
    uint8_t *rgba;
    int32_t lds_fill;
    int32_t multi_step;
    RmDiagBlock *diag_block;
    RmDiagDevice *diag_out;
    const uint32_t *step_tab;
    float sb_origin[3], sb_inv[3];
    int32_t sb_bins, sb_stride;
    int32_t step_box;
    RmLeafRect *leaf_rects;
    int32_t rect_cull;
};
```

cpu_raymarcher_amd/csrc/rm_v2_fields.h:

```cpp
#pragma once

#define RM_V2_FIXED_SCALARS(X)                                                                                                  \
    X(width) X(height) X(accel) X(shader) X(tile_w) X(nodes_in_lds) X(filter) X(variant) X(list_cap) X(coop) X(use_grid)         \
    X(refill_threshold) X(hw_xcd) X(item_px) X(rel_boxes) X(lpt_stride) X(prim_filter) X(n0_batch) X(use_nn) X(tile_w_log2)     \
    X(tile_h_log2) X(tiles_x) X(item_wide) X(item_w_log2) X(sub_dx) X(sub_dy) X(tiles_x_magic) X(leaf_order) X(algorithm)       \
    X(general) X(uniform_radius) X(multi_step) X(use_ext) X(step_box) X(sb_bins) X(sb_stride) X(rect_cull)

#define RM_V2_FIXED_COUNTS(X)                                                                                                    \
    X(n_prims) X(bvh_nodes) X(oct_nodes) X(bvh_prim_count) X(oct_prim_count) X(pq_cell_count) X(pq_list_count) X(bvh_leaf_count) \
    X(nn_cell_count) X(nn_list_count)

#define RM_V2_FIXED_ARRAYS(X) \
    X(pq_dim, 3) X(lds_off, 11) X(nn_dim, 3) X(pq_origin, 3) X(pq_inv, 3) X(pq_cell, 3) X(nn_inv, 3) X(light, 3) X(light_d, 3) \
    X(ext_dim, 3) X(ext_origin, 3) X(ext_inv, 3) X(sb_origin, 3) X(sb_inv, 3)
```

include/rm_raymarch.h:

```cpp
#ifndef RM_RAYMARCH_H
#define RM_RAYMARCH_H

#include <stddef.h>
#include <stdint.h>

#ifdef __cplusplus
extern "C" {
#endif

#define RM_API __attribute__((visibility("default")))

typedef struct rm_ctx rm_ctx;

typedef enum rm_status {
    RM_OK = 0,
    RM_E_INVALID = -1,
    RM_E_UNSUPPORTED = -2,
    RM_E_NO_DEVICE = -3,
    RM_E_HIP = -4,
    RM_E_NO_SCENE = -5,
    RM_E_NOMEM = -6
} rm_status;

typedef enum rm_accel { RM_ACCEL_NONE = 0, RM_ACCEL_OCTREE = 1, RM_ACCEL_BVH = 2 } rm_accel;
// ... 312 lines not shown
                                  void *d_rgba, void *stream);
RM_API int rm_shade_ranged(rm_ctx *ctx, int32_t counter, int32_t width, int32_t rows, int32_t n_frames,
                           const uint16_t *values, const rm_frame_hist *hist, uint32_t lo, uint32_t hi,
                           uint8_t *rgba);

RM_API int rm_shade_lit_device(rm_ctx *ctx, int32_t width, int32_t rows, int32_t n_frames, const void *d_depth,
                               const void *d_normal, const void *d_lit, const void *d_ao, void *d_rgba, void *stream);
RM_API int rm_shade_lit(rm_ctx *ctx, int32_t width, int32_t rows, int32_t n_frames, const uint8_t *depth,
                        const uint8_t *normal, const float *lit, const float *ao, uint8_t *rgba);

typedef enum rm_field_map { RM_FIELD_MAP_DISTANCE = 0, RM_FIELD_MAP_COUNT = 1 } rm_field_map;
typedef struct rm_field_shade {
    int32_t  map, reserved;
    double   range;
    double   band;
    double   line;
    uint32_t lo, hi;
} rm_field_shade;
RM_API int rm_shade_field_device(rm_ctx *ctx, const rm_field_shade *shade, int64_t n, const void *d_values, void *d_rgba,
                                 void *stream);
RM_API int rm_shade_field(rm_ctx *ctx, const rm_field_shade *shade, int64_t n, const void *values, uint8_t *rgba);

RM_API int rm_render_stripes_device(rm_ctx *ctx, const rm_job *job, int32_t shader, int32_t stripe_rows,
                                    int32_t n_parts, int32_t part, void *d_depth, void *d_normal,
                                    void *d_sdf, void *d_iters, void *d_rgba, void *stream);
RM_API int rm_stripe_rows(int32_t y_start, int32_t y_end, int32_t stripe_rows, int32_t n_parts, int32_t part);

RM_API int rm_deal_stripes(int32_t rows, int32_t stripe_rows, int32_t n_parts, const int32_t *weights, int32_t *owner);

RM_API int rm_render_stripe_list_device(rm_ctx *ctx, const rm_job *job, int32_t shader, int32_t stripe_rows,
                                        const int32_t *stripe_ids, int32_t n_stripes, void *d_depth, void *d_normal,
                                        void *d_sdf, void *d_iters, void *d_rgba, void *stream);

RM_API int rm_assemble_frame_device(rm_ctx *ctx, const void *d_gathered, int64_t rank_stride, int64_t section_offset,
                                    int32_t row_bytes, int32_t height, int32_t stripe_rows, const int32_t *owner,
                                    int32_t n_stripes, int32_t world, void *d_frame, int64_t acc_offset, void *d_acc,
                                    void *stream);

RM_API int rm_shade(rm_ctx *ctx, int32_t shader, int32_t width, int32_t height,
                    const uint8_t *depth, const uint8_t *normal, const uint16_t *sdf,
                    const uint16_t *iters, uint8_t *rgba);
RM_API int rm_shade_device(rm_ctx *ctx, int32_t shader, int32_t width, int32_t height,
                           const void *d_depth, const void *d_normal, const void *d_sdf,
                           const void *d_iters, void *d_rgba, void *stream);

RM_API int rm_reduce_counters(rm_ctx *ctx, const uint16_t *sdf, const uint16_t *iters, int64_t n,
                              rm_diagnostics *out);
RM_API int rm_reduce_counters_device(rm_ctx *ctx, const void *d_sdf, const void *d_iters, int64_t n,
                                     rm_diagnostics *out, void *stream);

RM_API int rm_reduce_counters_enqueue(rm_ctx *ctx, const void *d_sdf, const void *d_iters, int64_t n,
                                      void *d_acc, void *stream);

RM_API int rm_render_attach_diagnostics(rm_ctx *ctx, void *d_acc);


RM_API int rm_partition_rows(int32_t height, int32_t n_workers, int32_t i, int32_t *y_start,
                             int32_t *y_end);


RM_API int rm_selftest_hypot(rm_ctx *ctx, const float *xyz, int64_t n, double *out);

RM_API int rm_selftest_jsmath(rm_ctx *ctx, int32_t fn, const double *a, const double *b, int64_t n, double *out);

RM_API int rm_selftest_hypot64(rm_ctx *ctx, const double *xyz, int64_t n, int32_t on_device, double *out);

RM_API int rm_selftest_fastdiv(rm_ctx *ctx, uint64_t seed, int64_t n, uint64_t *mismatches);

RM_API int rm_selftest_recip(rm_ctx *ctx, int mode, uint64_t *mismatches);

RM_API int rm_debug_read_stamps(rm_ctx *ctx, uint64_t *out8);

RM_API int rm_rtc_source(rm_ctx *ctx, char *out, int64_t cap, int64_t *needed);
RM_API int rm_rtc_compile_check(rm_ctx *ctx, int32_t accel, int32_t other, char *log, int64_t cap, double *seconds);
RM_API int rm_rtc_status(rm_ctx *ctx, int32_t *compiled, int32_t *failed, char *log, int64_t cap);

RM_API int rm_debug_read_counts(rm_ctx *ctx, uint64_t *out32);
RM_API int rm_debug_read_lpt_costs(rm_ctx *ctx, uint8_t *out, int64_t n);
RM_API int rm_debug_scene_table(rm_ctx *ctx, const char *name, int32_t from_device, void *out, int64_t cap, int64_t *bytes);
RM_API int rm_debug_launch_fill(rm_ctx *ctx, int32_t asked, int32_t *effective);
RM_API int rm_debug_last_launch(rm_ctx *ctx, uint32_t out[4]);
RM_API int rm_debug_overlap_fill(rm_ctx *ctx, int32_t asked, int64_t items, int32_t *effective);
RM_API int rm_debug_step_box(rm_ctx *ctx, int32_t out[6]);
RM_API int rm_debug_rect_cull(rm_ctx *ctx, const float *rot9, const float *origin3, int32_t width, int32_t height, int32_t out[5]);
RM_API int rm_debug_leaf_rects(rm_ctx *ctx, const float *rot9, const float *origin3, int32_t width, int32_t height,
                               uint16_t *rects, int32_t *nodes, int64_t cap, int64_t *n);
RM_API int rm_debug_read_wave_times(rm_ctx *ctx, uint64_t *out24576);
RM_API int rm_debug_read_batch_log(rm_ctx *ctx, uint32_t *out196608);

RM_API int rm_set_option(rm_ctx *ctx, const char *key, int64_t value);
RM_API int rm_get_option(const rm_ctx *ctx, const char *key, int64_t *value);

#ifdef __cplusplus
}
#endif
#endif
```

Before: 1706.

## Add precomputed per-cell candidate table for BVH sphere-trace lookups

Builds a host-side cell table on the step-box grid that maps each cell to a merged box record holding a deduplicated candidate sphere list. In the v2 BVH kernel this table replaces the grid-plus-tree walk, so each query becomes three axis lookups and one record read, and the step box comes directly from the record bounds. The table is staged in LDS in place of the pq cells and lists. This trades more LDS and host build time for fewer divergent BVH traversals per SDF evaluation.

```diff
diff --git a/cpu_raymarcher_amd/_native.py b/cpu_raymarcher_amd/_native.py
--- a/cpu_raymarcher_amd/_native.py
+++ b/cpu_raymarcher_amd/_native.py
@@ -154,7 +154,7 @@
 SCENE_TABLES = {"spheres": "<f4", "radii": "<f8", "bvh": "u1", "bvh_prims": "<i4", "oct": "u1", "oct_prims": "<i4",
                 "pq_cells": "<u4", "pq_list": "<u2", "nn_cells": "<u4", "nn_list": "<u2", "prims": "u1", "prog": "u1",
                 "obj_ranges": "<i4", "oct_recs": "u1", "oct_lut": "<i4", "oct_sub_hdr": "<u4", "oct_sub_list": "u1",
-                "slot_object": "<i4", "ext_cells": "<u4", "ext_list": "<u2", "step_tab": "<u4"}
+                "slot_object": "<i4", "ext_cells": "<u4", "ext_list": "<u2", "step_tab": "<u4", "cell_tab": "<u4"}
 STEP_BOX_BINS, STEP_BOX_CAP = 32, 62
 
 
@@ -253,6 +253,7 @@
     "rm_debug_last_launch": (C.c_int, [_VP, C.POINTER(C.c_uint32)]),
     "rm_debug_overlap_fill": (C.c_int, [_VP, C.c_int32, C.c_int64, C.POINTER(C.c_int32)]),
     "rm_debug_step_box": (C.c_int, [_VP, C.POINTER(C.c_int32)]),
+    "rm_debug_cell_tab": (C.c_int, [_VP, C.POINTER(C.c_int32)]),
     "rm_debug_rect_cull": (C.c_int, [_VP, _VP, _VP, C.c_int32, C.c_int32, C.POINTER(C.c_int32)]),
     "rm_debug_leaf_rects": (C.c_int, [_VP, _VP, _VP, C.c_int32, C.c_int32, _VP, _VP, C.c_int64, C.POINTER(C.c_int64)]),
     "rm_rtc_source": (C.c_int, [_VP, C.c_char_p, C.c_int64, C.POINTER(C.c_int64)]),
diff --git a/cpu_raymarcher_amd/context.py b/cpu_raymarcher_amd/context.py
--- a/cpu_raymarcher_amd/context.py
+++ b/cpu_raymarcher_amd/context.py
@@ -159,6 +159,12 @@
         out = (C.c_int32 * 6)()
         N.check(self._h, N.lib().rm_debug_step_box(self._h, out))
         return dict(last=bool(out[0]), planned=bool(out[1]), reason=out[2], list_cap=out[3], list_cap_without=out[4], table_bytes=out[5])
+
+    def cell_tab(self):
+        out = (C.c_int32 * 12)()
+        N.check(self._h, N.lib().rm_debug_cell_tab(self._h, out))
+        return dict(last=bool(out[0]), planned=bool(out[1]), reason=out[2], list_cap=out[3], list_cap_without=out[4], table_bytes=out[5],
+                    per_cu=out[6], scene_bytes=out[7], scene_bytes_without=out[8], cells=out[9], records=out[10], leaf_sets=out[11])
 
     def rect_cull(self, rot, origin, width, height):
         r = np.ascontiguousarray(rot, dtype=np.float32).reshape(9)
diff --git a/cpu_raymarcher_amd/csrc/rm_api.cpp b/cpu_raymarcher_amd/csrc/rm_api.cpp
--- a/cpu_raymarcher_amd/csrc/rm_api.cpp
+++ b/cpu_raymarcher_amd/csrc/rm_api.cpp
@@ -27,7 +27,7 @@
 #define RM_SCENE_ARRAYS(X)                                                                                                        \
     X(spheres, 1) X(radii, 1) X(bvh, 1) X(bvh_prims, 1) X(oct, 1) X(oct_prims, 1) X(pq_cells, 1) X(pq_list, 1) X(nn_cells, 1)      \
     X(nn_list, 1) X(prims, 1) X(prog, 1) X(obj_ranges, 1) X(oct_recs, 1) X(oct_lut, 1) X(oct_sub_hdr, 1) X(oct_sub_list, 1)       \
-    X(slot_object, 0) X(ext_cells, 1) X(ext_list, 1) X(step_tab, 1)
+    X(slot_object, 0) X(ext_cells, 1) X(ext_list, 1) X(step_tab, 1) X(cell_tab, 1)
 
 struct DeviceScene {
 #define RM_X(name, always) decltype(rmh::HostScene::name)::value_type *name = nullptr;
@@ -366,10 +366,11 @@
     int64_t opt_min_fill = 1;
     int64_t opt_overlap_fill = 1;
     int hw_queues = 4;
-    uint32_t last_v2_shape[5] = {0, 0, 0, 0, 0};
+    uint32_t last_v2_shape[6] = {0, 0, 0, 0, 0, 0};
     int64_t opt_item_wide = 0;
     int64_t opt_multi_step = 1;
     int64_t opt_step_box = 1;
+    int64_t opt_cell_tab = 1;
     int64_t opt_lds_kb = 0;
     int64_t opt_refill = 64;
     int64_t opt_recs = 1;
@@ -1103,6 +1104,12 @@
     }
     p.step_box = (ctx->opt_step_box && ctx->opt_multi_step && ctx->host.accel == RM_ACCEL_BVH && !ctx->host.step_tab.empty() &&
                   (ctx->dev.step_tab || !ctx->has_device)) ? 1 : 0;
+    p.cell_tab = ctx->dev.cell_tab;
+    p.ct_rec_off = ctx->host.ct_rec_off;
+    p.ct_list_off = ctx->host.ct_list_off;
+    p.ct_words = static_cast<int32_t>(ctx->host.cell_tab.size());
+    for (int k = 0; k < 3; ++k) p.ct_dim[k] = ctx->host.ct_dim[k];
+    p.cell_on = (ctx->opt_cell_tab && p.step_box && !ctx->host.cell_tab.empty() && (ctx->dev.cell_tab || !ctx->has_device)) ? 1 : 0;
     p.uniform_radius = 0;
     if (ctx->opt_uniform && !ctx->host.general && ctx->host.spheres.size() >= 2 &&
         ctx->host.spheres.size() <= 256) {
@@ -3025,6 +3032,45 @@
     return RM_OK;
 }
 
+int rm_debug_cell_tab(rm_ctx *ctx, int32_t out[12]) {
+    if (!ctx || !out) return RM_E_INVALID;
+    for (int k = 0; k < 12; ++k) out[k] = 0;
+    out[0] = static_cast<int32_t>(ctx->last_v2_shape[5]);
+    if (!ctx->have_scene) return fail(ctx, RM_E_NO_SCENE, "no scene set");
+    rm_job job;
+    std::memset(&job, 0, sizeof job);
+    job.width = job.height = job.y_end = 64;
+    job.algorithm = RM_ALG_SPHERE_TRACER;
+    job.scene_preset_index = ctx->scene_is_uploaded ? RM_SCENE_UPLOADED : ctx->scene_preset;
+    job.acceleration_structure = ctx->host.accel;
+    job.overshoot_factor = job.step_size = std::nan("");
+    const double scene_time = ctx->time;
+    RmRenderParams p;
+    const int rc = fill_params(ctx, &job, p);
+    ctx->time = scene_time;
+    if (rc) return rc;
+    const auto &tab = ctx->host.cell_tab;
+    out[5] = static_cast<int32_t>(tab.size() * sizeof(uint32_t));
+    if (!tab.empty()) {
+        out[9] = static_cast<int32_t>(tab[0] * tab[1] * tab[2]);
+        out[10] = static_cast<int32_t>(tab[3]);
+        out[11] = static_cast<int32_t>(tab[7]);
+    }
+    RmRenderParams plain = p;
+    plain.cell_on = 0;
+    const RmV2Plan without = rm_v2_plan(plain);
+    out[4] = without.list_cap;
+    out[8] = static_cast<int32_t>(without.lds ? without.scene_bytes : 0);
+    const RmV2Plan plan = rm_v2_plan(p);
+    out[3] = plan.list_cap;
+    out[6] = plan.per_cu;
+    out[7] = static_cast<int32_t>(plan.lds ? plan.scene_bytes : 0);
+    const bool v2 = p.variant == 2 && p.algorithm == 0 && p.accel == 2;
+    out[1] = v2 && plan.cell_on ? 1 : 0;
+    out[2] = out[1] ? 0 : (tab.empty() && v2 && ctx->opt_cell_tab && ctx->opt_step_box && ctx->opt_multi_step ? 2 : (v2 && plan.cell_refused ? 3 : 1));
+    return RM_OK;
+}
+
 int rm_debug_rect_cull(rm_ctx *ctx, const float *rot9, const float *origin3, int32_t width, int32_t height, int32_t out[5]) {
     if (!ctx || !out || !rot9 || !origin3) return RM_E_INVALID;
     for (int k = 0; k < 5; ++k) out[k] = 0;
@@ -3099,6 +3145,7 @@
     {"lds_kb", &rm_ctx::opt_lds_kb, kZeroOrRange, {16, 64}, "lds_kb must be 0 (auto) or in [16, 64]"},
     {"multi_step", &rm_ctx::opt_multi_step, kSwitch, {}, nullptr},
     {"step_box", &rm_ctx::opt_step_box, kSwitch, {}, nullptr},
+    {"cell_tab", &rm_ctx::opt_cell_tab, kSwitch, {}, nullptr},
     {"item_wide", &rm_ctx::opt_item_wide, kSwitch, {}, nullptr},
     {"prune", &rm_ctx::opt_prune, kSwitch, {}, nullptr},
     {"rtc_spheres", &rm_ctx::opt_rtc_spheres, kRange, {0, 33}, "rtc_spheres must be 0..33"},
diff --git a/cpu_raymarcher_amd/csrc/rm_kernels.h b/cpu_raymarcher_amd/csrc/rm_kernels.h
--- a/cpu_raymarcher_amd/csrc/rm_kernels.h
+++ b/cpu_raymarcher_amd/csrc/rm_kernels.h
@@ -271,7 +271,8 @@
 
 struct RmV2Plan {
     bool lds, rel;
-    int list_cap, step_box, tier, refused;
+    int list_cap, step_box, tier, refused, cell_on, cell_refused;
+    int per_cu;
     size_t scene_bytes, list_bytes;
 };
 RmV2Plan rm_v2_plan(const RmRenderParams &p);
diff --git a/cpu_raymarcher_amd/csrc/rm_render_v2.hip b/cpu_raymarcher_amd/csrc/rm_render_v2.hip
--- a/cpu_raymarcher_amd/csrc/rm_render_v2.hip
+++ b/cpu_raymarcher_amd/csrc/rm_render_v2.hip
@@ -222,11 +222,11 @@
             const int cy = min(max(static_cast<int>((q.y - P.pq_origin[1]) * P.pq_inv[1]), 0), P.pq_dim[1] - 1);
             const int cz = min(max(static_cast<int>((q.z - P.pq_origin[2]) * P.pq_inv[2]), 0), P.pq_dim[2] - 1);
             in_root = true;
-            const uint32_t cell = S.pq_cells[(cz * P.pq_dim[1] + cy) * P.pq_dim[0] + cx];
+            const uint32_t cell = P.pq_cells[(cz * P.pq_dim[1] + cy) * P.pq_dim[0] + cx];
             const int ccnt = static_cast<int>(cell & 0xFFu);
             if (ccnt == 255) walk_tree = true;
             else {
-                const uint16_t *lst = S.pq_list + (cell >> 8);
+                const uint16_t *lst = P.pq_list + (cell >> 8);
                 for (int e = 0; e < ccnt; ++e) {
                     const RmBvhNode node = S.nodes[lst[e]];
                     if (!box_contains(node.lo, node.hi, q)) continue;
@@ -335,10 +335,25 @@
     return __builtin_fminf(a, b);
 }
 
+struct CellTabView {
+    const uint32_t *tab;
+    const uint32_t *step;
+    bool on;
+};
+__device__ __forceinline__ int cell_axis_index(const RmRenderParams &P, const uint32_t *step, int k, float x) {
+    const uint32_t *axis = step + k * P.sb_stride;
+    const int last = P.ct_dim[k] - 1;
+    const int b = min(max(static_cast<int>((x - P.sb_origin[k]) * P.sb_inv[k]), 0), P.sb_bins - 1);
+    int i = min(static_cast<int>(reinterpret_cast<const uint8_t *>(axis)[b]), last);
+    const float *T = reinterpret_cast<const float *>(axis + (P.sb_bins >> 2));
+    while (i < last && T[i + 1] <= x) i += 1;
+    return i;
+}
+
 template <bool UR>
 __device__ double bvh_distance_wave(const RmRenderParams &P, const SceneView &S, bool need, const Vec3f &q,
                                     uint32_t &count, int lane, bool coop, bool filter, bool use_grid,
-                                    unsigned long long *dbg_fallback_cycles, NormalAux *aux) {
+                                    unsigned long long *dbg_fallback_cycles, NormalAux *aux, const CellTabView CT) {
     aux->ok = false;
     aux->rho = 0.f;
     aux->rho_cell = 0.f;
@@ -363,7 +378,25 @@
         }
         found += static_cast<uint32_t>(cnt);
     };
-    if (need && use_grid) {
+    if (CT.on) {
+        if (need) {
+            const int ix = cell_axis_index(P, CT.step, 0, q.x), iy = cell_axis_index(P, CT.step, 1, q.y), iz = cell_axis_index(P, CT.step, 2, q.z);
+            const uint32_t r = reinterpret_cast<const uint16_t *>(CT.tab + 8)[(iz * P.ct_dim[1] + iy) * P.ct_dim[0] + ix];
+            const uint32_t *rec = CT.tab + P.ct_rec_off + 3u * r;
+            const uint32_t w0 = rec[0], w1 = rec[1], w2 = rec[2];
+            in_root = (w0 >> 24) != 0u;
+            const int cnt = static_cast<int>(w1 >> 24);
+            const uint16_t *lst = reinterpret_cast<const uint16_t *>(CT.tab + P.ct_list_off) + (w2 & 0xFFFFu);
+            for (int e = 0; e < cnt; ++e) {
+                const int id = lst[e];
+                RM_CNT(8)
+                scan_sphere<UR>(bs, S.spheres[id], id, q);
+            }
+            found = w2 >> 16;
+            nleaf16 = r << 16;
+            rho = 0.f;
+        }
+    } else if (need && use_grid) {
         const RmBvhNode root = S.nodes[0];
         const float m_root = box_margin(root.lo, root.hi, q);
         if (m_root >= 0.f) {
@@ -399,7 +432,7 @@
             }
         }
     }
-    if (need && (!use_grid || walk_tree)) {
+    if (need && !CT.on && (!use_grid || walk_tree)) {
         rho = 0.f;
         int i = 0;
         const int n = S.bvh_nodes;
@@ -648,12 +681,12 @@
 
 
 struct LdsLayout {
-    uint32_t nodes, prims, cells, list, oct, oct_prims, spheres, radii, rel, end, step;
+    uint32_t nodes, prims, cells, list, oct, oct_prims, spheres, radii, rel, end, step, ctab;
 };
 inline LdsLayout lds_layout_host(const RmRenderParams &C, int accel, bool lds, bool rel) {
     auto up = [](uint32_t v) { return (v + 15u) & ~15u; };
     auto words = [](uint32_t count, uint32_t size) { return ((count * size + 3u) / 4u) * 4u; };
-    LdsLayout o = {0, 0, 0, 0, 0, 0, 0, 0, 0, 0, 0};
+    LdsLayout o = {0, 0, 0, 0, 0, 0, 0, 0, 0, 0, 0, 0};
     uint32_t off = 0;
     if (lds) {
         if (accel == 2) {
@@ -662,9 +695,13 @@
             o.prims = off = up(off);
             off += words(static_cast<uint32_t>(C.bvh_prim_count), 4);
             o.cells = off = up(off);
-            off += words(static_cast<uint32_t>(C.pq_cell_count), 4);
+            off += words(static_cast<uint32_t>(C.cell_on ? 0 : C.pq_cell_count), 4);
             o.list = off = up(off);
-            off += words(static_cast<uint32_t>(C.pq_list_count), 2);
+            off += words(static_cast<uint32_t>(C.cell_on ? 0 : C.pq_list_count), 2);
+            if (C.cell_on) {
+                o.ctab = off = up(off);
+                off += static_cast<uint32_t>(C.ct_words) * 4u;
+            }
         } else if (accel == 1) {
             o.oct = off = up(off);
             off += words(static_cast<uint32_t>(C.oct_nodes), sizeof(RmOctNode));
@@ -702,6 +739,7 @@
     o.rel = C.lds_off[8];
     o.end = C.lds_off[9];
     o.step = C.lds_off[10];
+    o.ctab = C.lds_off[11];
     return o;
 }
 template <int ACCEL, bool LDS, bool REL>
@@ -867,9 +905,11 @@
                 off = lay.prims;
                 stage(smem, off, P.bvh_prims, P.bvh_prim_count);
                 off = lay.cells;
-                stage(smem, off, P.pq_cells, P.pq_cell_count);
+                stage(smem, off, P.pq_cells, P.cell_on ? 0 : P.pq_cell_count);
                 off = lay.list;
-                stage(smem, off, P.pq_list, P.pq_list_count);
+                stage(smem, off, P.pq_list, P.cell_on ? 0 : P.pq_list_count);
+                off = lay.ctab;
+                stage(smem, off, P.cell_tab, P.cell_on ? P.ct_words : 0);
             } else if (ACCEL == 1) {
                 off = lay.oct;
                 stage(smem, off, P.oct, P.oct_nodes);
@@ -1238,14 +1278,19 @@
         aux.found = 0;
         aux.rho = 0.f;
         aux.rho_cell = 0.f;
+        const bool cell_on = ACCEL == 2 && CB.cell_on != 0;
         if (ACCEL == 2) {
+            CellTabView CT;
+            CT.tab = LDS ? reinterpret_cast<const uint32_t *>(smem + CB.lds_off[11]) : CB.cell_tab;
+            CT.step = LDS ? reinterpret_cast<const uint32_t *>(smem + CB.lds_off[10]) : CB.step_tab;
+            CT.on = cell_on;
 #ifdef RM_STAMPS
             unsigned long long fbc = 0;
-            dist = bvh_distance_wave<UR>(CB, SB, need, q, evaluated, lane_b, coop, filter, use_grid, &fbc, &aux);
+            dist = bvh_distance_wave<UR>(CB, SB, need, q, evaluated, lane_b, coop, filter, use_grid, &fbc, &aux, CT);
             t_acc_[4] += fbc;
             t_prev_ += fbc;
 #else
-            dist = bvh_distance_wave<UR>(CB, SB, need, q, evaluated, lane_b, coop, filter, use_grid, nullptr, &aux);
+            dist = bvh_distance_wave<UR>(CB, SB, need, q, evaluated, lane_b, coop, filter, use_grid, nullptr, &aux, CT);
 #endif
         }
         else if (ACCEL == 1) dist = need ? oct_distance_lane(SB, onode, q, evaluated, filter) : RM_MAX_DIST;
@@ -1256,7 +1301,7 @@
         counters += evaluated << 16;
 
         RM_T(2)
-        const bool fuse = ACCEL == 2 && need && (st & ST_PHASE) == PH_N0 && aux.ok && aux.rho > RM_NRM_DELTA;
+        const bool fuse = ACCEL == 2 && need && (st & ST_PHASE) == PH_N0 && aux.ok && (cell_on || aux.rho > RM_NRM_DELTA);
         const bool was_marching = need && (st & ST_PHASE) == PH_MARCH;
         if (need) {
             const int ph = st & ST_PHASE;
@@ -1290,7 +1335,17 @@
                     const double r1 = SM.radii[aux.k1];
                     const bool step_box = CM.step_box != 0;
                     float b_lo[3], b_hi[3];
-                    if (step_box) {
+                    if (step_box && CM.cell_on) {
+                        const uint32_t *tab = LDS ? reinterpret_cast<const uint32_t *>(smem + CM.lds_off[10]) : CM.step_tab;
+                        const uint32_t *rec = (LDS ? reinterpret_cast<const uint32_t *>(smem + CM.lds_off[11]) : CM.cell_tab) + CM.ct_rec_off + 3u * (aux.found >> 16);
+                        const uint32_t w0 = rec[0], w1 = rec[1];
+#pragma unroll
+                        for (int k = 0; k < 3; ++k) {
+                            const float *T = reinterpret_cast<const float *>(tab + k * CM.sb_stride + (CM.sb_bins >> 2));
+                            b_lo[k] = T[(w0 >> (8 * k)) & 0xFFu];
+                            b_hi[k] = T[(w1 >> (8 * k)) & 0xFFu];
+                        }
+                    } else if (step_box) {
                         const uint32_t *tab = LDS ? reinterpret_cast<const uint32_t *>(smem + CM.lds_off[10]) : CM.step_tab;
                         const int last = CM.sb_stride - (CM.sb_bins >> 2) - 2;
                         const float qk[3] = {q.x, q.y, q.z};
@@ -1377,7 +1432,22 @@
             }
         }
         if (ACCEL == 2 && __any(fuse)) {
-            if (fuse) {
+            bool stable = true;
+            if (fuse && cell_on) {
+                const RmRenderParams CN = cold_params();
+                const uint32_t *tab = LDS ? reinterpret_cast<const uint32_t *>(smem + CN.lds_off[10]) : CN.step_tab;
+                const uint32_t *rec = (LDS ? reinterpret_cast<const uint32_t *>(smem + CN.lds_off[11]) : CN.cell_tab) + CN.ct_rec_off + 3u * (aux.found >> 16);
+                const uint32_t w0 = rec[0], w1 = rec[1];
+                const float qk[3] = {q.x, q.y, q.z};
+                float rho = __builtin_fmaxf(__builtin_fmaxf(__builtin_fabsf(q.x), __builtin_fabsf(q.y)), __builtin_fabsf(q.z)) < 16.0f ? __builtin_inff() : 0.f;
+#pragma unroll
+                for (int k = 0; k < 3; ++k) {
+                    const float *T = reinterpret_cast<const float *>(tab + k * CN.sb_stride + (CN.sb_bins >> 2));
+                    rho = __builtin_fminf(rho, __builtin_fminf(qk[k] - T[(w0 >> (8 * k)) & 0xFFu], T[(w1 >> (8 * k)) & 0xFFu] - qk[k]));
+                }
+                stable = rho > RM_NRM_DELTA;
+            }
+            if (fuse && stable) {
                 const SceneView SN = scene_view<ACCEL, LDS, REL>(cold_params(), smem);
                 const RmSphere s1 = SN.spheres[aux.k1];
                 const double r1 = SN.radii[aux.k1];
@@ -1447,7 +1517,8 @@
     const SceneView S = scene_view<2, false, false>(P, nullptr);
     uint32_t c = 0;
     NormalAux aux;
-    const double d = bvh_distance_wave<UR>(P, S, need, q, c, static_cast<int>(threadIdx.x & 63), P.coop != 0, P.filter != 0, P.use_grid != 0, nullptr, &aux);
+    const CellTabView CT = {P.cell_tab, P.step_tab, P.cell_on != 0};
+    const double d = bvh_distance_wave<UR>(P, S, need, q, c, static_cast<int>(threadIdx.x & 63), P.coop != 0, P.filter != 0, P.use_grid != 0, nullptr, &aux, CT);
     if (need) {
         dist[i] = d;
         count[i] = c;
@@ -1459,7 +1530,8 @@
     size_t b = 0;
     if (p.accel == 2) {
         b += up(static_cast<size_t>(p.bvh_nodes) * sizeof(RmBvhNode)) + up(static_cast<size_t>(p.bvh_prim_count) * 4);
-        b += up(static_cast<size_t>(p.pq_cell_count) * 4) + up(static_cast<size_t>(p.pq_list_count) * 2 + 4);
+        if (p.cell_on) b += 2 * 16 + up(static_cast<size_t>(p.ct_words) * 4);
+        else b += up(static_cast<size_t>(p.pq_cell_count) * 4) + up(static_cast<size_t>(p.pq_list_count) * 2 + 4);
     } else if (p.accel == 1) {
         b += up(static_cast<size_t>(p.oct_nodes) * sizeof(RmOctNode)) + up(static_cast<size_t>(p.oct_prim_count) * 4);
     }
@@ -1476,11 +1548,17 @@
     if (p.leaf_order) p.bvh_prim_count = 0;
     if (p.list_cap < 1) p.list_cap = 1;
     const bool want = p.accel == 2 && p.step_box != 0 && p.multi_step != 0 && p.sb_stride > 0;
-    auto pass = [&](bool with_table) {
+    const bool want_cells = want && p.cell_on != 0 && p.ct_words > 0 && !p.general;
+    auto pass = [&](bool with_table, bool with_cells = false, bool rel_allowed = true, int cap_most = 64) {
         RmRenderParams c = p;
         c.step_box = with_table ? 1 : 0;
+        c.cell_on = with_cells ? 1 : 0;
+        if (!rel_allowed) c.rel_boxes = 0;
+        if (c.list_cap > cap_most) c.list_cap = cap_most;
         RmV2Plan r;
         r.step_box = c.step_box;
+        r.cell_on = c.cell_on;
+        r.cell_refused = 0;
         r.list_cap = c.list_cap;
         r.list_bytes = c.accel == 2 ? static_cast<size_t>(4) * c.list_cap * 128 : 0;
         r.scene_bytes = scene_lds_bytes(c);
@@ -1488,9 +1566,15 @@
         r.rel = false;
         r.tier = 0;
         r.refused = 0;
-        if (!(r.lds && c.accel == 2)) return r;
         const size_t rel_bytes = static_cast<size_t>(c.bvh_nodes) * 48;
         constexpr size_t kLdsPerCu = 160 * 1024, kGranule = 1280, kStatic = sizeof(WaveDiag) * 4;
+        auto per_cu = [&](const RmV2Plan &v) {
+            const size_t bytes = (v.lds ? v.scene_bytes : 0) + (v.rel ? rel_bytes + 16 : 0) + v.list_bytes + 16 + kStatic;
+            const size_t n = kLdsPerCu / ((bytes + kGranule - 1) / kGranule * kGranule);
+            return static_cast<int>(n < RM_V2_WAVES ? n : RM_V2_WAVES);
+        };
+        r.per_cu = per_cu(r);
+        if (!(r.lds && c.accel == 2)) return r;
         auto budget_for = [&](size_t bytes) { return bytes / kGranule * kGranule - kStatic; };
         auto fits = [&](size_t extra, int cap, size_t budget) { return r.scene_bytes + extra + static_cast<size_t>(4) * cap * 128 + 16 <= budget; };
         auto trim = [&](size_t extra, size_t budget) {
@@ -1519,13 +1603,24 @@
             }
             r.rel = false;
         }
+        r.per_cu = per_cu(r);
         return r;
     };
     RmV2Plan plain = pass(false);
     if (!want) return plain;
-    const RmV2Plan with_table = pass(true);
-    if (with_table.lds == plain.lds && with_table.rel == plain.rel && with_table.tier <= plain.tier) return with_table;
+    RmV2Plan with_table = pass(true);
+    if (with_table.lds == plain.lds && with_table.rel == plain.rel && with_table.tier <= plain.tier) {
+        if (want_cells) {
+            const RmV2Plan with_cells = pass(true, true, with_table.rel, with_table.list_cap);
+            if (with_cells.lds && with_table.lds && with_cells.rel == with_table.rel && with_cells.tier <= with_table.tier &&
+                with_cells.list_cap >= with_table.list_cap)
+                return with_cells;
+            with_table.cell_refused = 1;
+        }
+        return with_table;
+    }
     plain.refused = 1;
+    plain.cell_refused = want_cells ? 1 : 0;
     return plain;
 }
 #endif
@@ -1628,6 +1723,7 @@
     const bool lds = plan.lds, rel = plan.rel;
     p.list_cap = plan.list_cap;
     p.step_box = plan.step_box;
+    p.cell_on = plan.cell_on;
     if (p.accel != 2 || !p.leaf_rects || !p.bvh_leaves || p.bvh_leaf_count <= 0 || p.bvh_leaf_count > RM_RECT_CULL_MAX_LEAVES ||
         p.width > 65536 || p.height > 65536)
         p.rect_cull = 0;
@@ -1639,8 +1735,8 @@
     }
     {
         const LdsLayout lay = lds_layout_host(p, p.accel, lds, rel && p.accel == 2);
-        const uint32_t v[11] = {lay.nodes, lay.prims, lay.cells, lay.list, lay.oct, lay.oct_prims, lay.spheres, lay.radii, lay.rel, lay.end, lay.step};
-        for (int k = 0; k < 11; ++k) p.lds_off[k] = v[k];
+        const uint32_t v[12] = {lay.nodes, lay.prims, lay.cells, lay.list, lay.oct, lay.oct_prims, lay.spheres, lay.radii, lay.rel, lay.end, lay.step, lay.ctab};
+        for (int k = 0; k < 12; ++k) p.lds_off[k] = v[k];
         if (lay.end + list_bytes > shmem) return hipErrorInvalidValue;
     }
     const int cus = p.num_cus > 0 ? p.num_cus : 256;
@@ -1654,6 +1750,7 @@
         shape[2] = static_cast<uint32_t>(shmem);
         shape[3] = p.step_box ? 1u : 0u;
         shape[4] = p.rect_cull ? 1u : 0u;
+        shape[5] = p.cell_on ? 1u : 0u;
     }
     hipError_t e = hipSuccess;
     if (!p.diag_block) e = hipMemsetAsync(p.tile_counters, 0, RM_QUEUES * RM_QSTRIDE * sizeof(unsigned int), stream);
diff --git a/cpu_raymarcher_amd/csrc/rm_scene_host.cpp b/cpu_raymarcher_amd/csrc/rm_scene_host.cpp
--- a/cpu_raymarcher_amd/csrc/rm_scene_host.cpp
+++ b/cpu_raymarcher_amd/csrc/rm_scene_host.cpp
@@ -1,9 +1,11 @@
 #include "rm_scene_host.h"
 
 #include <algorithm>
+#include <array>
 #include <cmath>
 #include <cstring>
 #include <limits>
+#include <map>
 #include <numeric>
 
 namespace rmh {
@@ -302,6 +304,150 @@
             bins[b] = static_cast<uint8_t>(i);
         }
     }
+}
+
+void build_cell_tab(HostScene &s) {
+    s.cell_tab.clear();
+    s.ct_dim[0] = s.ct_dim[1] = s.ct_dim[2] = 0;
+    s.ct_rec_off = s.ct_list_off = 0;
+    if (s.step_tab.empty() || s.general || s.program || s.bvh.empty() || s.bvh.size() >= 65536) return;
+    std::vector<float> th[3];
+    size_t cells = 1;
+    for (int k = 0; k < 3; ++k) {
+        const float *T = reinterpret_cast<const float *>(s.step_tab.data() + static_cast<size_t>(k) * s.sb_stride + s.sb_bins / 4);
+        const int slots = s.sb_stride - s.sb_bins / 4;
+        th[k].push_back(T[0]);
+        for (int i = 1; i < slots && std::isfinite(T[i]); ++i) th[k].push_back(T[i]);
+        s.ct_dim[k] = static_cast<int>(th[k].size());
+        cells *= th[k].size();
+    }
+    const int nx = s.ct_dim[0], ny = s.ct_dim[1], nz = s.ct_dim[2];
+    auto fail = [&]() {
+        s.cell_tab.clear();
+        s.ct_dim[0] = s.ct_dim[1] = s.ct_dim[2] = 0;
+        s.ct_rec_off = s.ct_list_off = 0;
+    };
+    if (cells > static_cast<size_t>(kCellTabCells)) return fail();
+    std::vector<int> leaves;
+    for (size_t i = 0; i < s.bvh.size(); ++i)
+        if (s.bvh[i].leaf >= 0 && (s.bvh[i].leaf & 0xFF) > 0) leaves.push_back(static_cast<int>(i));
+    auto contains = [](const RmBvhNode &nd, const float p[3]) {
+        return p[0] >= nd.lo[0] && p[0] <= nd.hi[0] && p[1] >= nd.lo[1] && p[1] <= nd.hi[1] && p[2] >= nd.lo[2] && p[2] <= nd.hi[2];
+    };
+    std::map<std::vector<int>, int> set_ids;
+    std::vector<std::vector<int>> sets;
+    std::vector<int> key(cells);
+    for (int z = 0; z < nz; ++z)
+        for (int y = 0; y < ny; ++y)
+            for (int x = 0; x < nx; ++x) {
+                const float p[3] = {th[0][x], th[1][y], th[2][z]};
+                std::vector<int> v;
+                v.push_back(contains(s.bvh[0], p) ? 1 : 0);
+                for (const int i : leaves)
+                    if (contains(s.bvh[i], p)) v.push_back(i);
+                auto it = set_ids.find(v);
+                if (it == set_ids.end()) {
+                    it = set_ids.emplace(v, static_cast<int>(sets.size())).first;
+                    sets.push_back(v);
+                }
+                key[(static_cast<size_t>(z) * ny + y) * nx + x] = it->second;
+            }
+    std::vector<uint16_t> lists;
+    std::map<std::vector<uint16_t>, uint32_t> list_at;
+    std::vector<uint32_t> set_w1(sets.size()), set_w2(sets.size());
+    for (size_t j = 0; j < sets.size(); ++j) {
+        std::vector<uint16_t> ids;
+        for (size_t e = 1; e < sets[j].size(); ++e) {
+            const RmBvhNode &nd = s.bvh[sets[j][e]];
+            const int first = nd.leaf >> 8, cnt = nd.leaf & 0xFF;
+            for (int k = 0; k < cnt; ++k) {
+                const int32_t id = s.bvh_prims[first + k];
+                if (id < 0 || id >= 65536) return fail();
+                ids.push_back(static_cast<uint16_t>(id));
+            }
+        }
+        if (ids.size() > 255) return fail();
+        auto it = list_at.find(ids);
+        if (it == list_at.end()) {
+            if (lists.size() + ids.size() > 65535) return fail();
+            it = list_at.emplace(ids, static_cast<uint32_t>(lists.size())).first;
+            lists.insert(lists.end(), ids.begin(), ids.end());
+        }
+        set_w1[j] = static_cast<uint32_t>(ids.size()) << 24;
+        set_w2[j] = it->second | (static_cast<uint32_t>(ids.size()) << 16);
+    }
+    std::vector<int> rec_of(cells, -1);
+    std::vector<uint32_t> recs;
+    std::map<std::array<uint32_t, 3>, int> rec_ids;
+    const int dim[3] = {nx, ny, nz};
+    for (int z = 0; z < nz; ++z)
+        for (int y = 0; y < ny; ++y)
+            for (int x = 0; x < nx; ++x) {
+                const size_t c = (static_cast<size_t>(z) * ny + y) * nx + x;
+                if (rec_of[c] >= 0) continue;
+                int lo[3] = {x, y, z}, hi[3] = {x + 1, y + 1, z + 1};
+                auto layer_ok = [&](int axis, int at) {
+                    int a[3] = {lo[0], lo[1], lo[2]}, b[3] = {hi[0], hi[1], hi[2]};
+                    a[axis] = at;
+                    b[axis] = at + 1;
+                    for (int cz = a[2]; cz < b[2]; ++cz)
+                        for (int cy = a[1]; cy < b[1]; ++cy)
+                            for (int cx = a[0]; cx < b[0]; ++cx)
+                                if (key[(static_cast<size_t>(cz) * ny + cy) * nx + cx] != key[c]) return false;
+                    return true;
+                };
+                for (bool grew = kCellTabMerge; grew;) {
+                    grew = false;
+                    for (int axis = 0; axis < 3; ++axis) {
+                        if (lo[axis] > 0 && layer_ok(axis, lo[axis] - 1)) {
+                            lo[axis] -= 1;
+                            grew = true;
+                        }
+                        if (hi[axis] < dim[axis] && layer_ok(axis, hi[axis])) {
+                            hi[axis] += 1;
+                            grew = true;
+                        }
+                    }
+                }
+                const uint32_t root = static_cast<uint32_t>(sets[key[c]][0]);
+                const std::array<uint32_t, 3> w = {
+                    static_cast<uint32_t>(lo[0]) | static_cast<uint32_t>(lo[1]) << 8 | static_cast<uint32_t>(lo[2]) << 16 | root << 24,
+                    static_cast<uint32_t>(hi[0]) | static_cast<uint32_t>(hi[1]) << 8 | static_cast<uint32_t>(hi[2]) << 16 | set_w1[key[c]],
+                    set_w2[key[c]]};
+                auto it = rec_ids.find(w);
+                if (it == rec_ids.end()) {
+                    it = rec_ids.emplace(w, static_cast<int>(recs.size() / 3)).first;
+                    recs.insert(recs.end(), w.begin(), w.end());
+                }
+                for (int cz = lo[2]; cz < hi[2]; ++cz)
+                    for (int cy = lo[1]; cy < hi[1]; ++cy)
+                        for (int cx = lo[0]; cx < hi[0]; ++cx) {
+                            int &r = rec_of[(static_cast<size_t>(cz) * ny + cy) * nx + cx];
+                            if (r < 0) r = it->second;
+                        }
+            }
+    const size_t cell_words = (cells + 1) / 2, list_words = (lists.size() + 1) / 2;
+    s.ct_rec_off = static_cast<int>(8 + cell_words);
+    s.ct_list_off = static_cast<int>(s.ct_rec_off + recs.size());
+    s.cell_tab.assign(static_cast<size_t>(s.ct_list_off) + list_words, 0);
+    uint32_t *w = s.cell_tab.data();
+    w[0] = static_cast<uint32_t>(nx);
+    w[1] = static_cast<uint32_t>(ny);
+    w[2] = static_cast<uint32_t>(nz);
+    w[3] = static_cast<uint32_t>(recs.size() / 3);
+    w[4] = static_cast<uint32_t>(s.ct_rec_off);
+    w[5] = static_cast<uint32_t>(s.ct_list_off);
+    w[6] = static_cast<uint32_t>(s.cell_tab.size());
+    {
+        std::vector<std::vector<int>> bare;
+        for (const auto &v : sets) bare.emplace_back(v.begin() + 1, v.end());
+        std::sort(bare.begin(), bare.end());
+        w[7] = static_cast<uint32_t>(std::unique(bare.begin(), bare.end()) - bare.begin());
+    }
+    uint16_t *cw = reinterpret_cast<uint16_t *>(w + 8);
+    for (size_t c = 0; c < cells; ++c) cw[c] = static_cast<uint16_t>(rec_of[c]);
+    std::copy(recs.begin(), recs.end(), w + s.ct_rec_off);
+    if (!lists.empty()) std::memcpy(w + s.ct_list_off, lists.data(), lists.size() * sizeof(uint16_t));
 }
 
 void build_exterior_grid(HostScene &s, const PairLoops *loops) {
@@ -736,6 +882,7 @@
             s.slot_object.swap(obj);
         }
     }
+    build_cell_tab(s);
     return true;
 }
 
diff --git a/cpu_raymarcher_amd/csrc/rm_scene_host.h b/cpu_raymarcher_amd/csrc/rm_scene_host.h
--- a/cpu_raymarcher_amd/csrc/rm_scene_host.h
+++ b/cpu_raymarcher_amd/csrc/rm_scene_host.h
@@ -10,6 +10,12 @@
 constexpr int kPresetCount = 19;
 constexpr int kStepBoxCap = 62;
 constexpr int kStepBoxBins = 32;
+constexpr int kCellTabCells = 4096;
+#ifdef RM_CELL_TAB_SINGLE
+constexpr bool kCellTabMerge = false;
+#else
+constexpr bool kCellTabMerge = true;
+#endif
 
 struct PrimDesc {
     int type = 0;
@@ -63,6 +69,9 @@
     int sb_bins = 0, sb_stride = 0;
     float sb_origin[3] = {0, 0, 0}, sb_inv[3] = {0, 0, 0};
     std::vector<uint32_t> step_tab;
+    int ct_dim[3] = {0, 0, 0};
+    int ct_rec_off = 0, ct_list_off = 0;
+    std::vector<uint32_t> cell_tab;
     std::vector<RmOctNode> oct;
     std::vector<int32_t> oct_prims;
     std::vector<RmSphereRec> oct_recs;
diff --git a/cpu_raymarcher_amd/csrc/rm_types.h b/cpu_raymarcher_amd/csrc/rm_types.h
--- a/cpu_raymarcher_amd/csrc/rm_types.h
+++ b/cpu_raymarcher_amd/csrc/rm_types.h
@@ -134,7 +134,7 @@
     int32_t launch_per_cu;
     int32_t v1_lists;
     int32_t v1_list_offset;
-    uint32_t lds_off[11];
+    uint32_t lds_off[12];
     int32_t prim_filter;
     int32_t n0_batch;
     const int32_t *stripe_ids;
@@ -200,4 +200,8 @@
     int32_t step_box;
     RmLeafRect *leaf_rects;
     int32_t rect_cull;
-};
+    const uint32_t *cell_tab;
+    int32_t ct_dim[3];
+    int32_t ct_rec_off, ct_list_off, ct_words;
+    int32_t cell_on;
+};
diff --git a/cpu_raymarcher_amd/csrc/rm_v2_fields.h b/cpu_raymarcher_amd/csrc/rm_v2_fields.h
--- a/cpu_raymarcher_amd/csrc/rm_v2_fields.h
+++ b/cpu_raymarcher_amd/csrc/rm_v2_fields.h
@@ -4,12 +4,13 @@
     X(width) X(height) X(accel) X(shader) X(tile_w) X(nodes_in_lds) X(filter) X(variant) X(list_cap) X(coop) X(use_grid)         \
     X(refill_threshold) X(hw_xcd) X(item_px) X(rel_boxes) X(lpt_stride) X(prim_filter) X(n0_batch) X(use_nn) X(tile_w_log2)     \
     X(tile_h_log2) X(tiles_x) X(item_wide) X(item_w_log2) X(sub_dx) X(sub_dy) X(tiles_x_magic) X(leaf_order) X(algorithm)       \
-    X(general) X(uniform_radius) X(multi_step) X(use_ext) X(step_box) X(sb_bins) X(sb_stride) X(rect_cull)
+    X(general) X(uniform_radius) X(multi_step) X(use_ext) X(step_box) X(sb_bins) X(sb_stride) X(rect_cull) \
+    X(ct_rec_off) X(ct_list_off) X(ct_words) X(cell_on)
 
 #define RM_V2_FIXED_COUNTS(X)                                                                                                    \
     X(n_prims) X(bvh_nodes) X(oct_nodes) X(bvh_prim_count) X(oct_prim_count) X(pq_cell_count) X(pq_list_count) X(bvh_leaf_count) \
     X(nn_cell_count) X(nn_list_count)
 
 #define RM_V2_FIXED_ARRAYS(X) \
-    X(pq_dim, 3) X(lds_off, 11) X(nn_dim, 3) X(pq_origin, 3) X(pq_inv, 3) X(pq_cell, 3) X(nn_inv, 3) X(light, 3) X(light_d, 3) \
-    X(ext_dim, 3) X(ext_origin, 3) X(ext_inv, 3) X(sb_origin, 3) X(sb_inv, 3)
+    X(pq_dim, 3) X(lds_off, 12) X(nn_dim, 3) X(pq_origin, 3) X(pq_inv, 3) X(pq_cell, 3) X(nn_inv, 3) X(light, 3) X(light_d, 3) \
+    X(ext_dim, 3) X(ext_origin, 3) X(ext_inv, 3) X(sb_origin, 3) X(sb_inv, 3) X(ct_dim, 3)
diff --git a/include/rm_raymarch.h b/include/rm_raymarch.h
--- a/include/rm_raymarch.h
+++ b/include/rm_raymarch.h
@@ -418,6 +418,7 @@
 RM_API int rm_debug_last_launch(rm_ctx *ctx, uint32_t out[4]);
 RM_API int rm_debug_overlap_fill(rm_ctx *ctx, int32_t asked, int64_t items, int32_t *effective);
 RM_API int rm_debug_step_box(rm_ctx *ctx, int32_t out[6]);
+RM_API int rm_debug_cell_tab(rm_ctx *ctx, int32_t out[12]);
 RM_API int rm_debug_rect_cull(rm_ctx *ctx, const float *rot9, const float *origin3, int32_t width, int32_t height, int32_t out[5]);
 RM_API int rm_debug_leaf_rects(rm_ctx *ctx, const float *rot9, const float *origin3, int32_t width, int32_t height,
                                uint16_t *rects, int32_t *nodes, int64_t cap, int64_t *n);
```

Result: faster. 1794 (median of 6 runs) (+5.2%).
